# keonlee9420/Comprehensive-Transformer-TTS

Hardware: AMD Instinct MI355X
Metric: mel-frames/sec (train step) LJSpeech batch=16, 1/2/4/8 MI355X (higher is better)
Workload: dtype f32; 1 GPU; LJSpeech transformer_fs2 batch=16/GPU seq<=128->mel<=1024x80; full train step fwd+loss+bwd+clip+Adam, dropout on; workload_detail=supervised durations (BASELINE configs[1]), global_batch=16, valid_frames_per_gpu=11992, padded_frames_per_gpu=16384, launch_mode=hipgraph(fwd+bwd | clip+adam), parallelism=dp1

## Files before the change

### comprehensive-transformer-tts_amd/_lib.py

```python
import ctypes as C
import os

_HERE = os.path.dirname(os.path.abspath(__file__))
LIB_PATH = os.environ.get("CTTS_LIB") or os.path.join(_HERE, "csrc", "libctts_hip.so")

_c_f32p = C.c_void_p
_i32, _i64, _f32, _u32, _vp = C.c_int32, C.c_int64, C.c_float, C.c_uint32, C.c_void_p


class GemmDesc(C.Structure):
    _fields_ = [
        ("A", _vp), ("B", _vp), ("C", _vp),
        ("M", _i32), ("N", _i32), ("K", _i32),
        ("lda", _i64), ("ldb", _i64), ("ldc", _i64),
        ("a_kc", _i32), ("b_kc", _i32),
        ("nb0", _i32), ("nb1", _i32),
        ("sA0", _i64), ("sA1", _i64), ("sB0", _i64), ("sB1", _i64), ("sC0", _i64), ("sC1", _i64),
        ("lens", _vp),
        ("lim_m", _i32), ("lim_n", _i32), ("lim_k", _i32),
        ("conv_T", _i32), ("conv_pad", _i32), ("conv_cin", _i32), ("conv_on_b", _i32),
        ("split_k", _i32),
        ("alpha", _f32),
        ("bias", _vp),
        ("Z", _vp), ("ldz", _i64),
        ("act", _i32),
        ("p_drop", _f32), ("seed", _vp), ("drop_offset", _u32),
        ("R", _vp), ("ldr", _i64),
        ("rowscale", _vp),
        ("row_lens", _vp), ("row_T", _i32), ("row_halo", _i32),
        ("tile_map", _vp),
        ("tile_group_n", _i32),
        ("E", _vp), ("rowsub", _vp),
        ("sk_ws", _vp), ("sk_ws_bytes", _i64),
        ("epi_bwd", _i32),
        ("split_out", _vp), ("split_out_floats", _i64),
        ("split_overwrite", _i32),
        ("bf16_split", _i32),
        ("A_planes", _vp),
        ("B_planes", _vp),
        ("C_planes", _vp),
    ]


class VconvDesc(C.Structure):
    _fields_ = [
        ("x", _vp), ("sxb", _i64), ("sxt", _i64), ("sxc", _i64),
        ("B", _i32), ("T", _i32), ("Cin", _i32), ("Cout", _i32), ("k", _i32), ("dil", _i32),
        ("transposed_u", _i32),
        ("act_in", _i32), ("slope", _f32),
        ("w", _vp), ("w_planes", _vp),
        ("bias", _vp),
        ("R", _vp),
        ("out", _vp),
        ("alpha", _f32), ("beta", _f32),
        ("bf16_split", _i32),
        ("lens", _vp), ("len_mul", _i32),
    ]


class VconvHDesc(C.Structure):
    _fields_ = [
        ("x", _vp), ("sxb", _i64), ("sxt", _i64), ("sxc", _i64),
        ("x_f32", _i32),
        ("B", _i32), ("T", _i32), ("Cin", _i32), ("Cout", _i32), ("k", _i32), ("dil", _i32),
        ("transposed_u", _i32),
        ("act_in", _i32), ("slope", _f32),
        ("w", _vp),
        ("bias", _vp),
        ("R", _vp),
        ("out", _vp),
        ("alpha", _f32), ("beta", _f32),
        ("lens", _vp), ("len_mul", _i32),
    ]


class PsumTask(C.Structure):
    _fields_ = [("src", _vp), ("dst", _vp), ("n", _i64), ("stride", _i64), ("count", _i32), ("alpha", _f32)]


class SplitTask(C.Structure):
    _fields_ = [("src", _vp), ("dst", _vp), ("rows", _i64), ("cols", _i64), ("ld", _i64)]


class RepackTask(C.Structure):
    _fields_ = [("src", _vp), ("dst", _vp), ("cout", _i32), ("cin", _i32), ("k", _i32)]


_SIGNATURES = {
    "ctts_conv_dgrad_weights": [C.POINTER(RepackTask), C.c_int, _vp],
    "ctts_gemm_split_plan": [C.POINTER(GemmDesc), C.POINTER(_i32), C.POINTER(_i64)],
    "ctts_partial_sums": [C.POINTER(PsumTask), C.c_int, _vp],
    "ctts_reduce_parts": [C.c_int, _i64, C.c_int],
    "ctts_xcd_probe": [_vp, C.c_int, _vp],
    "ctts_posembed_fwd": [_vp, _vp, _vp, _vp, _vp, _vp, _i64, C.c_int, _f32, _vp, _u32, _vp],
    "ctts_posembed_bwd": [_vp, _vp, _vp, _vp, _vp, _vp, _i64, C.c_int, _f32, _vp, _u32, C.c_int, _vp, _vp],
    "ctts_gemm": [C.POINTER(GemmDesc), _vp],
    "ctts_gemm_takes_persistent": [C.POINTER(GemmDesc)],
    "ctts_gemm_ws_enable": [C.c_int],
    "ctts_gemm_takes_weight_stationary": [C.POINTER(GemmDesc)],
    "ctts_gemm_takes_bf16_split": [C.POINTER(GemmDesc)],
    "ctts_gemm_takes_planes": [C.POINTER(GemmDesc)],
    "ctts_split_planes": [C.POINTER(SplitTask), C.c_int, _vp],
    "ctts_rowdot_heads": [_vp, _vp, _vp, C.c_int, C.c_int, C.c_int, C.c_int, _vp],
    "ctts_mel_prepare": [_vp, C.c_int, C.c_int, _vp, _vp],
    "ctts_mel_spectrogram": [_vp, _vp, _vp, _vp, _vp, _vp, _vp, _i64, C.c_int, C.c_int, C.c_int, C.c_int, C.c_int, _f32, C.c_int, _vp, _vp],
    "ctts_mha_fwd": [_vp, _vp, _vp, _vp, C.c_int, C.c_int, C.c_int, C.c_int, _f32, _vp],
    "ctts_mha_bwd": [_vp, _vp, _vp, _vp, _vp, _vp, _vp, _vp, _vp, C.c_int, C.c_int, C.c_int, C.c_int, _f32, C.c_int, _vp, _vp],
    "ctts_relmha_fwd": [_vp, _vp, _vp, _vp, _vp, _vp, C.c_int, C.c_int, C.c_int, C.c_int, _f32, _f32, _vp, _u32, _vp],
    "ctts_relmha_bwd": [_vp, _vp, _vp, _vp, _vp, _vp, _vp, _vp, _vp, _vp, _vp, _vp, _vp, C.c_int, C.c_int, C.c_int, C.c_int,
                        _f32, _f32, _vp, _u32, _vp],
    "ctts_weighted_colsum": [_vp, _vp, _vp, _i64, C.c_int, _f32, C.c_int, _vp, _vp, _vp],
    "ctts_epilogue_bwd": [_vp, _vp, _vp, _vp, _vp, _vp, _i64, C.c_int, C.c_int, _f32, _vp, _u32, _f32, C.c_int, _vp, _vp, _vp],
    "ctts_row_tile_map": [_vp, C.c_int, C.c_int, C.c_int, _vp, _vp],
    "ctts_conv_weight_repack": [_vp, _vp, C.c_int, C.c_int, C.c_int, C.c_int, _vp],
    "ctts_lr_index": [_vp, C.c_int, C.c_int, _vp, C.c_int, C.c_int, C.c_int, _vp, _vp, _vp, _vp],
    "ctts_lr_gather_fwd": [_vp, _vp, _vp, C.c_int, C.c_int, C.c_int, C.c_int, _vp],
    "ctts_lr_gather_bwd": [_vp, _vp, _vp, C.c_int, C.c_int, C.c_int, C.c_int, _vp],
    "ctts_embedding_fwd": [_vp, _vp, _vp, _i64, C.c_int, C.c_int, _vp],
    "ctts_embedding_bwd": [_vp, _vp, _vp, _i64, C.c_int, C.c_int, C.c_int, C.c_int, _vp, _vp],
    "ctts_positions": [_vp, C.c_int, _i64, C.c_int, C.c_int, _vp, _vp],
    "ctts_cwt_pitch": [_vp, _i64, C.c_int, _vp, _vp, _f32, _vp, C.c_int, _f32, _f32, _f32, C.c_int, _vp, _vp, _vp, C.c_int, C.c_int, C.c_int, _vp],
    "ctts_layernorm_fwd": [_vp, _vp, _vp, _vp, _vp, _vp, C.c_int, C.c_int, _f32, _f32, _vp, _u32, _vp, _vp, _vp],
    "ctts_layernorm_bwd": [_vp, _vp, _vp, _vp, _vp, _vp, _vp, _vp, C.c_int, C.c_int, _f32, _vp, _u32, _vp, C.c_int, _vp, _vp, _vp, _vp],
    "ctts_colstats": [_vp, _vp, C.c_int, C.c_int, _vp, _vp],
    "ctts_bn_finalize": [_vp, C.c_int, C.c_int, _f32, _f32, _vp, _vp, _vp, _vp, _vp, _vp],
    "ctts_bn_apply": [_vp, _vp, _vp, _vp, _vp, _vp, C.c_int, C.c_int, C.c_int, _f32, _vp, _u32, _vp, _vp],
    "ctts_bn_bwd_reduce": [_vp, _vp, _vp, _vp, _vp, _vp, _vp, C.c_int, C.c_int, C.c_int, _f32, _vp, _u32, _vp, _vp],
    "ctts_bn_bwd_apply": [_vp, _vp, _vp, _vp, _vp, _vp, _vp, _vp, _vp, _vp, C.c_int, C.c_int, C.c_int, _f32, _vp,
                          _u32, C.c_int, _vp, _vp],
    "ctts_softmax_fwd": [_vp, _vp, C.c_int, C.c_int, C.c_int, _i64, _vp],
    "ctts_softmax_bwd": [_vp, _vp, _vp, C.c_int, C.c_int, C.c_int, _i64, _vp],
    "ctts_act_dropout_bwd": [_vp, _vp, _vp, _i64, C.c_int, C.c_int, _f32, _f32, _vp, _u32, _vp],
    "ctts_rowscale_dropout": [_vp, _vp, _i64, C.c_int, _vp, _f32, _vp, _u32, _vp],
    "ctts_colsum": [_vp, _vp, _i64, C.c_int, _i64, _f32, C.c_int, _vp, _vp, _vp],
    "ctts_reflect_pad": [_vp, _vp, C.c_int, C.c_int, C.c_int, _i64, _vp],
    "ctts_stft_magnitude": [_vp, _i64, _vp, _i64, _vp, _i64, C.c_int, _vp],
    "ctts_log_clamp_transpose": [_vp, _vp, C.c_int, C.c_int, C.c_int, _f32, _vp],
    "ctts_relattn_split_fwd": [_vp, _vp, _vp, _vp, _vp, _vp, _i64, C.c_int, _vp],
    "ctts_relattn_split_bwd": [_vp, _vp, _vp, _vp, _i64, C.c_int, _vp],
    "ctts_glu_fwd": [_vp, _vp, _i64, C.c_int, _vp],
    "ctts_glu_bwd": [_vp, _vp, _vp, _i64, C.c_int, _vp],
    "ctts_dwconv_fwd": [_vp, _vp, _vp, C.c_int, C.c_int, C.c_int, C.c_int, C.c_int, _vp],
    "ctts_dwconv_wgrad": [_vp, _vp, _vp, _vp, C.c_int, C.c_int, C.c_int, C.c_int, C.c_int, _vp],
    "ctts_relpos_softmax_fwd": [_vp, _vp, _vp, C.c_int, C.c_int, _f32, _f32, _vp, _u32, _vp],
    "ctts_relpos_softmax_bwd": [_vp, _vp, C.c_int, C.c_int, _f32, _f32, _vp, _u32, _vp],
    "ctts_relshift_bwd": [_vp, _vp, C.c_int, C.c_int, _vp],
    "ctts_neg_sqdist": [_vp, _vp, _vp, C.c_int, C.c_int, C.c_int, C.c_int, _f32, _vp],
    "ctts_mas": [_vp, _vp, _vp, _vp, _vp, _vp, C.c_int, C.c_int, C.c_int, _vp],
    "ctts_forward_sum_fwd": [_vp, _vp, _vp, _f32, _vp, _vp, _vp, C.c_int, C.c_int, C.c_int, _vp],
    "ctts_forward_sum_bwd": [_vp, _vp, _vp, _f32, _vp, _vp, _vp, _vp, _vp, C.c_int, C.c_int, C.c_int, _vp],
    "ctts_var_loss_fwd": [_vp] * 2 + [C.c_int] + [_vp] * 12 + [C.c_int] * 3 + [_vp, C.c_int, _vp] + [_vp] * 4 + [_vp],
    "ctts_var_loss_bwd": [_vp] * 2 + [C.c_int] + [_vp] * 12 + [C.c_int] * 3 + [_vp, C.c_int, _vp] + [_vp] * 4 + [_vp] * 5 + [_vp],
    "ctts_bin_loss_fwd": [_vp, _vp, _i64, _vp, _vp, _vp],
    "ctts_bin_loss_bwd": [_vp, _vp, _vp, _vp, _vp, _i64, _vp],
    "ctts_masked_loss_fwd": [_vp, _vp, _vp, _i64, _i32, _vp, _vp, _vp],
    "ctts_masked_loss_bwd": [_vp, _vp, _vp, _vp, _vp, _vp, _i64, _i32, _vp],
    "ctts_mel_l1_fwd": [_vp, _vp, _vp, _vp, _vp, _vp, _i64, C.c_int, _vp, _vp],
    "ctts_mel_l1_bwd": [_vp, _vp, _vp, _vp, _vp, _vp, _vp, _vp, _i64, C.c_int, _vp],
    "ctts_adam_clip_step": [_vp, _vp, _vp, _vp, C.c_int64, _vp, _f32, _f32, _f32, _f32, _f32, _vp, _vp],
    "ctts_im2col_3x3s2": [_vp, _vp, C.c_int, C.c_int, C.c_int, C.c_int, _vp],
    "ctts_col2im_3x3s2": [_vp, _vp, C.c_int, C.c_int, C.c_int, C.c_int, _vp],
    "ctts_gru_fwd": [_vp, _vp, _vp, _vp, _vp, C.c_int, C.c_int, C.c_int, C.c_int, C.c_int, _vp],
    "ctts_gru_bwd": [_vp, _vp, _vp, _vp, _vp, _vp, _vp, C.c_int, C.c_int, C.c_int, C.c_int, C.c_int, _vp],
    "ctts_softmax_rect_fwd": [_vp, _vp, _vp, C.c_int, C.c_int, C.c_int, _vp],
    "ctts_softmax_rect_bwd": [_vp, _vp, _vp, _vp, C.c_int, C.c_int, C.c_int, _vp],
    "ctts_vocoder_conv": [C.POINTER(VconvDesc), _vp],
    "ctts_vocoder_post": [_vp, C.c_int, C.c_int, C.c_int, C.c_int, _vp, _vp, _f32, _vp, _vp],
    "ctts_vocoder_post_ragged": [_vp, C.c_int, C.c_int, C.c_int, C.c_int, _vp, _vp, _f32, _vp, _vp, C.c_int, _vp],
    "ctts_vocoder_conv_h": [C.POINTER(VconvHDesc), _vp],
    "ctts_vocoder_post_h": [_vp, C.c_int, C.c_int, C.c_int, C.c_int, _vp, _vp, _f32, _vp, _vp, C.c_int, _vp],
    "ctts_fastformer_pool_fwd": [_vp, _i64, _vp, _i64, _vp, _vp, _vp, _vp, C.c_int, C.c_int, C.c_int, C.c_int, _f32, _vp],
    "ctts_fastformer_pool_bwd": [_vp, _vp, _vp, _vp, _i64, _vp, _i64, _vp, _vp, _vp, _vp, C.c_int, C.c_int, C.c_int, C.c_int, _f32, _vp],
    "ctts_fastformer_bcast": [_vp, _i64, _vp, _vp, C.c_int, C.c_int, C.c_int, _vp],
    "ctts_fastformer_bcast_bwd": [_vp, _vp, _vp, _i64, _vp, _vp, _vp, _vp, _vp, C.c_int, C.c_int, C.c_int, _vp],
    "ctts_fastformer_resdrop": [_vp, _vp, _vp, _vp, _i64, C.c_int, _vp, _f32, _vp, _u32, C.c_int, _vp],
    "ctts_griffinlim_prepare": [_vp, C.c_int, C.c_int, _vp, _vp],
    "ctts_stft_transform": [_vp, _vp, _vp, _vp, _vp, _i64, _i64, _i64, C.c_int, C.c_int, C.c_int, C.c_int, _vp],
    "ctts_istft_frames": [_vp, _vp, _i64, _i64, _i64, _vp, _vp, _vp, _vp, C.c_int, C.c_int, C.c_int, C.c_int, _vp],
    "ctts_griffinlim_iter": [_vp, _vp, _vp, _vp, _vp, C.c_int, C.c_int, C.c_int, C.c_int, _vp],
    "ctts_istft_ola": [_vp, _vp, _vp, _vp, _i64, C.c_int, C.c_int, C.c_int, C.c_int, _vp],
    "ctts_griffinlim_iter_momentum": [_vp, _vp, _vp, _vp, _vp, _vp, _f32, C.c_int, C.c_int, C.c_int, C.c_int, C.c_int, _vp],
    "ctts_istft_frames_seeded": [_vp, _i64, _i64, _i64, _vp, _vp, _vp, _vp, _vp, C.c_int, C.c_int, C.c_int, C.c_int, _vp],
    "ctts_pitch_track_prepare": [_vp, _vp],
    "ctts_pitch_track": [_vp, _vp, _vp, _vp, _vp, _vp, C.c_int, C.c_int, C.c_int, C.c_int, _f32, _f32, _f32, _f32, _vp],
    "ctts_f0_targets": [_vp, _vp, _vp, _vp, _vp, _vp, _vp, C.c_int, C.c_int, _vp],
    "ctts_norm_interp_f0": [_vp, _vp, _vp, _vp, C.c_int, C.c_int, _f32, _vp],
    "ctts_trim_silence": [_vp, _vp, _vp, _vp, _vp, C.c_int, C.c_int, _f32, C.c_int, C.c_int, _vp],
    "ctts_attn_prior": [_vp, _vp, _vp, C.c_int, C.c_int, C.c_int, _i64, _i64, _f32, _vp],
    "ctts_outlier_stats": [_vp, _vp, _vp, _vp, _vp, _vp, _vp, _vp, C.c_int, C.c_int, _vp],
    "ctts_comm_unique_id": [_vp],
    "ctts_comm_create": [C.POINTER(_vp), _i32, _i32, _vp],
    "ctts_comm_destroy": [_vp],
    "ctts_allreduce_mean": [_vp, _i64, _vp, _vp],
}
COMM_ID_BYTES = 128
EXPORTED_SYMBOLS = sorted(list(_SIGNATURES) + ["ctts_last_error", "ctts_version", "ctts_mha_supported", "ctts_relmha_workspace_floats",
                                               "ctts_mel_spectrogram_workspace_bytes", "ctts_gemm_workspace_bytes", "ctts_workspace_bytes",
                                               "ctts_workspace_error_word", "ctts_fastformer_workspace_floats",
                                               "ctts_griffinlim_workspace_bytes", "ctts_griffinlim_state_floats",
                                               "ctts_pitch_track_workspace_bytes", "ctts_trim_silence_workspace_bytes"])
ADAM_STATE_FLOATS = 3 + 2048

_lib = None


class CttsError(RuntimeError):
    pass


def load():
    global _lib
    if _lib is not None:
        return _lib
    if not os.path.exists(LIB_PATH):
        raise CttsError(
            f"{LIB_PATH} not found - build it with comprehensive-transformer-tts_amd/csrc/build.sh "
            "(or __graft_entry__.build()).  There is no CPU / PyTorch fallback for the hot path."
        )
    lib = C.CDLL(LIB_PATH)
    for name, argtypes in _SIGNATURES.items():
        fn = getattr(lib, name)
        fn.argtypes = argtypes
        fn.restype = C.c_int
    lib.ctts_last_error.restype = C.c_char_p
    lib.ctts_last_error.argtypes = []
    lib.ctts_version.restype = C.c_int
    lib.ctts_version.argtypes = []
    lib.ctts_mha_supported.restype = C.c_int
    lib.ctts_mha_supported.argtypes = [C.c_int, C.c_int]
    lib.ctts_mel_spectrogram_workspace_bytes.restype = C.c_size_t
    lib.ctts_mel_spectrogram_workspace_bytes.argtypes = [C.c_int, C.c_int]
    lib.ctts_gemm_workspace_bytes.restype = C.c_size_t
    lib.ctts_gemm_workspace_bytes.argtypes = []
    lib.ctts_workspace_bytes.restype = C.c_size_t
    lib.ctts_workspace_bytes.argtypes = []
    lib.ctts_workspace_error_word.restype = C.c_void_p
    lib.ctts_workspace_error_word.argtypes = [C.c_void_p]
    lib.ctts_fastformer_workspace_floats.restype = C.c_size_t
    lib.ctts_fastformer_workspace_floats.argtypes = [C.c_int, C.c_int, C.c_int, C.c_int]
    lib.ctts_griffinlim_workspace_bytes.restype = C.c_size_t
    lib.ctts_griffinlim_workspace_bytes.argtypes = [C.c_int, C.c_int]
    lib.ctts_griffinlim_state_floats.restype = C.c_size_t
    lib.ctts_griffinlim_state_floats.argtypes = [C.c_int, C.c_int]
    lib.ctts_pitch_track_workspace_bytes.restype = C.c_size_t
    lib.ctts_pitch_track_workspace_bytes.argtypes = []
    lib.ctts_trim_silence_workspace_bytes.restype = C.c_size_t
    lib.ctts_trim_silence_workspace_bytes.argtypes = [C.c_int, C.c_int, C.c_int]
    lib.ctts_relmha_workspace_floats.restype = C.c_size_t
    lib.ctts_relmha_workspace_floats.argtypes = [C.c_int, C.c_int, C.c_int]
    _lib = lib
    return lib

# ... 6 lines not shown
```

### comprehensive-transformer-tts_amd/csrc/elementwise.hip

```cpp
#include "ctts_common.h"

namespace {
__global__ void zero_u32_kernel(uint32_t* __restrict__ p, size_t n) {
  for (size_t i = (size_t)blockIdx.x * blockDim.x + threadIdx.x; i < n; i += (size_t)gridDim.x * blockDim.x) p[i] = 0u;
}
}

int ctts_zero_async(void* p, size_t bytes, hipStream_t st) {
  if (bytes == 0) return 0;
  const size_t n = (bytes + 3) / 4;
  const unsigned blocks = (unsigned)((n + 255) / 256 > 2048 ? 2048 : (n + 255) / 256);
  hipLaunchKernelGGL(zero_u32_kernel, dim3(blocks), dim3(256), 0, st, (uint32_t*)p, n);
  return hipGetLastError() == hipSuccess ? 0 : -1;
}

namespace {

__global__ void act_dropout_bwd_kernel(const float* __restrict__ dg, const float* __restrict__ z, float* __restrict__ dz,
                                       long total, int act, float p_drop, const uint64_t* seed, uint32_t drop_offset) {
  const bool do_drop = p_drop > 0.f;
  uint32_t dkey = 0; float inv_keep = 1.f;
  if (do_drop) { dkey = ctts_drop_key(seed, drop_offset); inv_keep = 1.f / (1.f - p_drop); }
  if (total & 3) {
    for (long i = (long)blockIdx.x * blockDim.x + threadIdx.x; i < total; i += (long)gridDim.x * blockDim.x) {
      float g = dg[i];
      if (do_drop) g *= ctts_drop_scale(dkey, (uint32_t)i, p_drop, inv_keep);
      dz[i] = g * ctts_act_grad(z[i], act);
    }
    return;
  }
  const long n4 = total >> 2;
  for (long i = (long)blockIdx.x * blockDim.x + threadIdx.x; i < n4; i += (long)gridDim.x * blockDim.x) {
    const float4 g = reinterpret_cast<const float4*>(dg)[i];
    const float4 zz = reinterpret_cast<const float4*>(z)[i];
    float ga[4] = {g.x, g.y, g.z, g.w};
    const float za[4] = {zz.x, zz.y, zz.z, zz.w};
#pragma unroll
    for (int e = 0; e < 4; ++e) {
      if (do_drop) ga[e] *= ctts_drop_scale(dkey, (uint32_t)(i * 4 + e), p_drop, inv_keep);
      ga[e] *= ctts_act_grad(za[e], act);
    }
    reinterpret_cast<float4*>(dz)[i] = make_float4(ga[0], ga[1], ga[2], ga[3]);
  }
}

__global__ void rowscale_dropout_kernel(const float* __restrict__ x, float* __restrict__ y, long total, int C,
                                        const float* __restrict__ rowscale, float p_drop, const uint64_t* seed,
                                        uint32_t drop_offset) {
  const bool do_drop = p_drop > 0.f;
  uint32_t dkey = 0; float inv_keep = 1.f;
  if (do_drop) { dkey = ctts_drop_key(seed, drop_offset); inv_keep = 1.f / (1.f - p_drop); }
  if (C & 3) {
    for (long i = (long)blockIdx.x * blockDim.x + threadIdx.x; i < total; i += (long)gridDim.x * blockDim.x) {
      float a = x[i];
      if (do_drop) a *= ctts_drop_scale(dkey, (uint32_t)i, p_drop, inv_keep);
      y[i] = a * (rowscale ? rowscale[i / C] : 1.f);
    }
    return;
  }
  const long n4 = total >> 2;
  const int C4 = C >> 2;
  for (long i = (long)blockIdx.x * blockDim.x + threadIdx.x; i < n4; i += (long)gridDim.x * blockDim.x) {
    const float4 v = reinterpret_cast<const float4*>(x)[i];
    float a[4] = {v.x, v.y, v.z, v.w};
    const float sc = rowscale ? rowscale[i / C4] : 1.f;
#pragma unroll
    for (int e = 0; e < 4; ++e) {
      if (do_drop) a[e] *= ctts_drop_scale(dkey, (uint32_t)(i * 4 + e), p_drop, inv_keep);
      a[e] *= sc;
    }
    reinterpret_cast<float4*>(y)[i] = make_float4(a[0], a[1], a[2], a[3]);
  }
}

__device__ __forceinline__ void ctts_colsum_emit(float tot, float* s64, float* __restrict__ out, int c, int C, int creal, float scale,
                                                 int accumulate) {
  const int ty = threadIdx.x >> 6, l = threadIdx.x & 63;
  if (C != creal) {
    __syncthreads();
    if (ty == 0) s64[l] = c < C ? tot : 0.f;
    __syncthreads();
    if (ty == 0 && l < creal) {
      float a = 0.f;
      for (int j = l; j < C; j += creal) a += s64[j];
      out[l] = accumulate ? out[l] + scale * a : scale * a;
    }
    return;
  }
  if (ty == 0 && c < C) out[c] = accumulate ? out[c] + scale * tot : scale * tot;
}

__global__ __launch_bounds__(256) void colsum_kernel(const float* __restrict__ x, float* __restrict__ out, long rows, int C,
                                                      int creal, long ld, float scale, unsigned char* ws, int G, int accumulate,
                                                      float* __restrict__ parts) {
  __shared__ float s[4][64];
  const int c = blockIdx.x * 64 + (threadIdx.x & 63), ty = threadIdx.x >> 6;
  const long stripe = (rows + gridDim.y - 1) / gridDim.y;
  const long r0 = blockIdx.y * stripe, r1 = min(rows, r0 + stripe);
  float a = 0.f;
  if (c < C) {
#pragma unroll 4
    for (long r = r0 + ty; r < r1; r += 4) a += x[r * ld + c];
  }
  s[ty][threadIdx.x & 63] = a;
  __syncthreads();
  float tot[1] = {0.f};
  if (ty == 0) { const int l = threadIdx.x; tot[0] = s[0][l] + s[1][l] + s[2][l] + s[3][l]; }
  if (parts) {
    if (ty == 0 && c < C) parts[(long)blockIdx.y * C + c] = tot[0];
    return;
  }
  if (!ctts_ordered_colsum<float, 1>(tot, ws, blockIdx.x, blockIdx.y, gridDim.y, G)) return;
  ctts_colsum_emit(tot[0], s[0], out, c, C, creal, scale, accumulate);
}

__global__ __launch_bounds__(256) void epilogue_bwd_kernel(const float* __restrict__ dy, const float* __restrict__ rowscale,
                                                            const float* __restrict__ z, float* __restrict__ dz, float* __restrict__ gm,
                                                            float* __restrict__ dbias, long rows, int C, int act, float p_drop,
                                                            const uint64_t* seed, uint32_t drop_offset, float bias_scale,
                                                            unsigned char* ws, int G, int accumulate, float* __restrict__ parts) {
  __shared__ float s[4][64];
  const int c = blockIdx.x * 64 + (threadIdx.x & 63), ty = threadIdx.x >> 6;
  const long stripe = (rows + gridDim.y - 1) / gridDim.y;
  const long r0 = blockIdx.y * stripe, r1 = min(rows, r0 + stripe);
  const bool do_drop = p_drop > 0.f;
  uint32_t dkey = 0; float inv_keep = 1.f;
  if (do_drop) { dkey = ctts_drop_key(seed, drop_offset); inv_keep = 1.f / (1.f - p_drop); }
  float a = 0.f;
  if (c < C) {
#pragma unroll 4
    for (long r = r0 + ty; r < r1; r += 4) {
      const long e = r * C + c;
      float g = dy[e];
      if (rowscale) g *= rowscale[r];
      if (gm) gm[e] = g;
      if (do_drop) g *= ctts_drop_scale(dkey, (uint32_t)e, p_drop, inv_keep);
      if (z) g *= ctts_act_grad(z[e], act);
      dz[e] = g;
      a += g;
    }
  }
  if (!dbias && !parts) return;
  s[ty][threadIdx.x & 63] = a;
  __syncthreads();
  float tot[1] = {0.f};
  if (ty == 0) { const int l = threadIdx.x; tot[0] = s[0][l] + s[1][l] + s[2][l] + s[3][l]; }
  if (parts) {
    if (ty == 0 && c < C) parts[(long)blockIdx.y * C + c] = tot[0];
    return;
  }
  if (!ctts_ordered_colsum<float, 1>(tot, ws, blockIdx.x, blockIdx.y, gridDim.y, G)) return;
  ctts_colsum_emit(tot[0], s[0], dbias, c, C, C, bias_scale, accumulate);
}
// ... 151 lines not shown
    return 0;
  }
  const int gx = (C + 63) / 64;
  const int gy = colsum_stripes(gx, min((long)max(1, 1024 / gx), (long)rows / 64), ws != nullptr || parts != nullptr);
  hipLaunchKernelGGL(weighted_colsum_kernel, dim3(gx, gy), dim3(256), 0, st, x, w, out, (long)rows, C, scale, (unsigned char*)ws,
                     ctts_red_group(gy), accumulate, parts);
  CTTS_CHECK_LAUNCH("ctts_weighted_colsum");
  return 0;
}

extern "C" int ctts_colsum(const float* x, float* out, int64_t rows, int C, int64_t ld, float scale, int accumulate, void* ws,
                           float* parts, void* stream) {
  CTTS_REQUIRE(x && (out || parts) && C > 0 && (C + 63) / 64 <= CTTS_RED_MAX_COLBLOCKS, "ctts_colsum: bad arguments");
  CTTS_REQUIRE(!parts || ctts_reduce_parts(0, rows, C) > 0, "ctts_colsum: this shape has no deferred mode (ctts_reduce_parts = 0)");
  hipStream_t st = (hipStream_t)stream;
  if (rows == 0) {
    if (!accumulate && ctts_zero_async(out, sizeof(float) * C, st) != 0) { ctts_set_error("ctts_colsum: zero fill failed"); return -2; }
    return 0;
  }
  int k = 1;
  if (ld == C && !parts)
    while (C * k * 2 <= 64 && rows % (k * 2) == 0) k *= 2;
  const int Cv = C * k, gx = (Cv + 63) / 64;
  const long Rv = rows / k;
  const int gy = colsum_stripes(gx, min((long)max(1, 1024 / gx), Rv / 64), ws != nullptr || parts != nullptr);
  hipLaunchKernelGGL(colsum_kernel, dim3(gx, gy), dim3(256), 0, st, x, out, Rv, Cv, C, (long)ld * k, scale, (unsigned char*)ws,
                     ctts_red_group(gy), accumulate, parts);
  CTTS_CHECK_LAUNCH("ctts_colsum");
  return 0;
}

extern "C" int ctts_epilogue_bwd(const float* dy, const float* rowscale, const float* z, float* dz, float* gm, float* dbias,
                                 int64_t rows, int C, int act, float p_drop, const uint64_t* seed, uint32_t drop_offset, float bias_scale,
                                 int accumulate_bias, void* ws, float* parts, void* stream) {
  CTTS_REQUIRE(dy && dz && rows >= 0 && C > 0 && p_drop >= 0.f && p_drop < 1.f && (p_drop == 0.f || seed), "ctts_epilogue_bwd: bad arguments");
  CTTS_REQUIRE(!dbias || (C + 63) / 64 <= CTTS_RED_MAX_COLBLOCKS, "ctts_epilogue_bwd: C too large for the bias-gradient reduction");
  hipStream_t st = (hipStream_t)stream;
  if (rows == 0) {
    if (dbias && !accumulate_bias && ctts_zero_async(dbias, sizeof(float) * C, st) != 0) { ctts_set_error("ctts_epilogue_bwd: zero fill failed"); return -2; }
    return 0;
  }
  const int gx = (C + 63) / 64;
  const long want = min((long)max(1, 2048 / gx), (long)rows / 32);
  CTTS_REQUIRE(!parts || rows > 0, "ctts_epilogue_bwd: deferred bias gradient needs rows > 0");
  const int gy = (dbias || parts) ? colsum_stripes(gx, want, ws != nullptr || parts != nullptr) : (int)max((long)1, want);
  hipLaunchKernelGGL(epilogue_bwd_kernel, dim3(gx, gy), dim3(256), 0, st, dy, rowscale, act ? z : nullptr, dz, gm, dbias, (long)rows, C, act,
                     p_drop, seed, drop_offset, bias_scale, (unsigned char*)ws, ctts_red_group(gy), accumulate_bias, parts);
  CTTS_CHECK_LAUNCH("ctts_epilogue_bwd");
  return 0;
}

extern "C" int ctts_conv_weight_repack(const float* src, float* dst, int cout, int cin, int k, int mode, void* stream) {
  CTTS_REQUIRE(src && dst && mode >= 0 && mode <= 4, "ctts_conv_weight_repack: bad arguments");
  const long total = (long)cout * cin * k;
  if (total == 0) return 0;
  hipLaunchKernelGGL(conv_weight_repack_kernel, dim3(grid_for(total)), dim3(256), 0, (hipStream_t)stream, src, dst, cout, cin, k,
                     mode, total);
  CTTS_CHECK_LAUNCH("ctts_conv_weight_repack");
  return 0;
}

extern "C" int ctts_reflect_pad(const float* y, float* ypad, int B, int N, int pad, int64_t ld_out, void* stream) {
  CTTS_REQUIRE(y && ypad && N > pad && ld_out >= N + 2 * pad, "ctts_reflect_pad: need N > pad and ld_out >= N + 2*pad");
  const long total = (long)B * ld_out;
  if (total == 0) return 0;
  hipLaunchKernelGGL(reflect_pad_kernel, dim3(grid_for(total)), dim3(256), 0, (hipStream_t)stream, y, ypad, N, pad, (long)ld_out, total);
  CTTS_CHECK_LAUNCH("ctts_reflect_pad");
  return 0;
}

extern "C" int ctts_stft_magnitude(const float* reim, int64_t ld_reim, float* mag, int64_t ld_mag, float* energy,
                                   int64_t frames, int nbins, void* stream) {
  CTTS_REQUIRE(reim && mag && energy && ld_mag >= nbins, "ctts_stft_magnitude: bad arguments");
  if (frames == 0) return 0;
  const int blocks = (int)min((frames + 3) / 4, (int64_t)4096);
  hipLaunchKernelGGL(stft_magnitude_kernel, dim3(blocks), dim3(256), 0, (hipStream_t)stream, reim, (long)ld_reim, mag,
                     (long)ld_mag, energy, (long)frames, nbins);
  CTTS_CHECK_LAUNCH("ctts_stft_magnitude");
  return 0;
}

extern "C" int ctts_log_clamp_transpose(const float* mel_fm, float* out, int B, int F, int n_mel, float clip, void* stream) {
  CTTS_REQUIRE(mel_fm && out, "ctts_log_clamp_transpose: null pointer");
  const long total = (long)B * F * n_mel;
  if (total == 0) return 0;
  hipLaunchKernelGGL(log_clamp_transpose_kernel, dim3(grid_for(total)), dim3(256), 0, (hipStream_t)stream, mel_fm, out, F, n_mel,
                     clip, total);
  CTTS_CHECK_LAUNCH("ctts_log_clamp_transpose");
  return 0;
}


namespace {
constexpr int RPK_BATCH = 32;
struct RepackBatch {
  const float* src[RPK_BATCH];
  float* dst[RPK_BATCH];
  int cout[RPK_BATCH], cin[RPK_BATCH], k[RPK_BATCH];
  int first_block[RPK_BATCH + 1];
  int ntasks;
};

__global__ __launch_bounds__(256) void conv_dgrad_weights_kernel(const RepackBatch b) {
  __shared__ float tile[32][33];
  int t = 0;
  while (t + 1 < b.ntasks && (int)blockIdx.x >= b.first_block[t + 1]) ++t;
  const float* __restrict__ src = b.src[t];
  float* __restrict__ dst = b.dst[t];
  const int cout = b.cout[t], cin = b.cin[t], k = b.k[t];
  const int tco = (cout + 31) / 32, tci = (cin + 31) / 32;
  int blk = (int)blockIdx.x - b.first_block[t];
  const int kk = blk / (tco * tci);
  blk -= kk * tco * tci;
  const int co0 = (blk / tci) * 32, ci0 = (blk % tci) * 32;
  const int tx = threadIdx.x & 31, ty = threadIdx.x >> 5;
#pragma unroll
  for (int r = ty; r < 32; r += 8) {
    const int co = co0 + r, ci = ci0 + tx;
    tile[r][tx] = (co < cout && ci < cin) ? src[((long)co * k + (k - 1 - kk)) * cin + ci] : 0.f;
  }
  __syncthreads();
#pragma unroll
  for (int r = ty; r < 32; r += 8) {
    const int ci = ci0 + r, co = co0 + tx;
    if (ci < cin && co < cout) dst[((long)ci * k + kk) * cout + co] = tile[tx][r];
  }
}
}

extern "C" int ctts_conv_dgrad_weights(const ctts_repack_task* tasks, int ntasks, void* stream) {
  CTTS_REQUIRE(ntasks >= 0 && (tasks || ntasks == 0), "ctts_conv_dgrad_weights: bad arguments");
  hipStream_t st = (hipStream_t)stream;
  for (int t0 = 0; t0 < ntasks; t0 += RPK_BATCH) {
    RepackBatch b;
    b.ntasks = 0;
    int blocks = 0;
    for (int t = t0; t < ntasks && t < t0 + RPK_BATCH; ++t) {
      const ctts_repack_task& q = tasks[t];
      CTTS_REQUIRE(q.src && q.dst && q.cout > 0 && q.cin > 0 && q.k > 0, "ctts_conv_dgrad_weights: bad task %d", t);
      const int i = b.ntasks++;
      b.src[i] = q.src; b.dst[i] = q.dst; b.cout[i] = q.cout; b.cin[i] = q.cin; b.k[i] = q.k;
      b.first_block[i] = blocks;
      blocks += ((q.cout + 31) / 32) * ((q.cin + 31) / 32) * q.k;
    }
    if (b.ntasks == 0) continue;
    b.first_block[b.ntasks] = blocks;
    hipLaunchKernelGGL(conv_dgrad_weights_kernel, dim3(blocks), dim3(256), 0, st, b);
    CTTS_CHECK_LAUNCH("ctts_conv_dgrad_weights");
  }
  return 0;
}

namespace {
__global__ __launch_bounds__(256) void posembed_fwd_kernel(const float4* __restrict__ x, const int32_t* __restrict__ pos, const float4* __restrict__ table,
                                                            const float* __restrict__ alpha, const float* __restrict__ rowscale, float4* __restrict__ y,
                                                            long n4, int C4, float p_drop, const uint64_t* seed, uint32_t drop_offset) {
#pragma clang fp contract(off)
  const bool do_drop = p_drop > 0.f;
  uint32_t dkey = 0; float inv_keep = 1.f;
  if (do_drop) { dkey = ctts_drop_key(seed, drop_offset); inv_keep = 1.f / (1.f - p_drop); }
  const float a = alpha ? alpha[0] : 1.f;
  for (long i = (long)blockIdx.x * blockDim.x + threadIdx.x; i < n4; i += (long)gridDim.x * blockDim.x) {
    const long row = i / C4;
    const int c = (int)(i - row * C4);
    const float4 xv = x[i], tv = table[(long)pos[row] * C4 + c];
    float v[4] = {xv.x + a * tv.x, xv.y + a * tv.y, xv.z + a * tv.z, xv.w + a * tv.w};
    const float sc = rowscale ? rowscale[row] : 1.f;
#pragma unroll
    for (int e = 0; e < 4; ++e) {
      if (do_drop) v[e] *= ctts_drop_scale(dkey, (uint32_t)(i * 4 + e), p_drop, inv_keep);
      v[e] *= sc;
    }
    y[i] = make_float4(v[0], v[1], v[2], v[3]);
  }
}

__global__ __launch_bounds__(256) void posembed_bwd_kernel(const float4* __restrict__ dy, const int32_t* __restrict__ pos, const float4* __restrict__ table,
                                                            const float* __restrict__ rowscale, float4* __restrict__ dx, float* __restrict__ dalpha,
                                                            long n4, int C4, float p_drop, const uint64_t* seed, uint32_t drop_offset,
                                                            unsigned char* ws, int G, int accumulate) {
  __shared__ float s_w[4];
  const bool do_drop = p_drop > 0.f;
  uint32_t dkey = 0; float inv_keep = 1.f;
  if (do_drop) { dkey = ctts_drop_key(seed, drop_offset); inv_keep = 1.f / (1.f - p_drop); }
  float dot = 0.f;
  for (long i = (long)blockIdx.x * blockDim.x + threadIdx.x; i < n4; i += (long)gridDim.x * blockDim.x) {
    const long row = i / C4;
    const int c = (int)(i - row * C4);
    const float4 g = dy[i];
    float v[4] = {g.x, g.y, g.z, g.w};
    const float sc = rowscale ? rowscale[row] : 1.f;
#pragma unroll
    for (int e = 0; e < 4; ++e) {
      v[e] *= sc;
      if (do_drop) v[e] *= ctts_drop_scale(dkey, (uint32_t)(i * 4 + e), p_drop, inv_keep);
    }
    dx[i] = make_float4(v[0], v[1], v[2], v[3]);
    if (dalpha) {
      const float4 tv = table[(long)pos[row] * C4 + c];
      dot += v[0] * tv.x + v[1] * tv.y + v[2] * tv.z + v[3] * tv.w;
    }
  }
  if (!dalpha) return;
  dot = ctts_wave_sum(dot);
  if ((threadIdx.x & 63) == 0) s_w[threadIdx.x >> 6] = dot;
  __syncthreads();
  float tot[1] = {0.f};
  if (threadIdx.x == 0) tot[0] = ((s_w[0] + s_w[1]) + s_w[2]) + s_w[3];
  if (!ctts_ordered_colsum<float, 1>(tot, ws, 0, blockIdx.x, gridDim.x, G)) return;
  if (threadIdx.x == 0) dalpha[0] = accumulate ? dalpha[0] + tot[0] : tot[0];
}
}

extern "C" int ctts_posembed_fwd(const float* x, const int32_t* pos, const float* table, const float* alpha, const float* rowscale, float* y,
                                 int64_t rows, int C, float p_drop, const uint64_t* seed, uint32_t drop_offset, void* stream) {
  CTTS_REQUIRE(x && pos && table && y && rows >= 0 && C > 0 && (C % 4) == 0 && p_drop >= 0.f && p_drop < 1.f && (p_drop == 0.f || seed),
               "ctts_posembed_fwd: bad arguments (C %% 4 must be 0)");
  const long n4 = (long)rows * (C / 4);
  if (n4 == 0) return 0;
  hipLaunchKernelGGL(posembed_fwd_kernel, dim3(grid_for(n4)), dim3(256), 0, (hipStream_t)stream, (const float4*)x, pos, (const float4*)table, alpha,
                     rowscale, (float4*)y, n4, C / 4, p_drop, seed, drop_offset);
  CTTS_CHECK_LAUNCH("ctts_posembed_fwd");
  return 0;
}

extern "C" int ctts_posembed_bwd(const float* dy, const int32_t* pos, const float* table, const float* rowscale, float* dx, float* dalpha,
                                 int64_t rows, int C, float p_drop, const uint64_t* seed, uint32_t drop_offset, int accumulate, void* ws,
                                 void* stream) {
  CTTS_REQUIRE(dy && dx && rows >= 0 && C > 0 && (C % 4) == 0 && p_drop >= 0.f && p_drop < 1.f && (p_drop == 0.f || seed) &&
               (!dalpha || (pos && table)), "ctts_posembed_bwd: bad arguments (C %% 4 must be 0)");
  const long n4 = (long)rows * (C / 4);
  hipStream_t st = (hipStream_t)stream;
  if (n4 == 0) {
    if (dalpha && !accumulate && ctts_zero_async(dalpha, sizeof(float), st) != 0) return -2;
    return 0;
  }
  int grid = grid_for(n4, 1024);
  if (dalpha && !ws) grid = 1;
  hipLaunchKernelGGL(posembed_bwd_kernel, dim3(grid), dim3(256), 0, st, (const float4*)dy, pos, (const float4*)table, rowscale, (float4*)dx, dalpha,
                     n4, C / 4, p_drop, seed, drop_offset, (unsigned char*)ws, ctts_red_group(grid), accumulate);
  CTTS_CHECK_LAUNCH("ctts_posembed_bwd");
  return 0;
}

namespace {
constexpr int PSUM_BATCH = 24;
struct PsumBatch {
  const float* src[PSUM_BATCH];
  float* dst[PSUM_BATCH];
  long n[PSUM_BATCH];
  long stride[PSUM_BATCH];
  int count[PSUM_BATCH];
  float alpha[PSUM_BATCH];
  int first_block[PSUM_BATCH + 1];
  int ntasks;
};

#ifndef CTTS_PSUM_CHUNKS
#define CTTS_PSUM_CHUNKS 8
#endif
constexpr int PSUM_CHUNKS = CTTS_PSUM_CHUNKS;
__global__ __launch_bounds__(256) void partial_sums_kernel(const PsumBatch b) {
  int t = 0;
  while (t + 1 < b.ntasks && (int)blockIdx.x >= b.first_block[t + 1]) ++t;
  const float* src = b.src[t];
  float* dst = b.dst[t];
  const long n = b.n[t], stride = b.stride[t];
  const int count = b.count[t];
  const float alpha = b.alpha[t];
  const bool aligned = !(stride & 3) && !((reinterpret_cast<uintptr_t>(src) | reinterpret_cast<uintptr_t>(dst)) & 15);
  const long s4 = stride >> 2;
#pragma unroll 1
  for (int c = 0; c < PSUM_CHUNKS; ++c) {
    const long i0 = (((long)(blockIdx.x - b.first_block[t]) * PSUM_CHUNKS + c) * 256 + threadIdx.x) * 4;
    if (i0 >= n) return;
    if (aligned && i0 + 4 <= n) {
      const float4* p = reinterpret_cast<const float4*>(src + i0);
      float4 a = make_float4(0.f, 0.f, 0.f, 0.f);
      for (int s = 0; s < count; s += 8) {
        float4 v[8];
#pragma unroll
        for (int u = 0; u < 8; ++u) v[u] = (s + u < count) ? p[(long)(s + u) * s4] : make_float4(0.f, 0.f, 0.f, 0.f);
#pragma unroll
        for (int u = 0; u < 8; ++u) { a.x += v[u].x; a.y += v[u].y; a.z += v[u].z; a.w += v[u].w; }
      }
      float4 cc = *reinterpret_cast<float4*>(dst + i0);
      cc.x += alpha * a.x; cc.y += alpha * a.y; cc.z += alpha * a.z; cc.w += alpha * a.w;
      *reinterpret_cast<float4*>(dst + i0) = cc;
    } else {
      for (int q = 0; q < 4 && i0 + q < n; ++q) {
        float a = 0.f;
        for (int s = 0; s < count; ++s) a += src[(long)s * stride + i0 + q];
        dst[i0 + q] += alpha * a;
      }
    }
  }
}
}

extern "C" int ctts_partial_sums(const ctts_psum_task* tasks, int ntasks, void* stream) {
  CTTS_REQUIRE(ntasks >= 0 && (tasks || ntasks == 0), "ctts_partial_sums: bad arguments");
  hipStream_t st = (hipStream_t)stream;
  for (int t0 = 0; t0 < ntasks; t0 += PSUM_BATCH) {
    PsumBatch b;
    b.ntasks = 0;
    int blocks = 0;
// ... 17 lines not shown
```

### comprehensive-transformer-tts_amd/csrc/gemm_common.h

```cpp
#pragma once
#include "ctts_common.h"

typedef float floatx16 __attribute__((ext_vector_type(16)));

namespace {

template <int MT, int NT>
__device__ __forceinline__ void gemm_epilogue(const ctts_gemm_desc& d, floatx16 (&acc)[MT][NT], float* Cb, int z, int row0, int col0,
                                              int wm0, int wn0, int l31, int h, int Mv, int Nv) {
  const float alpha = d.alpha;
  const bool do_drop = d.p_drop > 0.f;
  uint32_t dkey = 0;
  float inv_keep = 1.f;
  if (do_drop) { dkey = ctts_drop_key(d.seed, d.drop_offset); inv_keep = 1.f / (1.f - d.p_drop); }
  const uint32_t zoff = (uint32_t)z * (uint32_t)d.M * (uint32_t)d.N;
  if (d.E) {
    const float* Eb = d.E + (Cb - d.C);
    const float* rs = d.rowsub + (long)z * d.M;
#pragma unroll
    for (int i = 0; i < MT; ++i)
#pragma unroll
      for (int j = 0; j < NT; ++j) {
        const int n = col0 + wn0 + j * 32 + l31;
#pragma unroll
        for (int r = 0; r < 16; ++r) {
          const int m = row0 + wm0 + i * 32 + (r & 3) + 8 * (r >> 2) + 4 * h;
          if (m < Mv && n < Nv) Cb[(long)m * d.ldc + n] = Eb[(long)m * d.ldc + n] * (alpha * acc[i][j][r] - rs[m]);
        }
      }
    return;
  }
  if (d.epi_bwd) {
#pragma unroll
    for (int i = 0; i < MT; ++i)
#pragma unroll
      for (int j = 0; j < NT; ++j) {
        const int n = col0 + wn0 + j * 32 + l31;
#pragma unroll
        for (int r = 0; r < 16; ++r) {
          const int m = row0 + wm0 + i * 32 + (r & 3) + 8 * (r >> 2) + 4 * h;
          if (m < Mv && n < Nv) {
            float v = alpha * acc[i][j][r];
            if (do_drop) v *= ctts_drop_scale(dkey, zoff + (uint32_t)m * (uint32_t)d.N + (uint32_t)n, d.p_drop, inv_keep);
            if (d.act) v *= ctts_act_grad(d.Z[(long)m * d.ldz + n], d.act);
            Cb[(long)m * d.ldc + n] = v;
          }
        }
      }
    return;
  }
#pragma unroll
  for (int i = 0; i < MT; ++i)
#pragma unroll
    for (int j = 0; j < NT; ++j) {
      const int n = col0 + wn0 + j * 32 + l31;
      const float bv = (d.bias && n < Nv) ? d.bias[n] : 0.f;
#pragma unroll
      for (int r = 0; r < 16; ++r) {
        const int m = row0 + wm0 + i * 32 + (r & 3) + 8 * (r >> 2) + 4 * h;
        if (m < Mv && n < Nv) {
          float v = alpha * (acc[i][j][r] + bv);
          if (d.Z) d.Z[(long)m * d.ldz + n] = v;
          v = ctts_act(v, d.act);
          if (do_drop) v *= ctts_drop_scale(dkey, zoff + (uint32_t)m * (uint32_t)d.N + (uint32_t)n, d.p_drop, inv_keep);
          if (d.R) v += d.R[(long)m * d.ldr + n];
          if (d.rowscale) v *= d.rowscale[m];
          Cb[(long)m * d.ldc + n] = v;
        }
      }
    }
}


constexpr unsigned GEMM_OOB = 0x80000000u;

typedef __bf16 gemm_bf16x2 __attribute__((ext_vector_type(2)));
typedef float gemm_floatx2 __attribute__((ext_vector_type(2)));
__device__ __forceinline__ void gemm_split3(float x, unsigned& hi, unsigned& mid, unsigned& lo) {
  const gemm_floatx2 v0 = {x, 0.f};
  unsigned hb = __builtin_bit_cast(unsigned, __builtin_convertvector(v0, gemm_bf16x2)) & 0xFFFFu;
  const bool x_fin = fabsf(x) < __builtin_inff();
  if ((hb & 0x7F80u) == 0x7F80u) {
    if (x_fin) hb = (hb & 0x8000u) | 0x7F7Fu;
    else { hi = hb; mid = 0u; lo = 0u; return; }
  }
  const float r1 = x - __uint_as_float(hb << 16);
  const gemm_floatx2 v1 = {r1, 0.f};
  const unsigned mb = __builtin_bit_cast(unsigned, __builtin_convertvector(v1, gemm_bf16x2)) & 0xFFFFu;
  const float r2 = r1 - __uint_as_float(mb << 16);
  const gemm_floatx2 v2 = {r2, 0.f};
  const unsigned lb = __builtin_bit_cast(unsigned, __builtin_convertvector(v2, gemm_bf16x2)) & 0xFFFFu;
  hi = hb; mid = mb; lo = lb;
}
__device__ __host__ __forceinline__ bool gemm_fits32(const void* p, long M, long ld, long N);

__device__ __forceinline__ __amdgpu_buffer_rsrc_t gemm_rsrc(const void* p, long bytes) {
  return __builtin_amdgcn_make_buffer_rsrc(const_cast<void*>(p), 0, (int)bytes, 0x00020000);
}

template <int MT, int NT, int ACT, bool DROP, bool BWD, bool AUX, bool RS = false, bool PLANES = false>
__device__ __forceinline__ void gemm_epilogue_lean(const ctts_gemm_desc& d, const floatx16 (&acc)[MT][NT], float* Cb, int z, int row0,
                                                   int col0, int wm0, int wn0, int l31, int h, int Mv, int Nv) {
#pragma clang fp contract(off)
  const bool planes_on = PLANES && d.C_planes != nullptr;
  const __amdgpu_buffer_rsrc_t rp = gemm_rsrc(d.C_planes, planes_on ? (long)Mv * d.ldc * 6 : 0);
  const unsigned p_row = (unsigned)(d.ldc * 6);
  const unsigned p_sel = (l31 & 1) ? 0x03020706u : 0x05040100u;
  const float alpha = d.alpha;
  uint32_t dkey = 0;
  float inv_keep = 1.f;
  if (DROP) { dkey = ctts_drop_key(d.seed, d.drop_offset); inv_keep = 1.f / (1.f - d.p_drop); }
  const uint32_t zoff = (uint32_t)z * (uint32_t)d.M * (uint32_t)d.N;
  const uint32_t dthr = DROP ? ctts_drop_threshold(d.p_drop) : 0u;
  const uint32_t drow = (uint32_t)d.N * CTTS_DROP_G;
  const long last = Mv - 1;
  const float* aux_p = BWD ? d.Z : d.R;
  const long aux_ld = BWD ? d.ldz : d.ldr;
  const bool has_z = !BWD && ACT && d.Z;
  const __amdgpu_buffer_rsrc_t rc = gemm_rsrc(Cb, (last * d.ldc + Nv) * 4);
  const __amdgpu_buffer_rsrc_t ra = gemm_rsrc(aux_p, AUX ? (last * aux_ld + Nv) * 4 : 0);
  const __amdgpu_buffer_rsrc_t rz = gemm_rsrc(d.Z, has_z ? (last * d.ldz + Nv) * 4 : 0);
  const __amdgpu_buffer_rsrc_t rr = gemm_rsrc(d.rowscale, RS ? (long)Mv * 4 : 0);
  const unsigned c_row = (unsigned)(d.ldc * 4), a_row = (unsigned)(aux_ld * 4), z_row = (unsigned)(d.ldz * 4);
#pragma unroll
  for (int j = 0; j < NT; ++j) {
    const int n = col0 + wn0 + j * 32 + l31;
    const bool n_ok = n < Nv;
    const unsigned c_lane = n_ok ? (unsigned)(4 * h) * c_row + (unsigned)n * 4u : GEMM_OOB;
    const unsigned a_lane = n_ok ? (unsigned)(4 * h) * a_row + (unsigned)n * 4u : GEMM_OOB;
    const unsigned z_lane = n_ok ? (unsigned)(4 * h) * z_row + (unsigned)n * 4u : GEMM_OOB;
    const float bv = (!BWD && d.bias && n_ok) ? d.bias[n] : 0.f;
    const uint32_t dlane = (zoff + (uint32_t)(4 * h) * (uint32_t)d.N + (uint32_t)n) * CTTS_DROP_G + dkey;
    const unsigned p_lane = n_ok ? (unsigned)(4 * h + (l31 & 1)) * p_row + (unsigned)(n >> 5) * 192u + (unsigned)(n & 30) * 2u : GEMM_OOB;
#pragma unroll
    for (int ib = 0; ib < 2 * MT; ++ib) {
      const int i = ib >> 1, rb = (ib & 1) * 8;
      float aux[8], rs[8];
      if (AUX) {
#pragma unroll
        for (int q = 0; q < 8; ++q) {
          const int r = rb + q, mu = row0 + wm0 + i * 32 + (r & 3) + 8 * (r >> 2);
          aux[q] = __builtin_bit_cast(float, __builtin_amdgcn_raw_buffer_load_b32(ra, a_lane + (unsigned)mu * a_row, 0, 0));
        }
      }
      if (RS) {
#pragma unroll
        for (int q = 0; q < 8; ++q) {
          const int r = rb + q, mu = row0 + wm0 + i * 32 + (r & 3) + 8 * (r >> 2);
          rs[q] = __builtin_bit_cast(float, __builtin_amdgcn_raw_buffer_load_b32(rr, (unsigned)(mu + 4 * h) * 4u, 0, 0));
        }
      }
#pragma unroll
      for (int q = 0; q < 8; ++q) {
        const int r = rb + q, mu = row0 + wm0 + i * 32 + (r & 3) + 8 * (r >> 2);
        const int m = mu + 4 * h;
        float v;
        if (BWD) {
          v = alpha * acc[i][j][r];
          if (DROP) v *= ctts_drop_scale_pre(dlane + (uint32_t)mu * drow, dthr, inv_keep);
          if (ACT) v *= ctts_act_grad(aux[q], ACT);
        } else {
          v = alpha * (acc[i][j][r] + bv);
          if (ACT) __builtin_amdgcn_raw_buffer_store_b32(__builtin_bit_cast(unsigned, v), rz, z_lane + (unsigned)mu * z_row, 0, 0);
          v = ctts_act(v, ACT);
          if (DROP) v *= ctts_drop_scale_pre(dlane + (uint32_t)mu * drow, dthr, inv_keep);
          if (AUX) v += aux[q];
          if (RS) v *= rs[q];
        }
        __builtin_amdgcn_raw_buffer_store_b32(__builtin_bit_cast(unsigned, v), rc, c_lane + (unsigned)mu * c_row, 0, 0);
        if (PLANES) aux[q] = v;
      }
      if (PLANES) {
        if (planes_on) {
#pragma unroll
          for (int q = 0; q < 8; q += 2) {
            const int r = rb + q, mu = row0 + wm0 + i * 32 + (r & 3) + 8 * (r >> 2);
            unsigned ha, ma, la, hb, mb, lb;
            gemm_split3(aux[q], ha, ma, la);
            gemm_split3(aux[q + 1], hb, mb, lb);
            const unsigned own[3] = {ha | (hb << 16), ma | (mb << 16), la | (lb << 16)};
#pragma unroll
            for (int pc = 0; pc < 3; ++pc) {
              const unsigned nbr = (unsigned)__builtin_amdgcn_mov_dpp((int)own[pc], 0xB1, 0xF, 0xF, true);
              const unsigned out = __builtin_amdgcn_perm(nbr, own[pc], p_sel);
              __builtin_amdgcn_raw_buffer_store_b32(out, rp, p_lane + (unsigned)mu * p_row + (unsigned)(pc * 64), 0, 0);
            }
          }
        }
      }
    }
  }
}

template <int MT, int NT>
__device__ __forceinline__ void gemm_accumulate_lean(const ctts_gemm_desc& d, const floatx16 (&acc)[MT][NT], float* Cb, int row0, int col0,
                                                     int wm0, int wn0, int l31, int h, int Mv, int Nv) {
  const __amdgpu_buffer_rsrc_t rc = gemm_rsrc(Cb, ((long)(Mv - 1) * d.ldc + Nv) * 4);
  const unsigned c_row = (unsigned)(d.ldc * 4);
#pragma unroll
  for (int j = 0; j < NT; ++j) {
    const int n = col0 + wn0 + j * 32 + l31;
    const unsigned c_lane = n < Nv ? (unsigned)(4 * h) * c_row + (unsigned)n * 4u : GEMM_OOB;
#pragma unroll
    for (int ib = 0; ib < 2 * MT; ++ib) {
      const int i = ib >> 1, rb = (ib & 1) * 8;
      float old[8];
#pragma unroll
      for (int q = 0; q < 8; ++q) {
        const int r = rb + q, mu = row0 + wm0 + i * 32 + (r & 3) + 8 * (r >> 2);
        old[q] = __builtin_bit_cast(float, __builtin_amdgcn_raw_buffer_load_b32(rc, c_lane + (unsigned)mu * c_row, 0, 0));
      }
#pragma unroll
      for (int q = 0; q < 8; ++q) {
        const int r = rb + q, mu = row0 + wm0 + i * 32 + (r & 3) + 8 * (r >> 2);
        const float v = old[q] + d.alpha * acc[i][j][r];
        __builtin_amdgcn_raw_buffer_store_b32(__builtin_bit_cast(unsigned, v), rc, c_lane + (unsigned)mu * c_row, 0, 0);
      }
    }
  }
}

__device__ __host__ __forceinline__ long gemm_partial_ld(int N) { return (long)((N + 3) / 4) * 4; }
__device__ __forceinline__ float* gemm_partial_base(const ctts_gemm_desc& d, int z, int split) {
  float* P = reinterpret_cast<float*>(reinterpret_cast<unsigned char*>(d.sk_ws) + CTTS_WS_SLABS);
  return P + ((long)z * d.split_k + split) * (long)d.M * gemm_partial_ld(d.N);
}

template <int MT, int NT>
__device__ __forceinline__ void gemm_softmax_bwd_lean(const ctts_gemm_desc& d, const floatx16 (&acc)[MT][NT], float* Cb, int z, int row0,
                                                      int col0, int wm0, int wn0, int l31, int h, int Mv, int Nv) {
  const long bytes = ((long)(Mv - 1) * d.ldc + Nv) * 4;
  const __amdgpu_buffer_rsrc_t rc = gemm_rsrc(Cb, bytes);
  const __amdgpu_buffer_rsrc_t re = gemm_rsrc(d.E + (Cb - d.C), bytes);
  const __amdgpu_buffer_rsrc_t rr = gemm_rsrc(d.rowsub + (long)z * d.M, (long)Mv * 4);
  const unsigned c_row = (unsigned)(d.ldc * 4);
#pragma unroll
  for (int i = 0; i < MT; ++i) {
    float rs[16];
#pragma unroll
    for (int r = 0; r < 16; ++r)
      rs[r] = __builtin_bit_cast(float, __builtin_amdgcn_raw_buffer_load_b32(rr, (unsigned)(row0 + wm0 + i * 32 + (r & 3) + 8 * (r >> 2) + 4 * h) * 4u, 0, 0));
#pragma unroll
    for (int j = 0; j < NT; ++j) {
      const int n = col0 + wn0 + j * 32 + l31;
      const unsigned c_lane = n < Nv ? (unsigned)(4 * h) * c_row + (unsigned)n * 4u : GEMM_OOB;
#pragma unroll
      for (int rb = 0; rb < 16; rb += 8) {
        float e[8];
#pragma unroll
        for (int q = 0; q < 8; ++q) {
          const int r = rb + q, mu = row0 + wm0 + i * 32 + (r & 3) + 8 * (r >> 2);
          e[q] = __builtin_bit_cast(float, __builtin_amdgcn_raw_buffer_load_b32(re, c_lane + (unsigned)mu * c_row, 0, 0));
        }
#pragma unroll
        for (int q = 0; q < 8; ++q) {
          const int r = rb + q, mu = row0 + wm0 + i * 32 + (r & 3) + 8 * (r >> 2);
          const float v = e[q] * (d.alpha * acc[i][j][r] - rs[r]);
          __builtin_amdgcn_raw_buffer_store_b32(__builtin_bit_cast(unsigned, v), rc, c_lane + (unsigned)mu * c_row, 0, 0);
        }
      }
    }
  }
}

__device__ __host__ __forceinline__ bool gemm_fits32(const void* p, long M, long ld, long N) {
  return !p || ((M + 128) * ld * 4 < 0x7FFF0000L && ld >= N);
}

template <int MT, int NT>
__device__ __forceinline__ void gemm_epilogue_auto(const ctts_gemm_desc& d, floatx16 (&acc)[MT][NT], float* Cb, int z, int row0, int col0,
                                                   int wm0, int wn0, int l31, int h, int Mv, int Nv) {
  const bool flat = d.nb0 * d.nb1 == 1 && Mv == d.M && Nv == d.N;
  const bool c_ok = gemm_fits32(Cb, Mv, d.ldc, Nv);
  if (d.E) {
    if (c_ok) return gemm_softmax_bwd_lean<MT, NT>(d, acc, Cb, z, row0, col0, wm0, wn0, l31, h, Mv, Nv);
  } else if (c_ok && (flat ? gemm_fits32(d.Z, d.M, d.ldz, d.N) && gemm_fits32(d.R, d.M, d.ldr, d.N) : !d.Z && !d.R && !d.rowscale)) {
#define CTTS_LEAN(ACT, DROP, BWD, AUX, RS) \
  return gemm_epilogue_lean<MT, NT, ACT, DROP, BWD, AUX, RS>(d, acc, Cb, z, row0, col0, wm0, wn0, l31, h, Mv, Nv)
    const bool drop = d.p_drop > 0.f, res = d.R != nullptr, rs = d.rowscale != nullptr;
    if (!d.epi_bwd) {
      if (d.act == 0 && !d.Z) {
        if (!res && !rs && !drop) CTTS_LEAN(0, false, false, false, false);
        if (res && !rs) { if (drop) CTTS_LEAN(0, true, false, true, false); else CTTS_LEAN(0, false, false, true, false); }
        if (res && rs) { if (drop) CTTS_LEAN(0, true, false, true, true); else CTTS_LEAN(0, false, false, true, true); }
      } else if (!res && !rs && flat) {
        if (d.act == 1 && !drop) CTTS_LEAN(1, false, false, false, false);
        if (d.act == 2) { if (drop) CTTS_LEAN(2, true, false, false, false); else CTTS_LEAN(2, false, false, false, false); }
        if (d.act == 4) { if (drop) CTTS_LEAN(4, true, false, false, false); else CTTS_LEAN(4, false, false, false, false); }
      }
    } else if (d.Z && !rs && flat) {
      if (d.act == 1 && !drop) CTTS_LEAN(1, false, true, true, false);
      if (d.act == 2 && drop) CTTS_LEAN(2, true, true, true, false);
      if (d.act == 4 && drop) CTTS_LEAN(4, true, true, true, false);
    }
#undef CTTS_LEAN
  }
  gemm_epilogue<MT, NT>(d, acc, Cb, z, row0, col0, wm0, wn0, l31, h, Mv, Nv);
}

}

int ctts_gemm_sk_try(const ctts_gemm_desc& d, hipStream_t st);

int ctts_gemm_ws_try(const ctts_gemm_desc& d, hipStream_t st);

int ctts_gemm_pl_try(const ctts_gemm_desc& d, hipStream_t st);

int ctts_gemm_plw_try(const ctts_gemm_desc& d, hipStream_t st);
int ctts_gemm_plw_takes(const ctts_gemm_desc& d);
```

### comprehensive-transformer-tts_amd/csrc/gemm_pl.hip

```cpp
#include "gemm_pl_common.h"
#include "planes_common.h"
#include <stdlib.h>
#include <type_traits>

namespace {

struct PlArgs {
  int tiles_m, tiles_n;
  int nkb;
  int gw;
  int whole_tiles;
  int ntap;
  int nutt, tpu;
  int debug;
  unsigned* ws;
};

__host__ __device__ __forceinline__ int pl_epilogue_kind(const ctts_gemm_desc& d) {
  const bool drop = d.p_drop > 0.f, res = d.R != nullptr, rs = d.rowscale != nullptr;
  if (d.E || !gemm_fits32(d.C, d.M, d.ldc, d.N) || !gemm_fits32(d.Z, d.M, d.ldz, d.N) || !gemm_fits32(d.R, d.M, d.ldr, d.N)) return -1;
  if (d.epi_bwd) {
    if (d.Z && !rs && drop && d.act == 2) return 8;
    if (d.Z && !rs && drop && d.act == 4) return 9;
    return -1;
// ... 250 lines not shown
    const bool do_mma = PL_DBG(8) == 0 && !(SKEW && idle);
    if (do_mma) {
      read_frag(stage, 1, f1);
      mma_terms(f0, 0, 6);
      if constexpr (TERMS == 1) { PL_INTERLEAVE_4x1(); } else { PL_INTERLEAVE_12(); }
    }
    __builtin_amdgcn_sched_barrier(0);
    __builtin_amdgcn_s_waitcnt(0xC07F);
    asm volatile("s_waitcnt vmcnt(0)\n\ts_barrier" ::: "memory");
    if constexpr (!SKEW) {
      if (have_l && !PL_DBG(1)) loader_issue(stage);
      __builtin_amdgcn_sched_barrier(0);
    }
    if (do_mma) {
      read_frag(stage ^ 1, 0, f0);
      mma_terms(f1, 0, 6);
      if constexpr (TERMS == 1) { PL_INTERLEAVE_4x1(); } else { PL_INTERLEAVE_12(); }
    }
    __builtin_amdgcn_sched_barrier(0);
    if constexpr (SKEW) {
      if (have_l && !PL_DBG(1)) loader_issue(stage);
    }
    if (have_l) loader_advance();
    --remaining;
    ++ckb;
    stage ^= 1;
    if (ckb < cp.kb_hi) continue;

    int e_l31 = l31, e_h = h, e_wm0 = wm0, e_wn0 = wn0;
    unsigned long long kargs = (unsigned long long)(const void*)__builtin_amdgcn_kernarg_segment_ptr();
    asm volatile("" : "+v"(e_l31), "+v"(e_h), "+s"(e_wm0), "+s"(e_wn0), "+s"(kargs));
    const ctts_gemm_desc& dc = *(const ctts_gemm_desc*)(const __attribute__((address_space(4))) ctts_gemm_desc*)kargs;
    const int Mv = dc.M, Nv = dc.N;
    int row0, col0; bool pad_hi;
    decode(cp, row0, col0, pad_hi);
    if (cp.kb_hi < nkb) {
      const unsigned base = (unsigned)blockIdx.x * (PL_SLAB * 4) + (unsigned)(wave * (PL_SLAB / 8) + lane * 4) * 4u;
#pragma unroll
      for (int i = 0; i < 2; ++i)
#pragma unroll
        for (int j = 0; j < 2; ++j)
#pragma unroll
          for (int q = 0; q < 4; ++q) {
            pl_u32x4 v;
            v.x = __float_as_uint(acc[i][j][4 * q + 0]); v.y = __float_as_uint(acc[i][j][4 * q + 1]);
            v.z = __float_as_uint(acc[i][j][4 * q + 2]); v.w = __float_as_uint(acc[i][j][4 * q + 3]);
            __builtin_amdgcn_raw_buffer_store_b128(v, rs_src, base + (unsigned)(((i * 2 + j) * 4 + q) * 1024), 0, 16);
          }
      asm volatile("s_waitcnt vmcnt(0)" ::: "memory");
      __syncthreads();
      if (tid == 0) __hip_atomic_store((pl_gu32*)(flags + blockIdx.x), 1u, __ATOMIC_RELAXED, __HIP_MEMORY_SCOPE_AGENT);
    } else {
      if (cp.kb_lo > 0) {
        const int tile_lo = cp.t * nkb;
        const int Ux = (rg.T1 - rg.T0) * nkb;
        int upper = rg.lo;
        for (int jj = wj - 1; jj >= 0 && upper > tile_lo; --jj) {
          const int blo = sk_bound(g, Ux, jj);
          if (blo >= upper) continue;
          upper = blo;
          const int src = jj * 8 + xcd;
          if (tid == 0) {
            unsigned spins = 0;
            while (__hip_atomic_load((pl_gu32*)(flags + src), __ATOMIC_RELAXED, __HIP_MEMORY_SCOPE_AGENT) != 1u) {
              __builtin_amdgcn_s_sleep(8);
              if (++spins > (1u << 24)) {
                __hip_atomic_store((pl_gu32*)(flags + PL_MAX_WG), 1u + (unsigned)src, __ATOMIC_RELAXED, __HIP_MEMORY_SCOPE_AGENT);
                break;
              }
            }
            __hip_atomic_store((pl_gu32*)(flags + src), 0u, __ATOMIC_RELAXED, __HIP_MEMORY_SCOPE_AGENT);
            __builtin_amdgcn_fence(__ATOMIC_ACQUIRE, "agent");
          }
          asm volatile("s_waitcnt vmcnt(0)" ::: "memory");
          __syncthreads();
          const unsigned base = (unsigned)src * (PL_SLAB * 4) + (unsigned)(wave * (PL_SLAB / 8) + lane * 4) * 4u;
#pragma unroll
          for (int g = 0; g < 16 / PL_SLAB_BATCH; ++g) {
            pl_u32x4 sv[PL_SLAB_BATCH];
#pragma unroll
            for (int e = 0; e < PL_SLAB_BATCH; ++e) sv[e] = __builtin_amdgcn_raw_buffer_load_b128(rs_src, base + (unsigned)((g * PL_SLAB_BATCH + e) * 1024), 0, 0);
#pragma unroll
            for (int e = 0; e < PL_SLAB_BATCH; ++e) {
              const int n = g * PL_SLAB_BATCH + e, i = n >> 3, j = (n >> 2) & 1, q = n & 3;
              acc[i][j][4 * q + 0] += __uint_as_float(sv[e].x); acc[i][j][4 * q + 1] += __uint_as_float(sv[e].y);
              acc[i][j][4 * q + 2] += __uint_as_float(sv[e].z); acc[i][j][4 * q + 3] += __uint_as_float(sv[e].w);
            }
          }
        }
      }
      if (pad_hi && e_wm0 == 64) {
        for (int e = lane; e < 64 * 64; e += 64) {
          const int r = e >> 6, c = e & 63;
          const int n = col0 + e_wn0 + c;
          if (n < Nv) {
            dc.C[(long)(row0 + 64 + r) * dc.ldc + n] = 0.f;
            if (dc.Z && !dc.epi_bwd) dc.Z[(long)(row0 + 64 + r) * dc.ldz + n] = 0.f;
          }
        }
      } else if (!PL_DBG(4)) {
        pl_epilogue(dc, acc, row0, col0, e_wm0, e_wn0, e_l31, e_h, Mv, Nv);
      }
    }
    if (PL_DBG(16) && blockIdx.x == 8 && tid == 0) {
      unsigned long long* o = reinterpret_cast<unsigned long long*>(p.ws + PL_MAX_WG + 2);
      o[0] = clock64() - dbg_c0;
      o[1] = wall_clock64() - dbg_w0;
    }
    __builtin_amdgcn_s_waitcnt(0);
    if (!sk_next_piece(cu, rg.lo, nkb, cp)) break;
    ckb = cp.kb_lo;
    zero_acc();
    if constexpr (SKEW) { int r0_, c0_; decode(cp, r0_, c0_, idle); }
    read_frag(stage, 0, f0);
  }
  };
  if (wave >= 4 && !PL_DBG(32)) run(std::true_type{});
  else run(std::false_type{});
}

int pl_env(const char* name, int dflt) {
  const char* v = getenv(name);
  return v ? atoi(v) : dflt;
}

constexpr int SPL_BATCH = 32;
struct SplitBatch {
  const float* src[SPL_BATCH];
  uint16_t* dst[SPL_BATCH];
  long rows[SPL_BATCH], cols8[SPL_BATCH], ld[SPL_BATCH];
  int first_block[SPL_BATCH + 1];
  int ntasks;
};
constexpr int SPL_PER_BLOCK = 256 * 4;

__global__ __launch_bounds__(256) void split_planes_kernel(const SplitBatch b) {
  int t = 0;
  while (t + 1 < b.ntasks && (int)blockIdx.x >= b.first_block[t + 1]) ++t;
  const float* __restrict__ src = b.src[t];
  uint16_t* __restrict__ dst = b.dst[t];
  const long c8 = b.cols8[t], ld = b.ld[t], n8 = b.rows[t] * c8;
  const long g0 = (long)((int)blockIdx.x - b.first_block[t]) * SPL_PER_BLOCK;
#pragma unroll
  for (int u = 0; u < 4; ++u) {
    const long gidx = g0 + u * 256 + threadIdx.x;
    if (gidx >= n8) continue;
    const long r = gidx / c8, c = (gidx - r * c8) * 8;
    const float4 x0 = *reinterpret_cast<const float4*>(src + r * ld + c), x1 = *reinterpret_cast<const float4*>(src + r * ld + c + 4);
    const float xs[8] = {x0.x, x0.y, x0.z, x0.w, x1.x, x1.y, x1.z, x1.w};
    spl_store8(dst, r, ld, c, xs);
  }
}

}

extern "C" int ctts_split_planes(const ctts_split_task* tasks, int ntasks, void* stream) {
  CTTS_REQUIRE(ntasks >= 0 && (tasks || ntasks == 0), "ctts_split_planes: bad arguments");
  hipStream_t st = (hipStream_t)stream;
  for (int t0 = 0; t0 < ntasks; t0 += SPL_BATCH) {
    SplitBatch b;
    b.ntasks = 0;
    long blocks = 0;
    for (int t = t0; t < ntasks && t < t0 + SPL_BATCH; ++t) {
      const ctts_split_task& q = tasks[t];
      CTTS_REQUIRE(q.src && q.dst && q.rows >= 0 && q.cols >= 0 && q.cols % 32 == 0 && q.ld >= q.cols && q.ld % 32 == 0 &&
                       (reinterpret_cast<uintptr_t>(q.src) & 15) == 0 && (reinterpret_cast<uintptr_t>(q.dst) & 15) == 0,
                   "ctts_split_planes: task %d needs 16-byte aligned pointers, cols %% 32 == 0 and ld %% 32 == 0", t);
      if (q.rows == 0 || q.cols == 0) continue;
      const int i = b.ntasks++;
      b.src[i] = q.src; b.dst[i] = q.dst; b.rows[i] = q.rows; b.cols8[i] = q.cols / 8; b.ld[i] = q.ld;
      b.first_block[i] = (int)blocks;
      blocks += (q.rows * (q.cols / 8) + SPL_PER_BLOCK - 1) / SPL_PER_BLOCK;
      CTTS_REQUIRE(blocks < (1L << 30), "ctts_split_planes: too many elements in one call");
    }
    if (b.ntasks == 0) continue;
    b.first_block[b.ntasks] = (int)blocks;
    hipLaunchKernelGGL(split_planes_kernel, dim3((unsigned)blocks), dim3(256), 0, st, b);
    CTTS_CHECK_LAUNCH("ctts_split_planes");
  }
  return 0;
}

static int pl_try(const ctts_gemm_desc& d, hipStream_t st, bool launch) {
  static const int enabled = pl_env("CTTS_PL", 1);
  static const int min_units = pl_env("CTTS_PL_MIN_UNITS", 4096);
  static const int split_from = pl_env("CTTS_PL_SPLIT_NKB", 24);
  static const int max_split = pl_env("CTTS_PL_MAX_SPLIT", 8);
  static const int wg_units = pl_env("CTTS_PL_WG_UNITS", 16);
  static const int force_w = pl_env("CTTS_PL_W", 0);
  static const int debug = pl_env("CTTS_PL_DEBUG", 0);
  if (!enabled || d.bf16_split < 1 || !d.A_planes || !d.B_planes) return 0;
  if (!d.sk_ws || d.sk_ws_bytes < (int64_t)CTTS_WS_BYTES) return 0;
  if (!d.a_kc || !d.b_kc || d.nb0 * d.nb1 != 1 || d.lens || d.E) return 0;
  if (d.split_k > 1 && !d.split_overwrite) return 0;
  if (d.K % 32 != 0 || d.K < 64 || d.N % 128 != 0 || d.N < 256 || d.M < 128) return 0;
  auto al16 = [](const void* q) { return (reinterpret_cast<uintptr_t>(q) & 15) == 0; };
  if (!al16(d.A_planes) || !al16(d.B_planes) || ((d.lda | d.ldb) & 31)) return 0;
  const bool conv = d.conv_T > 0;
  if (conv && (d.conv_on_b || d.conv_cin % 32 != 0 || d.K % d.conv_cin != 0 || d.conv_T < 16)) return 0;
  const long a_ext = (long)(d.M + 256) * d.lda * 3 + 3L * d.K;
  const long b_ext = (long)(d.N + 256) * d.ldb * 3 + 3L * d.K;
  if (a_ext * 2 >= 0x7FFF0000L || b_ext * 2 >= 0x7FFF0000L) return 0;
  if (pl_epilogue_kind(d) < 0) return 0;
  PlArgs p;
  p.nutt = p.tpu = 0;
  p.tiles_m = (d.M + PL_BM - 1) / PL_BM;
  long act_tiles_m = p.tiles_m;
  if (d.row_lens) {
    if (d.row_T <= 0 || d.row_T % PL_BM != 0 || d.M % d.row_T != 0 || d.M / d.row_T > PL_MAX_UTT) return 0;
    p.nutt = d.M / d.row_T;
    p.tpu = d.row_T / PL_BM;
  }
  p.tiles_n = (d.N + PL_BN - 1) / PL_BN;
  p.nkb = d.K / 32;
  p.ntap = conv ? d.K / d.conv_cin : 1;
  p.whole_tiles = p.nkb < split_from ? 1 : 0;
  p.gw = (p.tiles_n % 4 == 0) ? p.tiles_n / 4 : p.tiles_n;
  p.debug = debug;
  p.ws = reinterpret_cast<unsigned*>(d.sk_ws);
  const long tiles = act_tiles_m * p.tiles_n;
  const long units = tiles * p.nkb;
  const bool forced = d.bf16_split == 2 || d.bf16_split == 4;
  if (!forced && units < min_units) return 0;
  const int cuts = p.whole_tiles ? 1 : ((p.nkb >= 256 && max_split < 4) ? 4 : max_split);
  long W = force_w > 0 ? force_w : 32;
  const long Wu = units / (8L * wg_units);
  if (W > Wu) W = Wu;
  const long Wt = (d.row_lens && p.tpu >= 4) ? (tiles * cuts * 3 / 4) / 8 : (tiles * cuts) / 8;
  if (W > Wt) W = Wt;
  if (W < 1) {
    if (!forced) return 0;
    W = 1;
  }
  const int grid = (int)W * 8;
  if (grid > PL_MAX_WG || (long)grid * PL_SLAB > PL_SLAB_FLOATS_MAX) return 0;
  if (!launch) return 1;
  if (d.bf16_split >= 3) {
    if (conv) hipLaunchKernelGGL((gemm_pl_kernel<true, 1>), dim3(grid), dim3(512), 0, st, d, p);
    else hipLaunchKernelGGL((gemm_pl_kernel<false, 1>), dim3(grid), dim3(512), 0, st, d, p);
  } else {
    if (conv) hipLaunchKernelGGL((gemm_pl_kernel<true, 6>), dim3(grid), dim3(512), 0, st, d, p);
    else hipLaunchKernelGGL((gemm_pl_kernel<false, 6>), dim3(grid), dim3(512), 0, st, d, p);
  }
  CTTS_CHECK_LAUNCH("ctts_gemm(planes)");
  return 1;
}

int ctts_gemm_pl_try(const ctts_gemm_desc& d, hipStream_t st) { return pl_try(d, st, true); }

extern "C" int ctts_gemm_takes_planes(const ctts_gemm_desc* d) {
  if (!d) return 0;
  ctts_gemm_desc c = *d;
  if (c.nb0 < 1) c.nb0 = 1;
  if (c.nb1 < 1) c.nb1 = 1;
  return (pl_try(c, nullptr, false) > 0 || ctts_gemm_plw_takes(c)) ? 1 : 0;
}
```

### comprehensive-transformer-tts_amd/csrc/gemm_ws.hip

```cpp
#include "ctts_common.h"
#include "gemm_common.h"
#include <stdlib.h>
#include <type_traits>

namespace {

typedef int ws_i32x4 __attribute__((ext_vector_type(4)));
typedef unsigned int ws_u32x4 __attribute__((ext_vector_type(4)));
constexpr unsigned WS_OOB = GEMM_OOB;

__device__ __forceinline__ ws_i32x4 ws_make_rsrc(const void* base) {
  const unsigned long long a = reinterpret_cast<unsigned long long>(base);
  ws_i32x4 r;
  r.x = __builtin_amdgcn_readfirstlane((int)(unsigned)a);
  r.y = __builtin_amdgcn_readfirstlane((int)(unsigned)(a >> 32));
  r.z = 0x7FFFFFFE;
  r.w = 0x00020000;
  return r;
}

__device__ __forceinline__ void ws_dma16(ws_i32x4 rsrc, unsigned lds_addr, unsigned voff) {
  asm volatile("s_mov_b32 m0, %0\n\tbuffer_load_dwordx4 %1, %2, 0 offen lds"
               :: "s"(__builtin_amdgcn_readfirstlane(lds_addr)), "v"(voff), "s"(rsrc) : "memory");
}

struct WsArgs {
  int tiles_m;
  int n_blocks;
  int wg_per_block;
  int xcd_aligned;
  int debug;
};

template <int KB, bool B_KC, int ACT, bool DROP, bool BWD, bool AUX>
__global__ __launch_bounds__(256, 2) void gemm_ws_kernel(const ctts_gemm_desc d, const WsArgs p) {
  constexpr int HB = KB / 2;
  constexpr int STAGE = 64 * HB * 32;
  extern __shared__ __attribute__((aligned(16))) float smem[];
  const int tid = threadIdx.x, lane = tid & 63;
  const int wave = __builtin_amdgcn_readfirstlane(tid >> 6);
  const int l31 = lane & 31, h = lane >> 5;
  int nb, wj;
  if (p.xcd_aligned) {
    const int xcd = blockIdx.x & 7, idx = blockIdx.x >> 3;
    nb = idx % p.n_blocks;
    wj = (idx / p.n_blocks) * 8 + xcd;
  } else {
    nb = blockIdx.x % p.n_blocks;
    wj = blockIdx.x / p.n_blocks;
  }
  const int col0 = nb * 128, wn0 = wave * 32;
  const int n = col0 + wn0 + l31;

  typedef const __attribute__((address_space(4))) int32_t* ws_cmap;
  const ws_cmap mmap = (ws_cmap)(uintptr_t)d.tile_map;
  const int n_mt = mmap ? mmap[0] : p.tiles_m;
  if (mmap) {
    const int n_zero = (p.tiles_m - n_mt) * p.n_blocks;
    for (int zt = blockIdx.x; zt < n_zero; zt += gridDim.x) {
      const int mi = zt / p.n_blocks, zb = zt - mi * p.n_blocks;
      const int row0 = mmap[1 + n_mt + mi] * 64, c0 = zb * 128;
      const int nrows = min(64, d.M - row0), ncols = min(128, d.N - c0);
      for (int e = tid; e < nrows * 128; e += 256) {
        const int r = e >> 7, c = e & 127;
        if (c < ncols) {
          d.C[(long)(row0 + r) * d.ldc + c0 + c] = 0.f;
          if (d.Z && !d.epi_bwd) d.Z[(long)(row0 + r) * d.ldz + c0 + c] = 0.f;
        }
      }
      if (BWD && d.C_planes) {
        for (int e = tid; e < nrows * 48; e += 256) {
          const int r = e / 48, q = e - r * 48;
          if (q * 8 / 96 * 32 < ncols)
            *reinterpret_cast<uint4*>(d.C_planes + (long)(row0 + r) * d.ldc * 3 + (long)(c0 >> 5) * 96 + q * 8) = make_uint4(0u, 0u, 0u, 0u);
        }
      }
    }
  }
  const ws_i32x4 ra_src = ws_make_rsrc(d.A);
  const unsigned smem_addr = (unsigned)reinterpret_cast<uintptr_t>(smem);
  const int r_in = lane >> 3;
  const int c_in = lane & 7;
  auto issue_half = [&](int slot, int half) {
    const int row0 = (mmap ? mmap[1 + slot] : slot) * 64;
    for (int kbi = wave; kbi < HB; kbi += 4) {
#pragma unroll
      for (int g = 0; g < 8; ++g) {
        const int r = g * 8 + r_in;
        const int c = c_in ^ ((r >> 1) & 7);
        const int row = row0 + r;
        const unsigned v = row < d.M ? ((unsigned)row * (unsigned)d.lda + (unsigned)((half * HB + kbi) * 32 + c * 4)) * 4u : WS_OOB;
        ws_dma16(ra_src, smem_addr + (unsigned)(half * STAGE + kbi * 2048 + g * 256) * 4u, v);
      }
    }
  };
  if (wj < n_mt) issue_half(wj, 0);
  float bf[KB][16];
  if (n < d.N) {
    if (B_KC) {
      const float* bp = d.B + (long)n * d.ldb + h * 16;
#pragma unroll
      for (int kb = 0; kb < KB; ++kb)
#pragma unroll
        for (int q = 0; q < 4; ++q) {
          const float4 v = *reinterpret_cast<const float4*>(bp + kb * 32 + q * 4);
          bf[kb][4 * q + 0] = v.x; bf[kb][4 * q + 1] = v.y; bf[kb][4 * q + 2] = v.z; bf[kb][4 * q + 3] = v.w;
        }
    } else {
      const float* bp = d.B + (long)(h * 16) * d.ldb + n;
#pragma unroll
      for (int kb = 0; kb < KB; ++kb)
#pragma unroll
        for (int j = 0; j < 16; ++j) bf[kb][j] = bp[(long)(kb * 32 + j) * d.ldb];
    }
  } else {
#pragma unroll
    for (int kb = 0; kb < KB; ++kb)
#pragma unroll
      for (int j = 0; j < 16; ++j) bf[kb][j] = 0.f;
  }

  const int sw = (l31 >> 1) & 7;
  floatx16 acc[2][1];
  auto compute_half = [&](auto HALF) {
    constexpr int half = decltype(HALF)::value;
    const float* sA = smem + half * STAGE + l31 * 32;
    auto ld = [&](int g, int i) {
      return *reinterpret_cast<const float4*>(sA + (g >> 2) * 2048 + i * 1024 + (((h * 4 + (g & 3)) ^ sw) << 2));
    };
    float4 c0 = ld(0, 0), c1 = ld(0, 1);
#pragma unroll
    for (int g = 0; g < HB * 4; ++g) {
      float4 n0 = c0, n1 = c1;
      if (g + 1 < HB * 4) { n0 = ld(g + 1, 0); n1 = ld(g + 1, 1); }
      __builtin_amdgcn_sched_barrier(0);
      const int kb = half * HB + (g >> 2), j = (g & 3) * 4;
      acc[0][0] = __builtin_amdgcn_mfma_f32_32x32x2f32(c0.x, bf[kb][j + 0], acc[0][0], 0, 0, 0);
      acc[1][0] = __builtin_amdgcn_mfma_f32_32x32x2f32(c1.x, bf[kb][j + 0], acc[1][0], 0, 0, 0);
      acc[0][0] = __builtin_amdgcn_mfma_f32_32x32x2f32(c0.y, bf[kb][j + 1], acc[0][0], 0, 0, 0);
      acc[1][0] = __builtin_amdgcn_mfma_f32_32x32x2f32(c1.y, bf[kb][j + 1], acc[1][0], 0, 0, 0);
      acc[0][0] = __builtin_amdgcn_mfma_f32_32x32x2f32(c0.z, bf[kb][j + 2], acc[0][0], 0, 0, 0);
      acc[1][0] = __builtin_amdgcn_mfma_f32_32x32x2f32(c1.z, bf[kb][j + 2], acc[1][0], 0, 0, 0);
      acc[0][0] = __builtin_amdgcn_mfma_f32_32x32x2f32(c0.w, bf[kb][j + 3], acc[0][0], 0, 0, 0);
      acc[1][0] = __builtin_amdgcn_mfma_f32_32x32x2f32(c1.w, bf[kb][j + 3], acc[1][0], 0, 0, 0);
      c0 = n0; c1 = n1;
    }
  };
  const bool wave_has_cols = col0 + wn0 < d.N;

  int slot = wj;
  long long t_start = 0, t_loop = 0, t_w1 = 0, t_w2 = 0, t_epi = 0, t_c0 = 0, t_c1 = 0;
  if (p.debug & 1) t_start = __builtin_readcyclecounter();
  int n_done = 0;
  for (; slot < n_mt; slot += p.wg_per_block) {
    const int row0 = (mmap ? mmap[1 + slot] : slot) * 64;
    long long t0 = 0, t1 = 0;
    if (p.debug & 1) t0 = __builtin_readcyclecounter();
    asm volatile("s_waitcnt vmcnt(0)\n\ts_barrier" ::: "memory");
    __builtin_amdgcn_s_waitcnt(0);
    if (p.debug & 1) { t1 = __builtin_readcyclecounter(); if (n_done == 0) t_loop = t1; else t_w1 += t1 - t0; }
    if (!(p.debug & 4)) issue_half(slot, 1);
#pragma unroll
    for (int i = 0; i < 2; ++i)
#pragma unroll
      for (int r = 0; r < 16; ++r) acc[i][0][r] = 0.f;
    if (!(p.debug & 8)) compute_half(std::integral_constant<int, 0>{});
    if (p.debug & 1) { t0 = __builtin_readcyclecounter(); t_c0 += t0 - t1; }
    asm volatile("s_waitcnt vmcnt(0)\n\ts_barrier" ::: "memory");
    if (p.debug & 1) { t1 = __builtin_readcyclecounter(); t_w2 += t1 - t0; }
    const int next = slot + p.wg_per_block;
    if (next < n_mt && !(p.debug & 4)) issue_half(next, 0);
    if (!(p.debug & 8)) compute_half(std::integral_constant<int, 1>{});
    if (p.debug & 1) { t0 = __builtin_readcyclecounter(); t_c1 += t0 - t1; }
    if (wave_has_cols && !(p.debug & 2)) gemm_epilogue_lean<2, 1, ACT, DROP, BWD, AUX, false, BWD>(d, acc, d.C, 0, row0, col0, 0, wn0, l31, h, d.M, d.N);
    if (p.debug & 1) { t1 = __builtin_readcyclecounter(); t_epi += t1 - t0; }
    ++n_done;
  }
  if ((p.debug & 1) && d.sk_ws && tid == 0 && blockIdx.x < 1024) {
    long long* o = reinterpret_cast<long long*>(reinterpret_cast<char*>(d.sk_ws) + d.sk_ws_bytes - 65536) + blockIdx.x * 8;
    const long long t_end = __builtin_readcyclecounter();
    o[0] = t_end - t_start; o[1] = t_loop - t_start; o[2] = t_w1; o[3] = t_w2; o[4] = t_c0; o[5] = t_c1; o[6] = t_epi; o[7] = n_done;
  }
}

template <int KB, bool B_KC, int ACT, bool DROP, bool BWD, bool AUX>
int ws_launch(const ctts_gemm_desc& d, const WsArgs& p, hipStream_t st) {
  const size_t lds = (size_t)64 * KB * 32 * sizeof(float);
  (void)hipFuncSetAttribute(reinterpret_cast<const void*>(gemm_ws_kernel<KB, B_KC, ACT, DROP, BWD, AUX>),
                            hipFuncAttributeMaxDynamicSharedMemorySize, (int)lds);
  hipLaunchKernelGGL((gemm_ws_kernel<KB, B_KC, ACT, DROP, BWD, AUX>), dim3(p.n_blocks * p.wg_per_block), dim3(256), lds, st, d, p);
  CTTS_CHECK_LAUNCH("ctts_gemm(weight-stationary)");
  return 1;
}

template <int KB, bool B_KC, int ACT>
int ws_launch_act(const ctts_gemm_desc& d, const WsArgs& p, hipStream_t st) {
  const bool drop = d.p_drop > 0.f;
  if (d.epi_bwd)
    return drop ? ws_launch<KB, B_KC, ACT, true, true, ACT != 0>(d, p, st) : ws_launch<KB, B_KC, ACT, false, true, ACT != 0>(d, p, st);
  if (d.R) return drop ? ws_launch<KB, B_KC, ACT, true, false, true>(d, p, st) : ws_launch<KB, B_KC, ACT, false, false, true>(d, p, st);
  return drop ? ws_launch<KB, B_KC, ACT, true, false, false>(d, p, st) : ws_launch<KB, B_KC, ACT, false, false, false>(d, p, st);
}

template <int KB, bool B_KC>
int ws_launch_layout(const ctts_gemm_desc& d, const WsArgs& p, hipStream_t st) {
  switch (d.act) {
    case 0: return ws_launch_act<KB, B_KC, 0>(d, p, st);
    case 1: return ws_launch_act<KB, B_KC, 1>(d, p, st);
    case 2: return ws_launch_act<KB, B_KC, 2>(d, p, st);
    case 4: return ws_launch_act<KB, B_KC, 4>(d, p, st);
    default: return 0;
  }
}

int ws_env(const char* name, int dflt) {
  const char* v = getenv(name);
  return v ? atoi(v) : dflt;
}

}

static int g_ws_enabled = -1;

extern "C" int ctts_gemm_ws_enable(int on) {
  const int prev = g_ws_enabled < 0 ? ws_env("CTTS_WS", 1) : g_ws_enabled;
  g_ws_enabled = on ? 1 : 0;
  return prev;
}

static bool ws_plan(const ctts_gemm_desc& d, WsArgs& p) {
  if (g_ws_enabled < 0) g_ws_enabled = ws_env("CTTS_WS", 1) ? 1 : 0;
  static const int min_rows = ws_env("CTTS_WS_MIN_ROWS", 4096);
  static const int slots = ws_env("CTTS_WS_SLOTS", 512);
  static const int align = ws_env("CTTS_WS_XCD_ALIGN", 1);
  static const int debug = ws_env("CTTS_WS_DEBUG", 0);
  if (!g_ws_enabled) return false;
  if (d.nb0 * d.nb1 != 1 || (d.lens && (d.lim_m || d.lim_n || d.lim_k)) || d.E || d.split_k > 1 || d.conv_T > 0) return false;
  if (!d.a_kc || d.K != 256) return false;
  if (d.M < min_rows || d.N < 64) return false;
  auto al16 = [](const void* q) { return (reinterpret_cast<uintptr_t>(q) & 15) == 0; };
  if (!al16(d.A) || !al16(d.B) || ((d.lda | d.ldb) & 3)) return false;
  if ((long)(d.M + 64) * d.lda * 4 >= 0x7FFF0000L) return false;
  if (!gemm_fits32(d.C, d.M, d.ldc, d.N) || !gemm_fits32(d.Z, d.M, d.ldz, d.N) || !gemm_fits32(d.R, d.M, d.ldr, d.N)) return false;
  if (d.row_lens && !d.tile_map) return false;
  if (d.C_planes && (!d.epi_bwd || (d.ldc & 31) || (d.N & 31) || !al16(d.C_planes) || (long)(d.M + 64) * d.ldc * 6 >= 0x7FFF0000L)) return false;
  if (d.rowscale || d.act == 3 || (d.Z && !d.act && !d.epi_bwd)) return false;
  if (d.tile_map == reinterpret_cast<const int32_t*>(1)) return false;
  p.tiles_m = (d.M + 63) / 64;
  p.n_blocks = (d.N + 127) / 128;
  if (p.n_blocks > slots) return false;
  int per = slots / p.n_blocks;
  if (per > p.tiles_m) per = p.tiles_m;
  const int rounds = (p.tiles_m + per - 1) / per;
  const int per8 = 8 * ((slots / 8) / p.n_blocks);
  p.xcd_aligned = 0;
  if (align && per8 >= 8 && per8 <= p.tiles_m && (p.tiles_m + per8 - 1) / per8 <= rounds) { per = per8; p.xcd_aligned = 1; }
  p.wg_per_block = per;
  p.debug = debug;
  return true;
}

int ctts_gemm_ws_try(const ctts_gemm_desc& d, hipStream_t st) {
  WsArgs p;
  if (!ws_plan(d, p)) return 0;
  return d.b_kc ? ws_launch_layout<8, true>(d, p, st) : ws_launch_layout<8, false>(d, p, st);
}

extern "C" int ctts_gemm_takes_weight_stationary(const ctts_gemm_desc* dp) {
  if (!dp) return 0;
  ctts_gemm_desc d = *dp;
  if (d.nb0 < 1) d.nb0 = 1;
  if (d.nb1 < 1) d.nb1 = 1;
  WsArgs p;
  return ws_plan(d, p) ? 1 : 0;
}
```

### comprehensive-transformer-tts_amd/kernels.py

```python
import ctypes as C

import torch

from . import _lib
from ._lib import GemmDesc

ACT_NONE, ACT_RELU, ACT_GELU, ACT_TANH, ACT_SWISH = 0, 1, 2, 3, 4


def _stream():
    return C.c_void_p(torch.cuda.current_stream().cuda_stream)


def _p(t, offset=0):
    if t is None:
        return None
    if not t.is_cuda:
        raise _lib.CttsError("ctts kernels need device (HIP) tensors; got a CPU tensor - no CPU fallback exists")
    return t.data_ptr() + offset * t.element_size()


def _f32c(t, name):
    if t.dtype != torch.float32 or not t.is_contiguous():
        raise _lib.CttsError(f"{name}: expected contiguous float32 tensor, got {t.dtype} contiguous={t.is_contiguous()}")
# ... 32 lines not shown
SK_ENABLED = _os.environ.get("CTTS_SK", "1") != "0"
BF16_SPLIT = 0 if _os.environ.get("CTTS_X6", "1") == "0" else 1
PLW_ENABLED = _os.environ.get("CTTS_PLW", "1") != "0"
PLANES_ENABLED = _os.environ.get("CTTS_PL", "1") != "0"
PLANES_MIN_UNITS = int(_os.environ.get("CTTS_PL_MIN_UNITS", "4096"))
PLANES_MIN_TILES = int(_os.environ.get("CTTS_PL_MIN_TILES", "64"))
_SK_WS = {}


def gemm_workspace(device):
    key = (device.index if device.index is not None else torch.cuda.current_device(), torch.cuda.current_stream().cuda_stream)
    ws = _SK_WS.get(key)
    if ws is None:
        if SK_ENABLED and not torch.cuda.is_current_stream_capturing():
            check_xcd_dispatch(device)
        ws = torch.zeros(_lib.load().ctts_workspace_bytes(), dtype=torch.uint8, device=device)
        _SK_WS[key] = ws
    return ws


_XCD_OK = {}


def check_xcd_dispatch(device):
    global SK_ENABLED
    idx = device.index if device.index is not None else torch.cuda.current_device()
    if idx in _XCD_OK:
        return _XCD_OK[idx]
    out = torch.full((64,), -1, dtype=torch.int32, device=device)
    _lib.check(_lib.load().ctts_xcd_probe(_p(out), 64, _stream()), "ctts_xcd_probe")
    got = out.cpu().tolist()
    ok = got == [b % 8 for b in range(64)]
    _XCD_OK[idx] = ok
    if not ok:
        import warnings
        SK_ENABLED = False
        warnings.warn(f"ctts_amd: workgroups are not dispatched round-robin over 8 XCDs on cuda:{idx} (XCC_ID of workgroups 0..15: {got[:16]}) - "
                      "not the SPX partition mode; the persistent stream-K GEMM is disabled, the tile kernels take its launches")
    return ok


workspace = gemm_workspace


def _ws(t):
    return gemm_workspace(t.device).data_ptr()


class WorkspaceErrorProbe:

    def __init__(self):
        self._pending = []

    def poll(self):
        lib = _lib.load()
        self._pending = []
        for ws in list(_SK_WS.values()):
            off = lib.ctts_workspace_error_word(C.c_void_p(ws.data_ptr())) - ws.data_ptr()
            host = torch.empty(4, dtype=torch.uint8, pin_memory=True)
            with torch.cuda.device(ws.device):
                host.copy_(ws[off:off + 4], non_blocking=True)
                ev = torch.cuda.Event()
                ev.record()
            self._pending.append((ws, host, ev))

    def check(self):
        bad = []
        for ws, host, ev in self._pending:
            ev.synchronize()
            word = int(host.view(torch.int32)[0])
            if word != 0:
                bad.append((ws, word))
        self._pending = []
        for ws, word in bad:
            torch.cuda.synchronize(ws.device)
            ws.zero_()
        if bad:
            raise _lib.CttsError("stream-K GEMM hand-off failed: an owner workgroup gave up waiting for workgroup "
                                 f"{bad[0][1] - 1}'s partial tile - the results of that launch are invalid (workspace re-zeroed)")

    def poll_and_check(self):
        self.poll()
        self.check()


class PartialSink:

    FLUSH_BYTES = int(float(_os.environ.get("CTTS_DEFER_FLUSH_MB", "256")) * (1 << 20))

    def __init__(self):
        self.tasks = []
        self.keep = []
        self.pending = 0
        self.streams = []

    def add(self, src, count, stride, n, dst, alpha, src_off=0, dst_off=0):
        d0 = dst.data_ptr() + 4 * int(dst_off)
        if any(d0 < t[1] + 4 * t[2] and t[1] < d0 + 4 * int(n) for t in self.tasks):
            self.flush()
        self.tasks.append((src.data_ptr() + 4 * int(src_off), d0, int(n), int(stride), int(count), float(alpha)))
        self.keep.append((src, dst))
        if src.is_cuda:
            st = torch.cuda.current_stream(src.device)
            if st not in self.streams:
                self.streams.append(st)
        self.pending += 4 * int(count) * int(n)
        if self.FLUSH_BYTES and self.pending >= self.FLUSH_BYTES:
            self.flush()

    def flush(self):
        if not self.tasks:
            return
        arr = (_lib.PsumTask * len(self.tasks))()
        for t, (src, dst, n, stride, count, alpha) in zip(arr, self.tasks):
            t.src, t.dst, t.n, t.stride, t.count, t.alpha = src, dst, n, stride, count, alpha
        self.tasks = []
        self.pending = 0
        producers, self.streams = self.streams, []
        try:
            cur = torch.cuda.current_stream()
            for st in producers:
                if st != cur:
                    cur.wait_stream(st)
            _lib.check(_lib.load().ctts_partial_sums(arr, len(arr), _stream()), "ctts_partial_sums")
            for src, _ in self.keep:
                if src.is_cuda:
                    src.record_stream(cur)
        finally:
            self.keep = []


WEIGHTS_EPOCH = [0]

_SINK = None
DEFER_ENABLED = _os.environ.get("CTTS_DEFER_SUMS", "1") != "0"


def set_partial_sink(sink):
    global _SINK
    prev, _SINK = _SINK, (sink if DEFER_ENABLED else None)
    return prev


def _sink_for(dst):
    if _SINK is None or dst is None or not dst.is_contiguous():
        return None
    return _SINK


def _gemm_desc(A, B, Cout, M, N, K, lda, ldb, ldc, a_kc=True, b_kc=True, a_off=0, b_off=0, c_off=0, nb0=1, nb1=1,
               sA=(0, 0), sB=(0, 0), sC=(0, 0), lens=None, lim=(0, 0, 0), conv=None, conv_on_b=False, split_k=1, alpha=1.0,
               bias=None, Z=None, ldz=0, act=ACT_NONE, p_drop=0.0, seed=None, drop_offset=0, R=None, ldr=0, rowscale=None,
               row_lens=None, row_T=0, row_halo=0, tile_map=None, E=None, rowsub=None, use_sk=None, epi_bwd=False, split_overwrite=False,
               bf16_split=None, a_planes=None, b_planes=None, c_planes=None):
    d = GemmDesc()
    if c_planes is not None:
        d.C_planes = c_planes.data_ptr()
    d.bf16_split = int(BF16_SPLIT if bf16_split is None else bf16_split)
    if a_planes is not None and b_planes is not None:
        d.A_planes, d.B_planes = a_planes.data_ptr(), b_planes.data_ptr()
    d.A, d.B, d.C = _p(A, a_off), _p(B, b_off), _p(Cout, c_off)
    d.M, d.N, d.K = int(M), int(N), int(K)
    d.lda, d.ldb, d.ldc = int(lda), int(ldb), int(ldc)
    d.a_kc, d.b_kc = int(a_kc), int(b_kc)
    d.nb0, d.nb1 = int(nb0), int(nb1)
    d.sA0, d.sA1 = int(sA[0]), int(sA[1])
    d.sB0, d.sB1 = int(sB[0]), int(sB[1])
    d.sC0, d.sC1 = int(sC[0]), int(sC[1])
    d.lens = _p(lens)
    d.lim_m, d.lim_n, d.lim_k = int(lim[0]), int(lim[1]), int(lim[2])
    if conv is not None:
        d.conv_T, d.conv_pad, d.conv_cin = int(conv[0]), int(conv[1]), int(conv[2])
        d.conv_on_b = int(conv_on_b)
    d.split_k = int(split_k)
    d.alpha = float(alpha)
    d.bias = _p(bias)
    d.Z, d.ldz = _p(Z), int(ldz)
    d.act = int(act)
    d.p_drop = float(p_drop)
    d.seed = _p(seed)
    d.drop_offset = int(drop_offset)
    d.R, d.ldr = _p(R), int(ldr)
    d.rowscale = _p(rowscale)
    if row_lens is not None:
        d.row_lens, d.row_T, d.row_halo = _p(row_lens), int(row_T), int(row_halo)
        d.tile_map = _p(tile_map)
    d.E, d.rowsub = _p(E), _p(rowsub)
    d.epi_bwd = int(bool(epi_bwd))
    d.split_overwrite = int(bool(split_overwrite))
    if int(split_k) > 1 or a_planes is not None or ((SK_ENABLED if use_sk is None else use_sk) and nb0 * nb1 == 1 and M * N * K >= (1 << 24)):
        ws = gemm_workspace(A.device)
        d.sk_ws, d.sk_ws_bytes = ws.data_ptr(), ws.numel()
    return d


def gemm(A, B, Cout, M, N, K, lda, ldb, ldc, a_kc=True, b_kc=True, defer=False, **kw):
    d = _gemm_desc(A, B, Cout, M, N, K, lda, ldb, ldc, a_kc, b_kc, **kw)
    lib = _lib.load()
    if defer and _SINK is not None and d.split_k > 1 and d.nb0 * d.nb1 == 1 and ldc == N and N % 4 == 0:
        cnt, stride = C.c_int32(0), C.c_int64(0)
        if lib.ctts_gemm_split_plan(C.byref(d), C.byref(cnt), C.byref(stride)) == 1:
            P = torch.empty(d.split_k * stride.value, dtype=torch.float32, device=A.device)
            d.split_out, d.split_out_floats = P.data_ptr(), P.numel()
            _lib.check(lib.ctts_gemm(C.byref(d), _stream()), "ctts_gemm")
            _SINK.add(P, cnt.value, stride.value, M * N, Cout, d.alpha, dst_off=kw.get("c_off", 0))
            return Cout
    _lib.check(lib.ctts_gemm(C.byref(d), _stream()), "ctts_gemm")
    return Cout


def gemm_takes_persistent(A, B, Cout, M, N, K, lda, ldb, ldc, a_kc=True, b_kc=True, **kw):
    if not SK_ENABLED:
        return False
    d = _gemm_desc(A, B, Cout, M, N, K, lda, ldb, ldc, a_kc, b_kc, **kw)
    return bool(_lib.load().ctts_gemm_takes_persistent(C.byref(d)))


def gemm_takes_bf16_split(A, B, Cout, M, N, K, lda, ldb, ldc, a_kc=True, b_kc=True, **kw):
    d = _gemm_desc(A, B, Cout, M, N, K, lda, ldb, ldc, a_kc, b_kc, **kw)
    return bool(_lib.load().ctts_gemm_takes_bf16_split(C.byref(d)))


def gemm_bf16_split_enable(on):
    global BF16_SPLIT
    prev = BF16_SPLIT
    BF16_SPLIT = 3 if on == "amp" else (int(on) if on in (2, 3, 4) else int(bool(on)))
    return prev


def amp_split():
    if BF16_SPLIT < 1:
        return None
    return 4 if BF16_SPLIT in (2, 4) else 3


def gemm_takes_planes(A, B, Cout, M, N, K, lda, ldb, ldc, a_kc=True, b_kc=True, **kw):
    d = _gemm_desc(A, B, Cout, M, N, K, lda, ldb, ldc, a_kc, b_kc, **kw)
    return bool(_lib.load().ctts_gemm_takes_planes(C.byref(d)))


def plane_shape_ok(M, N, K, conv_cin=None):
    if not PLANES_ENABLED or BF16_SPLIT < 1 or not SK_ENABLED:
        return False
    if K % 32 or K < 64 or N % 128 or N < 256 or M < 128:
        return False
    if conv_cin is not None and (conv_cin % 32 or K % conv_cin):
        return False
    tiles = -(-M // 128) * -(-N // 256)
    return BF16_SPLIT in (2, 4) or (tiles * (K // 32) >= PLANES_MIN_UNITS and tiles >= PLANES_MIN_TILES)


def plane_wgrad_shape_ok(Mo, No, Kred, cin=None):
    if not PLANES_ENABLED or not PLW_ENABLED or BF16_SPLIT < 1 or not SK_ENABLED:
        return False
    if Mo % 128 or No % 256 or Kred < 64:
        return False
    if cin is not None and (cin % 256 or No % cin):
        return False
    tiles = (Mo // 128) * (No // 256)
    return BF16_SPLIT in (2, 4) or (tiles >= 32 and tiles * (-(-Kred // 32)) >= PLANES_MIN_UNITS)


def split_planes(mats):
    if not mats:
        return []
    outs = []
    arr = (_lib.SplitTask * len(mats))()
    for t, m in zip(arr, mats):
        _f32c(m, "split_planes operand")
        rows, cols = m.shape
        if cols % 32:
            raise _lib.CttsError(f"split_planes: cols = {cols} is not a multiple of 32")
        o = torch.empty(rows, cols // 32, 3, 32, dtype=torch.bfloat16, device=m.device)
        outs.append(o)
        t.src, t.dst, t.rows, t.cols, t.ld = _p(m), o.data_ptr(), int(rows), int(cols), int(cols)
    _lib.check(_lib.load().ctts_split_planes(arr, len(arr), _stream()), "ctts_split_planes")
    return outs


PRODUCER_PLANES = _os.environ.get("CTTS_PRODUCER_PLANES", "1") != "0"


def _al16(*ts):
    return all(t.data_ptr() % 16 == 0 for t in ts)


def new_planes(rows, cols, device):
    return torch.empty(rows, cols // 32, 3, 32, dtype=torch.bfloat16, device=device)


def attach_planes(t, pl):
    t._ctts_planes = (pl, t.data_ptr(), t._version, t.numel())
    return t


def planes_of(t):
    ent = getattr(t, "_ctts_planes", None)
    if ent is None:
        return None
    pl, ptr, ver, n = ent
    if ptr != t.data_ptr() or ver != t._version or n != t.numel() or pl.numel() != 3 * n:
        return None
    return pl


def planes_piece(pl, q):
    return pl[:, :, q, :].reshape(pl.shape[0], -1)


def gemm_takes_weight_stationary(A, B, Cout, M, N, K, lda, ldb, ldc, a_kc=True, b_kc=True, **kw):
    d = _gemm_desc(A, B, Cout, M, N, K, lda, ldb, ldc, a_kc, b_kc, **kw)
    return bool(_lib.load().ctts_gemm_takes_weight_stationary(C.byref(d)))


def gemm_ws_enable(on):
    return bool(_lib.load().ctts_gemm_ws_enable(1 if on else 0))


def row_tile_map(row_lens, row_T, row_halo, M):
    tm = torch.empty(1 + (M + 63) // 64, dtype=torch.int32, device=row_lens.device)
    lib = _lib.load()
    _lib.check(lib.ctts_row_tile_map(_p(row_lens), int(row_T), int(row_halo), int(M), _p(tm), _stream()), "ctts_row_tile_map")
    return tm


def conv_dgrad_weights(weights):
    if not weights:
        return []
    outs = [torch.empty(cin, k * cout, dtype=torch.float32, device=w.device) for w, cout, cin, k in weights]
    arr = (_lib.RepackTask * len(weights))()
    for t, (w, cout, cin, k), o in zip(arr, weights, outs):
        t.src, t.dst, t.cout, t.cin, t.k = _p(_f32c(w, "conv weight (GEMM-major)")), _p(o), int(cout), int(cin), int(k)
    _lib.check(_lib.load().ctts_conv_dgrad_weights(arr, len(arr), _stream()), "ctts_conv_dgrad_weights")
    return outs


def conv_weight_repack(src, dst, cout, cin, k, mode):
    lib = _lib.load()
    _lib.check(lib.ctts_conv_weight_repack(_p(src), _p(dst), cout, cin, k, mode, _stream()), "ctts_conv_weight_repack")
    return dst


def lr_index(dur, Tm, pad=None, round_mode=0, want_mel2ph=True):
    B, Ts = dur.shape
    is_float = dur.dtype == torch.float32
    if not is_float and dur.dtype != torch.int64:
        raise _lib.CttsError(f"lr_index: durations must be int64 or float32, got {dur.dtype}")
    dur = dur.contiguous()
    mel2ph = torch.empty(B, Tm, dtype=torch.int32, device=dur.device) if want_mel2ph else None
    mel_len = torch.empty(B, dtype=torch.int64, device=dur.device)
    cum = torch.empty(B, Ts, dtype=torch.int32, device=dur.device)
    padp = None
    if pad is not None:
        pad = pad.to(torch.uint8).contiguous()
        padp = _p(pad)
    lib = _lib.load()
    _lib.check(lib.ctts_lr_index(_p(dur), int(is_float), int(round_mode), padp, B, Ts, int(Tm), _p(mel2ph), _p(mel_len),
                                 _p(cum), _stream()), "ctts_lr_index")
    return mel2ph, mel_len, cum


def lr_gather_fwd(x, mel2ph):
    B, Ts, Cc = x.shape
    Tm = mel2ph.shape[1]
    out = torch.empty(B, Tm, Cc, dtype=torch.float32, device=x.device)
    lib = _lib.load()
    _lib.check(lib.ctts_lr_gather_fwd(_p(_f32c(x, "x")), _p(mel2ph), _p(out), B, Ts, Tm, Cc, _stream()), "ctts_lr_gather_fwd")
    return out


def lr_gather_bwd(dy, cum, Ts):
    B, Tm, Cc = dy.shape
    dx = torch.empty(B, Ts, Cc, dtype=torch.float32, device=dy.device)
    lib = _lib.load()
    _lib.check(lib.ctts_lr_gather_bwd(_p(_f32c(dy, "dy")), _p(cum), _p(dx), B, Ts, Tm, Cc, _stream()), "ctts_lr_gather_bwd")
    return dx


def positions(src, stride=1):
    B, T = src.shape[0], src.shape[1]
    pos = torch.empty(B, T, dtype=torch.int32, device=src.device)
    is_float = src.dtype == torch.float32
    lib = _lib.load()
    _lib.check(lib.ctts_positions(_p(src), int(is_float), int(stride), B, T, _p(pos), _stream()), "ctts_positions")
    return pos


def cwt_pitch(spec, f0_mean, f0_std, std_scale, eps, mel_min, mel_max, f0_bin, uv=None, uv_chan=-1, nscale=10, width=None):
    spec = _f32c(spec, "cwt_pitch spec")
    B, T, ld = spec.shape
    width = T if width is None else int(width)
    f0 = torch.empty(B, width, dtype=torch.float32, device=spec.device)
    den = torch.empty_like(f0)
    ids = torch.empty(B, width, dtype=torch.int64, device=spec.device)
    if uv is not None:
        uv = _f32c(uv if uv.dtype == torch.float32 else uv.float(), "cwt_pitch uv")
        if tuple(uv.shape) != (B, width):
            raise _lib.CttsError(f"cwt_pitch: uv has shape {tuple(uv.shape)}, expected {(B, width)}")
    f0_mean, f0_std = _f32c(f0_mean.contiguous(), "f0_mean"), _f32c(f0_std.contiguous(), "f0_std")
    _lib.check(_lib.load().ctts_cwt_pitch(_p(spec), ld, int(nscale), _p(f0_mean), _p(f0_std), float(std_scale),
                                          _p(uv), int(uv_chan), float(eps), float(mel_min), float(mel_max), int(f0_bin), _p(f0), _p(den), _p(ids),
                                          B, T, width, _stream()), "ctts_cwt_pitch")
    return f0, den, ids


def layernorm_fwd(x, gamma, beta, eps, p_drop=0.0, seed=None, drop_offset=0, rowscale=None, want_planes=False):
    Cc = x.shape[-1]
    rows = x.numel() // Cc
    y = torch.empty_like(x)
    mean = torch.empty(rows, dtype=torch.float32, device=x.device)
    rstd = torch.empty(rows, dtype=torch.float32, device=x.device)
    pl = new_planes(rows, Cc, x.device) if (want_planes and PRODUCER_PLANES and Cc % 32 == 0 and x.is_cuda) else None
    lib = _lib.load()
    _lib.check(lib.ctts_layernorm_fwd(_p(_f32c(x, "x")), _p(gamma), _p(beta), _p(y), _p(mean), _p(rstd), rows, Cc, eps,
                                      p_drop, _p(seed), drop_offset, _p(rowscale), _p(pl), _stream()), "ctts_layernorm_fwd")
    if pl is not None:
        attach_planes(y, pl)
    return y, mean, rstd


def layernorm_bwd(dy, x, gamma, mean, rstd, p_drop=0.0, seed=None, drop_offset=0, rowscale=None, acc_into=None, dres=None):
    Cc = x.shape[-1]
    rows = x.numel() // Cc
    dx = torch.empty_like(x)
    if acc_into is None:
        dgamma = torch.empty(Cc, dtype=torch.float32, device=x.device)
        dbeta = torch.empty(Cc, dtype=torch.float32, device=x.device)
    else:
        dgamma, dbeta = acc_into
    lib = _lib.load()
    sink = _sink_for(dgamma) if (acc_into is not None and dbeta.is_contiguous()) else None
    nparts = lib.ctts_reduce_parts(3, rows, Cc) if sink is not None else 0
    if nparts > 1:
        parts = torch.empty(nparts, 2 * Cc, dtype=torch.float32, device=x.device)
        _lib.check(lib.ctts_layernorm_bwd(_p(_f32c(dy, "dy")), _p(x), _p(gamma), _p(mean), _p(rstd), _p(dx), None, None, rows, Cc, p_drop,
                                          _p(seed), drop_offset, _p(rowscale), 1, _p(dres), None, _p(parts), _stream()), "ctts_layernorm_bwd")
        sink.add(parts, nparts, 2 * Cc, Cc, dgamma, 1.0)
        sink.add(parts, nparts, 2 * Cc, Cc, dbeta, 1.0, src_off=Cc)
        return dx, dgamma, dbeta
    _lib.check(lib.ctts_layernorm_bwd(_p(_f32c(dy, "dy")), _p(x), _p(gamma), _p(mean), _p(rstd), _p(dx), _p(dgamma),
                                      _p(dbeta), rows, Cc, p_drop, _p(seed), drop_offset, _p(rowscale), int(acc_into is not None),
                                      _p(dres), _ws(dy), None, _stream()), "ctts_layernorm_bwd")
    return dx, dgamma, dbeta


def colstats(x2d):
    rows, Cc = x2d.shape
    sums = torch.empty(2 * Cc, dtype=torch.float64, device=x2d.device)
    lib = _lib.load()
    _lib.check(lib.ctts_colstats(_p(_f32c(x2d, "x")), _p(sums), rows, Cc, _ws(x2d), _stream()), "ctts_colstats")
    return sums


def bn_batch_stats(x2d, eps, momentum, running_mean, running_var, num_batches):
    rows, Cc = x2d.shape
    sums = colstats(x2d)
    mean = torch.empty(Cc, dtype=torch.float32, device=x2d.device)
    rstd = torch.empty_like(mean)
    lib = _lib.load()
    _lib.check(lib.ctts_bn_finalize(_p(sums), rows, Cc, float(eps), float(momentum), _p(mean), _p(rstd), _p(running_mean),
                                    _p(running_var), _p(num_batches), _stream()), "ctts_bn_finalize")
    return mean, rstd


def bn_apply(x2d, mean, rstd, gamma, beta, act, p_drop=0.0, seed=None, drop_offset=0, want_planes=False):
    rows, Cc = x2d.shape
    y = torch.empty_like(x2d)
    pl = (new_planes(rows, Cc, x2d.device) if (want_planes and PRODUCER_PLANES and Cc % 32 == 0 and x2d.is_cuda and rows > 0
                                               and _al16(x2d, mean, rstd, gamma, beta)) else None)
    lib = _lib.load()
    _lib.check(lib.ctts_bn_apply(_p(_f32c(x2d, "x")), _p(mean), _p(rstd), _p(gamma), _p(beta), _p(y), rows, Cc, act, p_drop,
                                 _p(seed), drop_offset, _p(pl), _stream()), "ctts_bn_apply")
    return (y, pl) if want_planes else y


def bn_bwd(dy, x2d, mean, rstd, gamma, beta, act, p_drop, seed, drop_offset, batch_stats, acc_into=None, want_planes=False):
    rows, Cc = x2d.shape
    pl = (new_planes(rows, Cc, x2d.device) if (want_planes and PRODUCER_PLANES and Cc % 32 == 0 and x2d.is_cuda and rows > 0
                                               and _al16(dy, x2d, mean, rstd, gamma, beta)) else None)
    sums = torch.empty(2 * Cc, dtype=torch.float64, device=x2d.device)
    dx = torch.empty_like(x2d)
    if acc_into is not None:
        dgamma, dbeta = _f32c(acc_into[0], "dgamma"), _f32c(acc_into[1], "dbeta")
        batch_stats = int(batch_stats) | 2
    else:
        dgamma = torch.empty(Cc, dtype=torch.float32, device=x2d.device)
# ... 1010 lines not shown
```

### comprehensive-transformer-tts_amd/ops.py

```python
import math

import torch

from . import kernels as K
from .kernels import ACT_NONE, ACT_RELU, ACT_GELU, ACT_TANH, ACT_SWISH


_FUSE_GRAD_ACCUM = False


def set_grad_accumulation_fusion(flag):
    global _FUSE_GRAD_ACCUM
    _FUSE_GRAD_ACCUM = bool(flag)


def grad_accumulation_fusion():
    return _FUSE_GRAD_ACCUM


def _grad_of(p):
    if not _FUSE_GRAD_ACCUM or p is None or not p.requires_grad:
        return None
    if p.is_leaf:
        g = p.grad
        if g is None or g.dtype != torch.float32 or not (g.is_contiguous() or g.stride() == p.stride()):
            return None
        return g
    base = p._base
    if (base is None or not base.is_leaf or base.grad is None or base.grad.dtype != torch.float32 or p.numel() != base.numel()
            or not p.is_contiguous()):
        return None
    if base.is_contiguous() and base.grad.is_contiguous():
        return base.grad.view(p.shape)
    g = base.grad
    dense = sum((n - 1) * st for n, st in zip(base.shape, base.stride())) + 1 == base.numel()
    if dense and g.stride() == base.stride() and p.data_ptr() == base.data_ptr():
        return torch.as_strided(g, p.shape, p.stride(), g.storage_offset())
    return None


def _fusable(p):
    return _grad_of(p) is not None


_CUTS = None


class CutRecorder:

    def __init__(self, names):
        self.names = list(names)
        self.pairs = {}

    def __enter__(self):
        global _CUTS
        assert _CUTS is None, "CutRecorder is not re-entrant"
        _CUTS = self
        self.pairs = {}
        return self

    def __exit__(self, *exc):
        global _CUTS
        _CUTS = None
        return False

    def backward_stages(self, loss):
        missing = [n for n in self.names if n not in self.pairs]
        if missing:
            raise RuntimeError(f"staged backward: the forward never reached the cut point(s) {missing}")
        loss.backward()
        yield 0
        for s, name in enumerate(self.names, 1):
            xs, gs = [], []
            for x, leaf in self.pairs[name]:
                g, leaf.grad = leaf.grad, None
                if g is not None:
                    xs.append(x)
                    gs.append(g)
            if not xs:
                raise RuntimeError(f"staged backward: no gradient arrived at cut '{name}'")
            torch.autograd.backward(xs, gs)
            yield s
        self.pairs = {}


def stage_cut(x, name):
    rec = _CUTS
    if rec is None or name not in rec.names or not x.requires_grad:
        return x
    leaf = x.detach().requires_grad_(True)
    rec.pairs.setdefault(name, []).append((x, leaf))
    return leaf


def stage_cut_tree(obj, name):
    rec = _CUTS
    if rec is None or name not in rec.names:
        return obj

    def walk(o):
        if torch.is_tensor(o):
            return stage_cut(o, name) if (o.requires_grad and o.is_floating_point()) else o
        if isinstance(o, dict):
            new = {k: walk(v) for k, v in o.items()}
            return new if any(new[k] is not o[k] for k in o) else o
        if isinstance(o, (tuple, list)):
            new = [walk(v) for v in o]
            if all(a is b for a, b in zip(new, o)):
                return o
            return type(o)(new)
        return o
    return walk(obj)


def _gemm_major(w):
    if w.dim() != 3:
        return None
    N, Cin, k = w.shape
    if w.stride() == (k * Cin, 1, Cin) or (k == 1 and w.is_contiguous()):
        return w.permute(0, 2, 1).view(N, k * Cin)
    return None


_WGRAD = {"stream": None, "keep": [], "main": None, "max_rows": None}


def set_wgrad_stream(stream, max_rows=None):
    _WGRAD["stream"] = stream
    _WGRAD["max_rows"] = max_rows


def _wgrad_join():
    side, main = _WGRAD["stream"], _WGRAD["main"]
    if side is not None and main is not None:
        main.wait_stream(side)
    _WGRAD["keep"].clear()
    _WGRAD["main"] = None


class _OnWgradStream:
    def __init__(self, *operands):
        self.operands = operands

    def __enter__(self):
        side = _WGRAD["stream"]
        cur = torch.cuda.current_stream()
        if _WGRAD["main"] is None:
            _WGRAD["main"] = cur
            torch.autograd.Variable._execution_engine.queue_callback(_wgrad_join)
        side.wait_stream(cur)
        _WGRAD["keep"].extend(self.operands)
        self.ctx = torch.cuda.stream(side)
        self.ctx.__enter__()

    def __exit__(self, *exc):
        return self.ctx.__exit__(*exc)


class _Inline:
    def __enter__(self):
        return None

    def __exit__(self, *exc):
        return False


def _wgrad_scope(fused, *operands, rows=None):
    if not fused or _WGRAD["stream"] is None:
        return _Inline()
    if _WGRAD["max_rows"] is not None and rows is not None and rows > _WGRAD["max_rows"]:
        return _Inline()
    return _OnWgradStream(*operands)


import os as _os
_DGRAD_SPLIT_K = int(_os.environ.get("CTTS_DGRAD_SPLIT_K", "1"))
_FUSE_EPILOGUE_BWD = _os.environ.get("CTTS_FUSE_EPI_BWD", "1") != "0"
_WGRAD_SPLIT_MULT = float(_os.environ.get("CTTS_WGRAD_SPLIT_MULT", "1"))
_WGRAD_SPLIT_CAP = int(_os.environ.get("CTTS_WGRAD_SPLIT_CAP", "512"))


def _split_k_for(Mo, No, Kred):
    forced = int(_os.environ.get("CTTS_WGRAD_SPLIT", "0"))
    t128 = ((Mo + 127) // 128) * ((No + 127) // 128)
    if forced and t128 >= 64:
        return forced
    want = max(1, int(-(-512 // t128) * _WGRAD_SPLIT_MULT))
    return int(max(1, min(want, max(1, Kred // _WGRAD_SPLIT_CAP))))


class EpiLink:

    def __init__(self):
        self.Z = self.seed = None
        self.act, self.p_drop, self.drop_offset = ACT_NONE, 0.0, 0
        self.conv_dims = None
        self.armed = False
        self.gen = 0
        self.done = set()

    def arm(self, Z, act, p_drop, seed, drop_offset, conv_dims=None):
        self.Z, self.act, self.p_drop, self.seed, self.drop_offset = Z, act, p_drop, seed, drop_offset
        self.conv_dims = conv_dims
        self.gen += 1
        self.armed = True
        return self.gen

    def take(self):
        self.armed = False
        return (self.Z, self.act, self.p_drop, self.seed, self.drop_offset, self.gen, self.conv_dims)


class _LinearConv(torch.autograd.Function):

    @staticmethod
    def forward(ctx, x, w, b, residual, rowscale, act, alpha, p_drop, seed, drop_offset, ksize, row_lens, row_T, pr=None, link=None,
                link_role=0, pad_left=None):
        x = x.contiguous()
        Cin = x.shape[-1]
        M = x.numel() // Cin
        N = w.shape[0]
        out = torch.empty(*x.shape[:-1], N, dtype=torch.float32, device=x.device)
        Z = torch.empty_like(out) if act != ACT_NONE else None
        if ksize:
            T = x.shape[-2]
            wf = _gemm_major(w)
            if wf is None:
                wf = torch.empty(N, ksize * Cin, dtype=torch.float32, device=x.device)
                K.conv_weight_repack(w.contiguous(), wf, N, Cin, ksize, 0)
            ctx.pad_left = (ksize - 1) // 2 if pad_left is None else int(pad_left)
            conv = (T, ctx.pad_left, Cin)
            Kdim = ksize * Cin
        else:
            wf, conv, Kdim = w.contiguous(), None, Cin
        if residual is not None:
            residual = residual.contiguous()
        gk = dict(conv=conv, alpha=alpha, bias=b, Z=Z, ldz=N, act=act, p_drop=p_drop, seed=seed, drop_offset=drop_offset, R=residual, ldr=N,
                  rowscale=rowscale, row_lens=row_lens, row_T=row_T, row_halo=0)
        ctx.amp = (K.amp_split() if (ksize and x.is_cuda and torch.is_autocast_enabled("cuda")) else None)
        if ctx.amp is not None:
            gk["bf16_split"] = ctx.amp
        planes = _operand_planes("fwd", w, x.view(M, Cin), wf, M, N, Kdim, Cin, Kdim, N, out, gk, a_given=K.planes_of(x)) if ksize else {}
        K.gemm(x, wf, out, M, N, Kdim, Cin, Kdim, N, True, True, tile_map=pr.tile_map(0, M) if (pr is not None and not planes) else None,
               **gk, **planes)
        ctx.x_planes = planes.get("a_planes")
        ctx.save_for_backward(x, w, Z, rowscale, seed, row_lens, b)
        ctx.cfg = (act, alpha, p_drop, drop_offset, ksize, b is not None, residual is not None, row_T)
        ctx.pr = pr
        ctx.link, ctx.link_role, ctx.link_snap = None, 0, None
        if link is not None and _FUSE_EPILOGUE_BWD:
            if link_role == 1 and rowscale is None and residual is None and (act != ACT_NONE or p_drop > 0):
                ctx.link_gen = link.arm(Z, act, p_drop, seed, drop_offset, conv_dims=(Cin, ksize) if ksize else None)
                ctx.link, ctx.link_role = link, 1
            elif link_role == 2 and link.armed and not ksize:
                ctx.link, ctx.link_role, ctx.link_snap = link, 2, link.take()
        return out

    @staticmethod
    def backward(ctx, dY):
        x, w, Z, rowscale, seed, row_lens, b = ctx.saved_tensors
        act, alpha, p_drop, drop_offset, ksize, has_bias, has_res, row_T = ctx.cfg
        rl = dict(row_lens=row_lens, row_T=row_T) if row_lens is not None else {}
        if getattr(ctx, "amp", None) is not None:
            rl["bf16_split"] = ctx.amp
        pr = ctx.pr
        kmap = pr.tile_map(0, x.numel() // x.shape[-1]) if (pr is not None and row_lens is not None) else None
        dY = dY.contiguous()
        Cin = x.shape[-1]
        M = x.numel() // Cin
        N = w.shape[0]
        dX = dW = dB = None
        want_bias = has_bias and ctx.needs_input_grad[2]
        fuse_bias = want_bias and _fusable(b)
        if ctx.link_role == 1 and ctx.link_gen in ctx.link.done:
            ctx.link.done.discard(ctx.link_gen)
            dZ, d_res = dY, None
            if want_bias:
                if fuse_bias:
                    K.colsum(dZ.view(M, N), scale=alpha, acc_into=_grad_of(b))
                else:
                    dB = K.colsum(dZ.view(M, N), scale=alpha)
        elif rowscale is None and act == ACT_NONE and p_drop == 0:
            dZ, d_res = dY, (dY if has_res else None)
            if want_bias:
                if fuse_bias:
                    K.colsum(dZ.view(M, N), scale=alpha, acc_into=_grad_of(b))
                else:
                    dB = K.colsum(dZ.view(M, N), scale=alpha)
        else:
            dZ, gm, dBn = K.epilogue_bwd(dY, rowscale, Z, act, p_drop, seed, drop_offset, want_gm=has_res and rowscale is not None,
                                         want_bias=want_bias, bias_scale=alpha, bias_acc_into=_grad_of(b) if fuse_bias else None)
            d_res = (gm if rowscale is not None else dY) if has_res else None
            if want_bias and not fuse_bias:
                dB = dBn
        dz_planes = K.planes_of(dZ) if ksize else None
        if ksize:
            T = x.shape[-2]
            pad = ctx.pad_left
            pad_d = ksize - 1 - pad
            if ctx.needs_input_grad[0]:
                wd = _DGRAD_W.take(w, (Cin, ksize * N))
                if wd is None:
                    wd = torch.empty(Cin, ksize * N, dtype=torch.float32, device=x.device)
                    wmaj = _gemm_major(w)
                    if wmaj is not None:
                        K.conv_weight_repack(wmaj, wd, N, Cin, ksize, 4)
                    else:
                        K.conv_weight_repack(w.contiguous(), wd, N, Cin, ksize, 1)
                tiles = -(-M // 64) * -(-Cin // 64)
                sk = min(4, max(2, -(-2304 // tiles))) if (_DGRAD_SPLIT_K and tiles < 1536 and ksize * N >= 4096) else 1
                dX = torch.empty_like(x)
                dg0 = dict(conv=(T, pad_d, N), alpha=alpha, row_halo=pad_d, **rl)
                planes = _operand_planes("dgrad", w, dZ.view(M, N), wd, M, Cin, ksize * N, N, ksize * N, Cin, dX, dict(split_overwrite=True, **dg0),
                                         a_given=dz_planes)
                if planes:
                    dz_planes = planes["a_planes"]
                    K.gemm(dZ, wd, dX, M, Cin, ksize * N, N, ksize * N, Cin, True, True, split_k=1, split_overwrite=True, **dg0, **planes)
                else:
                    dg = dict(tile_map=pr.tile_map(pad_d, M) if pr is not None else None, **dg0)
                    if sk > 1 and K.gemm_takes_persistent(dZ, wd, x, M, Cin, ksize * N, N, ksize * N, Cin, True, True, split_k=1, **dg):
                        sk = 1
                    K.gemm(dZ, wd, dX, M, Cin, ksize * N, N, ksize * N, Cin, True, True, split_k=sk, split_overwrite=True, **dg)
            if ctx.needs_input_grad[1]:
                Kd = ksize * Cin
                fused = _fusable(w)
                gmaj = _gemm_major(_grad_of(w)) if fused else None
                wk = dict(conv=(T, pad, Cin), conv_on_b=True, split_k=max(2, _split_k_for(N, Kd, M)), alpha=alpha, **rl)
                if gmaj is not None:
                    wp = _wgrad_planes(dZ.view(M, N), x.view(M, Cin), dz_planes, getattr(ctx, "x_planes", None), gmaj, N, Kd, M, Cin, wk)
                    with _wgrad_scope(True, dZ, x, *wp.values(), rows=M):
                        K.gemm(dZ, x, gmaj, N, Kd, M, N, Cin, Kd, False, False, tile_map=kmap, defer=_WGRAD["stream"] is None, **wk, **wp)
                else:
                    dwf = torch.empty(N, Kd, dtype=torch.float32, device=x.device)
                    wk["split_overwrite"] = True
                    wp = _wgrad_planes(dZ.view(M, N), x.view(M, Cin), dz_planes, getattr(ctx, "x_planes", None), dwf, N, Kd, M, Cin, wk)
                    with _wgrad_scope(fused, dZ, x, dwf, *wp.values(), rows=M):
                        K.gemm(dZ, x, dwf, N, Kd, M, N, Cin, Kd, False, False, tile_map=kmap, **wk, **wp)
                        if fused:
                            K.conv_weight_repack(dwf, _grad_of(w), N, Cin, ksize, 3)
                        elif _gemm_major(w) is not None:
                            dW = dwf.view(N, ksize, Cin).permute(0, 2, 1)
                        else:
                            dW = torch.empty_like(w)
                            K.conv_weight_repack(dwf, dW, N, Cin, ksize, 2)
        else:
            if ctx.needs_input_grad[0]:
                dX = torch.empty_like(x)
                if ctx.link_role == 2:
                    lZ, lact, lp, lseed, loff, lgen, lconv = ctx.link_snap
                    gk = dict(alpha=alpha, epi_bwd=True, Z=lZ, ldz=Cin, act=lact, p_drop=lp, seed=lseed, drop_offset=loff,
                              tile_map=pr.tile_map(0, M) if pr is not None else None, **rl)
                    cpl = None
                    if (lconv is not None and K.PRODUCER_PLANES and dZ.is_cuda and Cin % 32 == 0
                            and K.plane_shape_ok(M, lconv[0], lconv[1] * Cin, Cin)):
                        cand = K.new_planes(M, Cin, dZ.device)
                        if K.gemm_takes_weight_stationary(dZ, w, dX, M, Cin, N, N, Cin, Cin, True, False, c_planes=cand, **gk):
                            cpl = cand
                    K.gemm(dZ, w, dX, M, Cin, N, N, Cin, Cin, True, False, c_planes=cpl, **gk)
                    if cpl is not None:
                        K.attach_planes(dX, cpl)
                    ctx.link.done.add(lgen)
                else:
                    K.gemm(dZ, w, dX, M, Cin, N, N, Cin, Cin, True, False, alpha=alpha,
                           tile_map=pr.tile_map(0, M) if pr is not None else None, **rl)
            if ctx.needs_input_grad[1] and N == 1 and row_lens is None:
                fused = _fusable(w)
                got = K.weighted_colsum(x.view(M, Cin), dZ.reshape(M), scale=alpha, acc_into=_grad_of(w).view(-1) if fused else None)
                dW = None if fused else got.view(1, Cin)
            elif ctx.needs_input_grad[1]:
                fused = _fusable(w)
                dW = _grad_of(w) if fused else torch.empty_like(w)
                with _wgrad_scope(fused, dZ, x, rows=M):
                    K.gemm(dZ, x, dW, N, Cin, M, N, Cin, Cin, False, False, split_k=max(2, _split_k_for(N, Cin, M)), alpha=alpha,
                           tile_map=kmap, defer=fused and _WGRAD["stream"] is None, split_overwrite=not fused, **rl)
                if fused:
                    dW = None
        return dX, dW, dB, d_res, None, None, None, None, None, None, None, None, None, None, None, None, None




def _wstamp(w):
    return (w._version, K.WEIGHTS_EPOCH[0])


class _DgradCache(dict):

    def take(self, w, shape):
        ent = dict.pop(self, w.data_ptr(), None)
        if ent is None or ent[1] != _wstamp(w) or tuple(ent[0].shape) != tuple(shape):
            return None
        return ent[0]


_DGRAD_W = _DgradCache()

_PLANES = {"fwd": {}, "dgrad": {}, "want_fwd": set(), "want_dgrad": set()}


def _operand_planes(kind, w, a_mat, b_mat, M, N, Kdim, lda, ldb, ldc, out, gk, a_given=None):
    conv = gk.get("conv")
    if not K.plane_shape_ok(M, N, Kdim, conv[2] if conv is not None else None):
        return {}
    if not (a_mat.is_contiguous() and b_mat.is_contiguous() and a_mat.shape[1] % 32 == 0 and b_mat.shape[1] % 32 == 0):
        return {}
    if not K.gemm_takes_planes(a_mat, b_mat, out, M, N, Kdim, lda, ldb, ldc, True, True, a_planes=_FakePlanes(a_mat), b_planes=_FakePlanes(b_mat), **gk):
        return {}
    ent = _PLANES[kind].get(w.data_ptr())
    if ent is not None and ent[1] == _wstamp(w) and ent[0].numel() == 3 * b_mat.numel():
        bp = ent[0]
    else:
        _PLANES["want_" + kind].add(w.data_ptr())
        bp = K.split_planes([b_mat])[0]
    return dict(a_planes=a_given if a_given is not None else K.split_planes([a_mat])[0], b_planes=bp)


def _wgrad_planes(dz_mat, x_mat, dz_pl, x_pl, out, Mo, No, Kred, cin, kw):
    if not K.plane_wgrad_shape_ok(Mo, No, Kred, cin) or not (dz_mat.is_contiguous() and x_mat.is_contiguous()):
        return {}
    a = dz_pl if dz_pl is not None else _FakePlanes(dz_mat)
    b = x_pl if x_pl is not None else _FakePlanes(x_mat)
    if not K.gemm_takes_planes(dz_mat, x_mat, out, Mo, No, Kred, Mo, cin, No, False, False, a_planes=a, b_planes=b, **kw):
        return {}
    made = iter(K.split_planes([m for m, pl in ((dz_mat, dz_pl), (x_mat, x_pl)) if pl is None]))
    return dict(a_planes=dz_pl if dz_pl is not None else next(made), b_planes=x_pl if x_pl is not None else next(made))


class _FakePlanes:

    def __init__(self, mat):
        self._m = mat

    def data_ptr(self):
        return self._m.data_ptr()


def prepare_dgrad_weights(params):
    clear_dgrad_weights()
    params = list(params)
    live = {w.data_ptr() for w in params}
    _PLANES["want_fwd"] &= live
    _PLANES["want_dgrad"] &= live
    todo = []
    for w in params:
        wm = _gemm_major(w) if w.dim() == 3 else None
        if wm is not None and w.requires_grad:
            N, Cin, k = w.shape
            todo.append((w, (wm.detach(), N, Cin, k)))
    mats, slots = [], []
    for (w, (wm, _, _, _)), wd in zip(todo, K.conv_dgrad_weights([t for _, t in todo])):
        _DGRAD_W[w.data_ptr()] = (wd, _wstamp(w))
        if w.data_ptr() in _PLANES["want_fwd"]:
            mats.append(wm.contiguous()); slots.append(("fwd", w))
        if w.data_ptr() in _PLANES["want_dgrad"]:
            mats.append(wd); slots.append(("dgrad", w))
    for (kind, w), pl in zip(slots, K.split_planes(mats)):
        _PLANES[kind][w.data_ptr()] = (pl, _wstamp(w))


def clear_dgrad_weights():
    _DGRAD_W.clear()
    _PLANES["fwd"].clear()
    _PLANES["dgrad"].clear()


class PadRows:

    def __init__(self, lens, T):
        self.lens, self.T = lens, int(T)
        self._maps = {}

    def tile_map(self, halo, M):
        key = (int(halo), int(M))
        if key not in self._maps:
            self._maps[key] = K.row_tile_map(self.lens, self.T, halo, M)
        return self._maps[key]


def _pad_rows(pad_rows):
    if pad_rows is None:
        return None, 0, None
    if isinstance(pad_rows, PadRows):
        return pad_rows.lens, pad_rows.T, pad_rows
    return pad_rows[0], int(pad_rows[1]), PadRows(pad_rows[0], pad_rows[1])


def linear(x, w, b=None, act=ACT_NONE, alpha=1.0, residual=None, rowscale=None, p_drop=0.0, drop=None, pad_rows=None, link=None,
           link_role=0):
    seed, off = (drop.seed, drop.next_offset()) if (drop is not None and p_drop > 0) else (None, 0)
    rl, rT, pr = _pad_rows(pad_rows)
    return _LinearConv.apply(x, w, b, residual, rowscale, act, alpha, p_drop if seed is not None else 0.0, seed, off, 0, rl, rT, pr,
                             link, link_role)


def conv1d(x, w, b=None, act=ACT_NONE, alpha=1.0, residual=None, rowscale=None, p_drop=0.0, drop=None, pad_rows=None, link=None,
           link_role=0, padding="SAME"):
    seed, off = (drop.seed, drop.next_offset()) if (drop is not None and p_drop > 0) else (None, 0)
    rl, rT, pr = _pad_rows(pad_rows)
    if padding not in ("SAME", "LEFT"):
        raise ValueError(f"conv1d: padding '{padding}' (SAME or LEFT)")
    k = w.shape[2]
    return _LinearConv.apply(x, w, b, residual, rowscale, act, alpha, p_drop if seed is not None else 0.0, seed, off,
                             k, rl, rT, pr, link, link_role, (k - 1) if padding == "LEFT" else (k - 1) // 2)


def _adjacent(ts):
    if any((not t.is_contiguous()) or t.dtype != torch.float32 for t in ts):
        return False
    try:
        st = ts[0].untyped_storage().data_ptr()
        if any(t.untyped_storage().data_ptr() != st for t in ts):
            return False
    except Exception:
        return False
    return all(b.data_ptr() == a.data_ptr() + a.numel() * 4 for a, b in zip(ts, ts[1:]))


class _PackedLinear(torch.autograd.Function):

    @staticmethod
    def forward(ctx, x, *ws):
        x = x.contiguous()
        Kd = x.shape[-1]
        M = x.numel() // Kd
        sizes = [w.shape[0] for w in ws]
        N = sum(sizes)
        wd = [w.detach() for w in ws]
        W = torch.as_strided(wd[0], (N, Kd), (Kd, 1)) if _adjacent(wd) else torch.cat(wd, 0)
        out = torch.empty(*x.shape[:-1], N, dtype=torch.float32, device=x.device)
        K.gemm(x, W, out, M, N, Kd, Kd, Kd, N, True, True)
        ctx.save_for_backward(x, *ws)
        ctx.sizes = sizes
        return out

    @staticmethod
    def backward(ctx, dY):
        x, ws = ctx.saved_tensors[0], ctx.saved_tensors[1:]
        dY = dY.contiguous()
        Kd = x.shape[-1]
        M = x.numel() // Kd
        N = sum(ctx.sizes)
        wd = [w.detach() for w in ws]
        W = torch.as_strided(wd[0], (N, Kd), (Kd, 1)) if _adjacent(wd) else torch.cat(wd, 0)
        dX = None
        if ctx.needs_input_grad[0]:
            dX = torch.empty_like(x)
            K.gemm(dY, W, dX, M, Kd, N, N, Kd, Kd, True, False)
        gs = [_grad_of(w) for w in ws]
        sk = max(2, _split_k_for(N, Kd, M))
        if all(g is not None for g in gs) and _adjacent(gs):
            G = torch.as_strided(gs[0], (N, Kd), (Kd, 1))
            K.gemm(dY, x, G, N, Kd, M, N, Kd, Kd, False, False, split_k=sk, defer=_WGRAD["stream"] is None)
            return (dX,) + (None,) * len(ws)
        dW = torch.empty(N, Kd, dtype=torch.float32, device=x.device)
        K.gemm(dY, x, dW, N, Kd, M, N, Kd, Kd, False, False, split_k=sk, split_overwrite=True)
        return (dX,) + tuple(dW.split(ctx.sizes, 0))


def linear_packed(x, weights):
    return _PackedLinear.apply(x, *weights)


class _LayerNorm(torch.autograd.Function):
    @staticmethod
    def forward(ctx, x, gamma, beta, eps, rowscale, p_drop, seed, drop_offset):
        x = x.contiguous()
        y, mean, rstd = K.layernorm_fwd(x, gamma, beta, eps, p_drop, seed, drop_offset, rowscale)
        ctx.save_for_backward(x, gamma, mean, rstd, rowscale, seed, beta)
        ctx.cfg = (p_drop, drop_offset)
        return y

    @staticmethod
    def backward(ctx, dy):
        x, gamma, mean, rstd, rowscale, seed, beta = ctx.saved_tensors
        p_drop, drop_offset = ctx.cfg
        if _fusable(gamma) and _fusable(beta):
            dx, _, _ = K.layernorm_bwd(dy.contiguous(), x, gamma, mean, rstd, p_drop, seed, drop_offset, rowscale,
                                       acc_into=(gamma.grad, beta.grad))
            return dx, None, None, None, None, None, None, None
        dx, dg, db = K.layernorm_bwd(dy.contiguous(), x, gamma, mean, rstd, p_drop, seed, drop_offset, rowscale)
        return dx, dg, db, None, None, None, None, None


class _LayerNormRes(torch.autograd.Function):

    @staticmethod
    def forward(ctx, x, gamma, beta, eps, want_planes=False):
        x = x.contiguous()
        y, mean, rstd = K.layernorm_fwd(x, gamma, beta, eps, 0.0, None, 0, None, want_planes=want_planes)
        ctx.save_for_backward(x, gamma, mean, rstd, beta)
        return y, x.view_as(x)

    @staticmethod
    def backward(ctx, dy, dres):
        x, gamma, mean, rstd, beta = ctx.saved_tensors
        if dy is None:
            return dres, None, None, None, None
        dres = dres.contiguous() if dres is not None else None
        if _fusable(gamma) and _fusable(beta):
            dx, _, _ = K.layernorm_bwd(dy.contiguous(), x, gamma, mean, rstd, acc_into=(gamma.grad, beta.grad), dres=dres)
            return dx, None, None, None, None
        dx, dg, db = K.layernorm_bwd(dy.contiguous(), x, gamma, mean, rstd, dres=dres)
        return dx, dg, db, None, None


def consumer_takes_planes(x, cout, ksize):
    Cc = x.shape[-1]
    return bool(x.is_cuda and K.PRODUCER_PLANES and K.plane_shape_ok(x.numel() // Cc, int(cout), int(ksize) * Cc, Cc))


# ... 966 lines not shown
```

### include/ctts.h

```cpp
#ifndef CTTS_H
#define CTTS_H
#include <stddef.h>
#include <stdint.h>

#ifdef __cplusplus
extern "C" {
#endif

const char* ctts_last_error(void);
int ctts_version(void);

typedef struct ctts_gemm_desc {
  const float* A; const float* B; float* C;
  int32_t M, N, K;
  int64_t lda, ldb, ldc;
  int32_t a_kc, b_kc;
  int32_t nb0, nb1;
  int64_t sA0, sA1, sB0, sB1, sC0, sC1;
  const int32_t* lens;
  int32_t lim_m, lim_n, lim_k;
  int32_t conv_T, conv_pad, conv_cin, conv_on_b;
  int32_t split_k;
  float alpha;
  const float* bias;
  float* Z; int64_t ldz;
  int32_t act;
  float p_drop; const uint64_t* seed; uint32_t drop_offset;
  const float* R; int64_t ldr;
  const float* rowscale;
  const int32_t* row_lens; int32_t row_T; int32_t row_halo;
  const int32_t* tile_map;
  int32_t tile_group_n;
  const float* E; const float* rowsub;
  void* sk_ws; int64_t sk_ws_bytes;
  int32_t epi_bwd;
  float* split_out; int64_t split_out_floats;
  int32_t split_overwrite;
  int32_t bf16_split;
  const uint16_t* A_planes;
  const uint16_t* B_planes;
  uint16_t* C_planes;
} ctts_gemm_desc;

int ctts_gemm(const ctts_gemm_desc* d, void* stream);
int ctts_gemm_split_plan(const ctts_gemm_desc* d, int32_t* count, int64_t* stride);
typedef struct ctts_repack_task { const float* src; float* dst; int32_t cout, cin, k; } ctts_repack_task;
int ctts_conv_dgrad_weights(const ctts_repack_task* tasks, int ntasks, void* stream);
int ctts_posembed_fwd(const float* x, const int32_t* pos, const float* table, const float* alpha, const float* rowscale, float* y,
                      int64_t rows, int C, float p_drop, const uint64_t* seed, uint32_t drop_offset, void* stream);
int ctts_posembed_bwd(const float* dy, const int32_t* pos, const float* table, const float* rowscale, float* dx, float* dalpha,
                      int64_t rows, int C, float p_drop, const uint64_t* seed, uint32_t drop_offset, int accumulate, void* ws, void* stream);
typedef struct ctts_psum_task { const float* src; float* dst; int64_t n; int64_t stride; int32_t count; float alpha; } ctts_psum_task;
int ctts_partial_sums(const ctts_psum_task* tasks, int ntasks, void* stream);
int ctts_reduce_parts(int kind, int64_t rows, int C);
size_t ctts_workspace_bytes(void);
size_t ctts_gemm_workspace_bytes(void);
const uint32_t* ctts_workspace_error_word(const void* ws);
int ctts_xcd_probe(int32_t* out, int nblocks, void* stream);
int ctts_gemm_takes_persistent(const ctts_gemm_desc* d);
int ctts_gemm_ws_enable(int on);
int ctts_gemm_takes_weight_stationary(const ctts_gemm_desc* d);
int ctts_gemm_takes_bf16_split(const ctts_gemm_desc* d);
int ctts_gemm_takes_planes(const ctts_gemm_desc* d);
typedef struct ctts_split_task { const float* src; uint16_t* dst; int64_t rows, cols, ld; } ctts_split_task;
int ctts_split_planes(const ctts_split_task* tasks, int ntasks, void* stream);

int ctts_rowdot_heads(const float* a, const float* b, float* out, int B, int T, int H, int dh, void* stream);

int ctts_weighted_colsum(const float* x, const float* w, float* out, int64_t rows, int C, float scale, int accumulate, void* ws, float* parts,
                         void* stream);

int ctts_epilogue_bwd(const float* dy, const float* rowscale, const float* z, float* dz, float* gm, float* dbias, int64_t rows, int C,
                      int act, float p_drop, const uint64_t* seed, uint32_t drop_offset, float bias_scale, int accumulate_bias,
                      void* ws, float* parts, void* stream);

int ctts_row_tile_map(const int32_t* row_lens, int row_T, int row_halo, int M, int32_t* tile_map, void* stream);

int ctts_conv_weight_repack(const float* src, float* dst, int cout, int cin, int k, int mode, void* stream);

int ctts_lr_index(const void* dur, int dur_is_float, int round_mode, const uint8_t* pad, int B, int Ts, int Tm,
                  int32_t* mel2ph, int64_t* mel_len, int32_t* cum, void* stream);
int ctts_lr_gather_fwd(const float* x, const int32_t* mel2ph, float* out, int B, int Ts, int Tm, int C, void* stream);
int ctts_lr_gather_bwd(const float* dy, const int32_t* cum, float* dx, int B, int Ts, int Tm, int C, void* stream);

int ctts_cwt_pitch(const float* spec, int64_t ld_spec, int nscale, const float* f0_mean, const float* f0_std, float std_scale,
                   const float* uv, int uv_chan, float eps, float mel_min, float mel_max, int f0_bin, float* f0, float* f0_denorm,
                   int64_t* ids, int B, int T, int width, void* stream);

int ctts_positions(const void* src, int src_is_float, int64_t stride, int B, int T, int32_t* pos, void* stream);

int ctts_layernorm_fwd(const float* x, const float* gamma, const float* beta, float* y, float* mean, float* rstd,
                       int rows, int C, float eps, float p_drop, const uint64_t* seed, uint32_t drop_offset,
                       const float* rowscale, uint16_t* planes, void* stream);
int ctts_layernorm_bwd(const float* dy, const float* x, const float* gamma, const float* mean, const float* rstd,
                       float* dx, float* dgamma, float* dbeta, int rows, int C, float p_drop, const uint64_t* seed,
                       uint32_t drop_offset, const float* rowscale, int accumulate, const float* dres, void* ws, float* parts,
                       void* stream);

int ctts_colstats(const float* x, double* sums, int rows, int C, void* ws, void* stream);
int ctts_bn_finalize(const double* sums, int rows, int C, float eps, float momentum, float* mean, float* rstd, float* running_mean,
                     float* running_var, int64_t* num_batches, void* stream);
int ctts_bn_apply(const float* x, const float* mean, const float* rstd, const float* gamma, const float* beta,
                  float* y, int rows, int C, int act, float p_drop, const uint64_t* seed, uint32_t drop_offset,
                  uint16_t* planes , void* stream);
int ctts_bn_bwd_reduce(const float* dy, const float* x, const float* mean, const float* rstd, const float* gamma,
                       const float* beta, double* sums, int rows, int C, int act, float p_drop, const uint64_t* seed,
                       uint32_t drop_offset, void* ws, void* stream);
int ctts_bn_bwd_apply(const float* dy, const float* x, const float* mean, const float* rstd, const float* gamma,
                      const float* beta, const double* sums, float* dx, float* dgamma, float* dbeta, int rows, int C,
                      int act, float p_drop, const uint64_t* seed, uint32_t drop_offset, int batch_stats,
                      uint16_t* planes , void* stream);

int ctts_softmax_fwd(float* S, const int32_t* lens, int nb0, int nb1, int T, int64_t ld, void* stream);
int ctts_softmax_bwd(const float* P, float* dP, const int32_t* lens, int nb0, int nb1, int T, int64_t ld,
                     void* stream);

int ctts_act_dropout_bwd(const float* dg, const float* z, float* dz, int64_t rows, int C, int act, float alpha_unused,
                         float p_drop, const uint64_t* seed, uint32_t drop_offset, void* stream);
int ctts_rowscale_dropout(const float* x, float* y, int64_t rows, int C, const float* rowscale, float p_drop,
                          const uint64_t* seed, uint32_t drop_offset, void* stream);
int ctts_colsum(const float* x, float* out, int64_t rows, int C, int64_t ld, float scale, int accumulate, void* ws, float* parts, void* stream);

int ctts_reflect_pad(const float* y, float* ypad, int B, int N, int pad, int64_t ld_out, void* stream);
int ctts_stft_magnitude(const float* reim, int64_t ld_reim, float* mag, int64_t ld_mag, float* energy, int64_t frames,
                        int nbins, void* stream);
int ctts_log_clamp_transpose(const float* mel_fm, float* out, int B, int F, int n_mel, float clip, void* stream);

int ctts_relattn_split_fwd(const float* qkv, const float* u_bias, const float* v_bias, float* qu, float* qv, float* kv, int64_t rows,
                           int C, void* stream);
int ctts_relattn_split_bwd(const float* dqu, const float* dqv, const float* dkv, float* dqkv, int64_t rows, int C, void* stream);
int ctts_glu_fwd(const float* a, float* out, int64_t rows, int C, void* stream);
int ctts_glu_bwd(const float* a, const float* dout, float* da, int64_t rows, int C, void* stream);
int ctts_dwconv_fwd(const float* x, const float* wT, float* y, int B, int T, int C, int K, int flip, void* stream);
int ctts_dwconv_wgrad(const float* dy, const float* x, float* dw, float* partials, int B, int T, int C, int K, int accumulate,
                      void* stream);
int ctts_relpos_softmax_fwd(float* S, const float* PS, float* Pd, int nbatch, int T, float scale, float p_drop,
                            const uint64_t* seed, uint32_t drop_offset, void* stream);
int ctts_relpos_softmax_bwd(const float* P, float* dPd, int nbatch, int T, float scale, float p_drop, const uint64_t* seed,
                            uint32_t drop_offset, void* stream);
int ctts_relshift_bwd(const float* dS, float* dPS, int nbatch, int T, void* stream);

int ctts_embedding_fwd(const int64_t* ids, const float* weight, float* out, int64_t n, int C, int V, void* stream);
int ctts_embedding_bwd(const int64_t* ids, const float* dy, float* dweight, int64_t n, int C, int V, int padding_idx, int accumulate,
                       void* ws, void* stream);

int ctts_neg_sqdist(const float* q, const float* k, float* out, int B, int Tq, int Tk, int C, float temp, void* stream);
int ctts_mas(const float* attn, const int32_t* in_lens, const int32_t* out_lens, float* opt, float* dur, uint8_t* back, int B,
             int Tq, int Tk, void* stream);
int ctts_forward_sum_fwd(const float* attn_logprob, const int32_t* in_lens, const int32_t* out_lens, float blank_logprob, float* lse,
                         float* alpha, float* nll, int B, int Tq, int Tk, void* stream);
int ctts_forward_sum_bwd(const float* attn_logprob, const int32_t* in_lens, const int32_t* out_lens, float blank_logprob,
                         const float* lse, const float* alpha, const float* nll, const float* gscale, float* grad, int B, int Tq,
                         int Tk, void* stream);

int ctts_im2col_3x3s2(const float* x, float* col, int B, int T, int W, int C, void* stream);
int ctts_col2im_3x3s2(const float* dcol, float* dx, int B, int T, int W, int C, void* stream);
int ctts_gru_fwd(const float* gi, const float* whh, const float* bhh, float* out, float* gates, int B, int T, int H, int ndir,
                 int rev_mask, void* stream);
int ctts_gru_bwd(const float* dout, const float* out, const float* gates, const float* whh, float* dgi, float* dgh, float* hprev,
                 int B, int T, int H, int ndir, int rev_mask, void* stream);
int ctts_softmax_rect_fwd(float* S, const int32_t* klens, const int32_t* qlens, int nb, int Tq, int Tk, void* stream);
int ctts_softmax_rect_bwd(const float* P, float* dP, const int32_t* klens, const int32_t* qlens, int nb, int Tq, int Tk,
                          void* stream);

size_t ctts_mel_spectrogram_workspace_bytes(int n_fft, int n_mel);
int ctts_mel_prepare(const float* mel_basis, int n_fft, int n_mel, float* workspace, void* stream);
int ctts_mel_spectrogram(const float* y, const int32_t* lens, const float* window, const float* workspace, float* mel, float* energy, float* mag,
                         int64_t ld_mag, int B, int N, int n_fft, int hop, int n_mel, float clip, int kmax, uint32_t* range_flag,
                         void* stream);

int ctts_mha_supported(int C, int H);
int ctts_mha_fwd(const float* qkv, const int32_t* lens, float* out, float* lse, int B, int T, int H, int C, float scale, void* stream);
int ctts_mha_bwd(const float* qkv, const int32_t* lens, const float* out, const float* dout, const float* lse, float* Dws, float* dS,
                 float* kv_part, float* dqkv, int B, int T, int H, int C, float scale, int q_split, void* ws, void* stream);
size_t ctts_relmha_workspace_floats(int B, int T, int H);
int ctts_relmha_fwd(const float* qu, const float* qv, const float* kv, const float* pos, float* out, float* lse, int B, int T,
                    int H, int C, float scale, float p_drop, const uint64_t* seed, uint32_t drop_offset, void* stream);
int ctts_relmha_bwd(const float* qu, const float* qv, const float* kv, const float* pos, const float* out,
                    const float* dout, const float* lse, float* Dws, float* dS, float* dqu, float* dqv, float* dkv,
                    float* dpos_b, int B, int T, int H, int C, float scale, float p_drop, const uint64_t* seed, uint32_t drop_offset,
                    void* stream);

int ctts_var_loss_fwd(const float* log_d, const void* dur, int dur_is_float, const int64_t* texts, const uint8_t* src_pad, const float* cwt,
                      const float* cwt_spec, const float* uv, const uint8_t* mel_pad, const float* f0m_p, const float* f0m_t,
                      const float* f0s_p, const float* f0s_t, const float* e_pred, const float* e_tgt, int B, int Ts, int Tm,
                      const float* lambdas5, int cwt_l2, const int64_t* sil_ids3, float* partials, float* wsum, float* terms, float* denoms,
                      void* stream);
int ctts_var_loss_bwd(const float* log_d, const void* dur, int dur_is_float, const int64_t* texts, const uint8_t* src_pad, const float* cwt,
                      const float* cwt_spec, const float* uv, const uint8_t* mel_pad, const float* f0m_p, const float* f0m_t,
                      const float* f0s_p, const float* f0s_t, const float* e_pred, const float* e_tgt, int B, int Ts, int Tm,
                      const float* lambdas5, int cwt_l2, const int64_t* sil_ids3, const float* partials, const float* wsum,
                      const float* denoms, const float* g8, float* d_log_d, float* d_cwt, float* d_f0m, float* d_f0s, float* d_e,
                      void* stream);
int ctts_bin_loss_fwd(const float* soft, const float* hard, int64_t n, float* partials, float* out2, void* stream);
int ctts_bin_loss_bwd(const float* soft, const float* hard, const float* out2, const float* g, float* dsoft, int64_t n, void* stream);
int ctts_masked_loss_fwd(const float* pred, const float* target, const float* weight, int64_t n, int kind, float* partials, float* out2,
                         void* stream);
int ctts_masked_loss_bwd(const float* pred, const float* target, const float* weight, const float* out2, const float* g, float* dpred,
                         int64_t n, int kind, void* stream);

#define CTTS_ADAM_PARTIALS 2048
#define CTTS_ADAM_STATE_FLOATS (3 + CTTS_ADAM_PARTIALS)
int ctts_adam_clip_step(float* p, const float* g, float* m, float* v, int64_t n, const float* lr, float beta1, float beta2, float eps,
                        float weight_decay, float max_norm, float* state, void* stream);

int ctts_mel_l1_fwd(const float* p1, const float* p2, const float* tgt, const uint8_t* pad, float* sums, float* roww, int64_t rows,
                    int C, void* ws, void* stream);
int ctts_mel_l1_bwd(const float* p1, const float* p2, const float* tgt, const float* roww, const float* sums, const float* g, float* d1,
                    float* d2, int64_t rows, int C, void* stream);

typedef struct ctts_vconv_desc {
  const float* x;
  int64_t sxb, sxt, sxc;
  int32_t B, T, Cin, Cout, k, dil;
  int32_t transposed_u;
  int32_t act_in; float slope;
  const float* w; const uint16_t* w_planes;
  const float* bias;
// ... 85 lines not shown
```

Baseline: 688,700 mel-frames/s.

## Fuse bias column sums into dgrad GEMM epilogue, emit planes only, merge weight prep

```diff
diff --git a/comprehensive-transformer-tts_amd/_lib.py b/comprehensive-transformer-tts_amd/_lib.py
--- a/comprehensive-transformer-tts_amd/_lib.py
+++ b/comprehensive-transformer-tts_amd/_lib.py
@@ -39,6 +39,8 @@
         ("A_planes", _vp),
         ("B_planes", _vp),
         ("C_planes", _vp),
+        ("col_parts", _vp),
+        ("c_planes_only", _i32),
     ]
 
 
@@ -86,8 +88,13 @@
     _fields_ = [("src", _vp), ("dst", _vp), ("cout", _i32), ("cin", _i32), ("k", _i32)]
 
 
+class WprepTask(C.Structure):
+    _fields_ = [("src", _vp), ("wd", _vp), ("fwd_planes", _vp), ("dgrad_planes", _vp), ("cout", _i32), ("cin", _i32), ("k", _i32)]
+
+
 _SIGNATURES = {
     "ctts_conv_dgrad_weights": [C.POINTER(RepackTask), C.c_int, _vp],
+    "ctts_conv_weight_prepare": [C.POINTER(WprepTask), C.c_int, _vp],
     "ctts_gemm_split_plan": [C.POINTER(GemmDesc), C.POINTER(_i32), C.POINTER(_i64)],
     "ctts_partial_sums": [C.POINTER(PsumTask), C.c_int, _vp],
     "ctts_reduce_parts": [C.c_int, _i64, C.c_int],
@@ -98,6 +105,8 @@
     "ctts_gemm_takes_persistent": [C.POINTER(GemmDesc)],
     "ctts_gemm_ws_enable": [C.c_int],
     "ctts_gemm_takes_weight_stationary": [C.POINTER(GemmDesc)],
+    "ctts_gemm_col_parts_rows": [C.POINTER(GemmDesc)],
+    "ctts_join_planes": [_vp, _vp, _i64, _i64, _vp],
     "ctts_gemm_takes_bf16_split": [C.POINTER(GemmDesc)],
     "ctts_gemm_takes_planes": [C.POINTER(GemmDesc)],
     "ctts_split_planes": [C.POINTER(SplitTask), C.c_int, _vp],
diff --git a/comprehensive-transformer-tts_amd/csrc/elementwise.hip b/comprehensive-transformer-tts_amd/csrc/elementwise.hip
--- a/comprehensive-transformer-tts_amd/csrc/elementwise.hip
+++ b/comprehensive-transformer-tts_amd/csrc/elementwise.hip
@@ -1,4 +1,5 @@
 #include "ctts_common.h"
+#include "planes_common.h"
 
 namespace {
 __global__ void zero_u32_kernel(uint32_t* __restrict__ p, size_t n) {
@@ -456,6 +457,86 @@
 }
 
 namespace {
+struct PrepBatch {
+  const float* src[RPK_BATCH];
+  float* wd[RPK_BATCH];
+  uint16_t* fwd[RPK_BATCH];
+  uint16_t* dgr[RPK_BATCH];
+  int cout[RPK_BATCH], cin[RPK_BATCH], k[RPK_BATCH];
+  int first_block[RPK_BATCH + 1];
+  int ntasks;
+};
+
+__global__ __launch_bounds__(256) void conv_weight_prepare_kernel(const PrepBatch b) {
+  __shared__ float tile[32][33];
+  int t = 0;
+  while (t + 1 < b.ntasks && (int)blockIdx.x >= b.first_block[t + 1]) ++t;
+  const float* __restrict__ src = b.src[t];
+  float* __restrict__ wd = b.wd[t];
+  uint16_t* __restrict__ fwd = b.fwd[t];
+  uint16_t* __restrict__ dgr = b.dgr[t];
+  const int cout = b.cout[t], cin = b.cin[t], k = b.k[t];
+  const int tco = (cout + 31) / 32, tci = (cin + 31) / 32;
+  int blk = (int)blockIdx.x - b.first_block[t];
+  const int kk = blk / (tco * tci);
+  blk -= kk * tco * tci;
+  const int co0 = (blk / tci) * 32, ci0 = (blk % tci) * 32;
+  const int tx = threadIdx.x & 31, ty = threadIdx.x >> 5;
+#pragma unroll
+  for (int r = ty; r < 32; r += 8) {
+    const int co = co0 + r, ci = ci0 + tx;
+    tile[r][tx] = (co < cout && ci < cin) ? src[((long)co * k + (k - 1 - kk)) * cin + ci] : 0.f;
+  }
+  __syncthreads();
+  if (wd) {
+#pragma unroll
+    for (int r = ty; r < 32; r += 8) {
+      const int ci = ci0 + r, co = co0 + tx;
+      if (ci < cin && co < cout) wd[((long)ci * k + kk) * cout + co] = tile[tx][r];
+    }
+  }
+  const int pr = threadIdx.x >> 3, pc = (threadIdx.x & 7) * 4;
+  if (fwd && co0 + pr < cout) {
+    const float xs[4] = {tile[pr][pc], tile[pr][pc + 1], tile[pr][pc + 2], tile[pr][pc + 3]};
+    spl_store4(fwd, co0 + pr, (long)k * cin, (long)(k - 1 - kk) * cin + ci0 + pc, xs);
+  }
+  if (dgr && ci0 + pr < cin) {
+    const float xs[4] = {tile[pc][pr], tile[pc + 1][pr], tile[pc + 2][pr], tile[pc + 3][pr]};
+    spl_store4(dgr, ci0 + pr, (long)k * cout, (long)kk * cout + co0 + pc, xs);
+  }
+}
+}
+
+extern "C" int ctts_conv_weight_prepare(const ctts_wprep_task* tasks, int ntasks, void* stream) {
+  CTTS_REQUIRE(ntasks >= 0 && (tasks || ntasks == 0), "ctts_conv_weight_prepare: bad arguments");
+  hipStream_t st = (hipStream_t)stream;
+  for (int t0 = 0; t0 < ntasks; t0 += RPK_BATCH) {
+    PrepBatch b;
+    b.ntasks = 0;
+    int blocks = 0;
+    for (int t = t0; t < ntasks && t < t0 + RPK_BATCH; ++t) {
+      const ctts_wprep_task& q = tasks[t];
+      CTTS_REQUIRE(q.src && q.cout > 0 && q.cin > 0 && q.k > 0, "ctts_conv_weight_prepare: bad task %d", t);
+      CTTS_REQUIRE(!q.fwd_planes || (q.cin % 32 == 0 && (reinterpret_cast<uintptr_t>(q.fwd_planes) & 15) == 0),
+                   "ctts_conv_weight_prepare: task %d: forward planes need cin %% 32 == 0 and a 16-byte aligned set", t);
+      CTTS_REQUIRE(!q.dgrad_planes || (q.cout % 32 == 0 && (reinterpret_cast<uintptr_t>(q.dgrad_planes) & 15) == 0),
+                   "ctts_conv_weight_prepare: task %d: data-gradient planes need cout %% 32 == 0 and a 16-byte aligned set", t);
+      if (!q.wd && !q.fwd_planes && !q.dgrad_planes) continue;
+      const int i = b.ntasks++;
+      b.src[i] = q.src; b.wd[i] = q.wd; b.fwd[i] = q.fwd_planes; b.dgr[i] = q.dgrad_planes;
+      b.cout[i] = q.cout; b.cin[i] = q.cin; b.k[i] = q.k;
+      b.first_block[i] = blocks;
+      blocks += ((q.cout + 31) / 32) * ((q.cin + 31) / 32) * q.k;
+    }
+    if (b.ntasks == 0) continue;
+    b.first_block[b.ntasks] = blocks;
+    hipLaunchKernelGGL(conv_weight_prepare_kernel, dim3(blocks), dim3(256), 0, st, b);
+    CTTS_CHECK_LAUNCH("ctts_conv_weight_prepare");
+  }
+  return 0;
+}
+
+namespace {
 __global__ __launch_bounds__(256) void posembed_fwd_kernel(const float4* __restrict__ x, const int32_t* __restrict__ pos, const float4* __restrict__ table,
                                                             const float* __restrict__ alpha, const float* __restrict__ rowscale, float4* __restrict__ y,
                                                             long n4, int C4, float p_drop, const uint64_t* seed, uint32_t drop_offset) {
diff --git a/comprehensive-transformer-tts_amd/csrc/gemm_common.h b/comprehensive-transformer-tts_amd/csrc/gemm_common.h
--- a/comprehensive-transformer-tts_amd/csrc/gemm_common.h
+++ b/comprehensive-transformer-tts_amd/csrc/gemm_common.h
@@ -100,9 +100,10 @@
 
 template <int MT, int NT, int ACT, bool DROP, bool BWD, bool AUX, bool RS = false, bool PLANES = false>
 __device__ __forceinline__ void gemm_epilogue_lean(const ctts_gemm_desc& d, const floatx16 (&acc)[MT][NT], float* Cb, int z, int row0,
-                                                   int col0, int wm0, int wn0, int l31, int h, int Mv, int Nv) {
+                                                   int col0, int wm0, int wn0, int l31, int h, int Mv, int Nv, float* csum = nullptr) {
 #pragma clang fp contract(off)
   const bool planes_on = PLANES && d.C_planes != nullptr;
+  const bool c_on = !(planes_on && d.c_planes_only);
   const __amdgpu_buffer_rsrc_t rp = gemm_rsrc(d.C_planes, planes_on ? (long)Mv * d.ldc * 6 : 0);
   const unsigned p_row = (unsigned)(d.ldc * 6);
   const unsigned p_sel = (l31 & 1) ? 0x03020706u : 0x05040100u;
@@ -117,7 +118,7 @@
   const float* aux_p = BWD ? d.Z : d.R;
   const long aux_ld = BWD ? d.ldz : d.ldr;
   const bool has_z = !BWD && ACT && d.Z;
-  const __amdgpu_buffer_rsrc_t rc = gemm_rsrc(Cb, (last * d.ldc + Nv) * 4);
+  const __amdgpu_buffer_rsrc_t rc = gemm_rsrc(Cb, c_on ? (last * d.ldc + Nv) * 4 : 0);
   const __amdgpu_buffer_rsrc_t ra = gemm_rsrc(aux_p, AUX ? (last * aux_ld + Nv) * 4 : 0);
   const __amdgpu_buffer_rsrc_t rz = gemm_rsrc(d.Z, has_z ? (last * d.ldz + Nv) * 4 : 0);
   const __amdgpu_buffer_rsrc_t rr = gemm_rsrc(d.rowscale, RS ? (long)Mv * 4 : 0);
@@ -168,6 +169,7 @@
           if (RS) v *= rs[q];
         }
         __builtin_amdgcn_raw_buffer_store_b32(__builtin_bit_cast(unsigned, v), rc, c_lane + (unsigned)mu * c_row, 0, 0);
+        if (PLANES && csum) *csum += v;
         if (PLANES) aux[q] = v;
       }
       if (PLANES) {
diff --git a/comprehensive-transformer-tts_amd/csrc/gemm_pl.hip b/comprehensive-transformer-tts_amd/csrc/gemm_pl.hip
--- a/comprehensive-transformer-tts_amd/csrc/gemm_pl.hip
+++ b/comprehensive-transformer-tts_amd/csrc/gemm_pl.hip
@@ -426,6 +426,38 @@
   }
 }
 
+__global__ __launch_bounds__(256) void join_planes_kernel(const uint16_t* __restrict__ src, float* __restrict__ dst, long n8, long c8) {
+  const long gidx = (long)blockIdx.x * 256 + threadIdx.x;
+  if (gidx >= n8) return;
+  const long r = gidx / c8, c = (gidx - r * c8) * 8;
+  const uint16_t* o = src + r * c8 * 24 + (c >> 5) * 96 + (c & 31);
+  const spl_u32x4 ph = *reinterpret_cast<const spl_u32x4*>(o), pm = *reinterpret_cast<const spl_u32x4*>(o + 32),
+                  pq = *reinterpret_cast<const spl_u32x4*>(o + 64);
+  float xs[8];
+#pragma unroll
+  for (int e = 0; e < 8; ++e) {
+    const int sh = (e & 1) ? 0 : 16;
+    const float a = __uint_as_float((ph[e >> 1] << sh) & 0xFFFF0000u);
+    const float b = __uint_as_float((pm[e >> 1] << sh) & 0xFFFF0000u);
+    const float q = __uint_as_float((pq[e >> 1] << sh) & 0xFFFF0000u);
+    xs[e] = (__float_as_uint(b) | __float_as_uint(q)) << 1 ? (a + b) + q : a;
+  }
+  *reinterpret_cast<float4*>(dst + r * c8 * 8 + c) = make_float4(xs[0], xs[1], xs[2], xs[3]);
+  *reinterpret_cast<float4*>(dst + r * c8 * 8 + c + 4) = make_float4(xs[4], xs[5], xs[6], xs[7]);
+}
+
+}
+
+extern "C" int ctts_join_planes(const uint16_t* planes, float* dst, int64_t rows, int64_t cols, void* stream) {
+  CTTS_REQUIRE(planes && dst && rows >= 0 && cols >= 0 && cols % 32 == 0 && (reinterpret_cast<uintptr_t>(planes) & 15) == 0 &&
+                   (reinterpret_cast<uintptr_t>(dst) & 15) == 0,
+               "ctts_join_planes: needs 16-byte aligned pointers and cols %% 32 == 0");
+  const long n8 = rows * (cols / 8);
+  if (n8 == 0) return 0;
+  CTTS_REQUIRE((n8 + 255) / 256 < (1L << 31), "ctts_join_planes: too many elements in one call");
+  hipLaunchKernelGGL(join_planes_kernel, dim3((unsigned)((n8 + 255) / 256)), dim3(256), 0, (hipStream_t)stream, planes, dst, n8, cols / 8);
+  CTTS_CHECK_LAUNCH("ctts_join_planes");
+  return 0;
 }
 
 extern "C" int ctts_split_planes(const ctts_split_task* tasks, int ntasks, void* stream) {
diff --git a/comprehensive-transformer-tts_amd/csrc/gemm_ws.hip b/comprehensive-transformer-tts_amd/csrc/gemm_ws.hip
--- a/comprehensive-transformer-tts_amd/csrc/gemm_ws.hip
+++ b/comprehensive-transformer-tts_amd/csrc/gemm_ws.hip
@@ -55,6 +55,7 @@
   typedef const __attribute__((address_space(4))) int32_t* ws_cmap;
   const ws_cmap mmap = (ws_cmap)(uintptr_t)d.tile_map;
   const int n_mt = mmap ? mmap[0] : p.tiles_m;
+  const bool c_on = !(BWD && d.C_planes && d.c_planes_only);
   if (mmap) {
     const int n_zero = (p.tiles_m - n_mt) * p.n_blocks;
     for (int zt = blockIdx.x; zt < n_zero; zt += gridDim.x) {
@@ -64,7 +65,7 @@
       for (int e = tid; e < nrows * 128; e += 256) {
         const int r = e >> 7, c = e & 127;
         if (c < ncols) {
-          d.C[(long)(row0 + r) * d.ldc + c0 + c] = 0.f;
+          if (c_on) d.C[(long)(row0 + r) * d.ldc + c0 + c] = 0.f;
           if (d.Z && !d.epi_bwd) d.Z[(long)(row0 + r) * d.ldz + c0 + c] = 0.f;
         }
       }
@@ -152,6 +153,7 @@
   long long t_start = 0, t_loop = 0, t_w1 = 0, t_w2 = 0, t_epi = 0, t_c0 = 0, t_c1 = 0;
   if (p.debug & 1) t_start = __builtin_readcyclecounter();
   int n_done = 0;
+  float csum = 0.f;
   for (; slot < n_mt; slot += p.wg_per_block) {
     const int row0 = (mmap ? mmap[1 + slot] : slot) * 64;
     long long t0 = 0, t1 = 0;
@@ -172,9 +174,14 @@
     if (next < n_mt && !(p.debug & 4)) issue_half(next, 0);
     if (!(p.debug & 8)) compute_half(std::integral_constant<int, 1>{});
     if (p.debug & 1) { t0 = __builtin_readcyclecounter(); t_c1 += t0 - t1; }
-    if (wave_has_cols && !(p.debug & 2)) gemm_epilogue_lean<2, 1, ACT, DROP, BWD, AUX, false, BWD>(d, acc, d.C, 0, row0, col0, 0, wn0, l31, h, d.M, d.N);
+    if (wave_has_cols && !(p.debug & 2))
+      gemm_epilogue_lean<2, 1, ACT, DROP, BWD, AUX, false, BWD>(d, acc, d.C, 0, row0, col0, 0, wn0, l31, h, d.M, d.N, BWD ? &csum : nullptr);
     if (p.debug & 1) { t1 = __builtin_readcyclecounter(); t_epi += t1 - t0; }
     ++n_done;
+  }
+  if (BWD && d.col_parts) {
+    const float other = __shfl_xor(csum, 32);
+    if (h == 0 && n < d.N) d.col_parts[(long)wj * d.N + n] = csum + other;
   }
   if ((p.debug & 1) && d.sk_ws && tid == 0 && blockIdx.x < 1024) {
     long long* o = reinterpret_cast<long long*>(reinterpret_cast<char*>(d.sk_ws) + d.sk_ws_bytes - 65536) + blockIdx.x * 8;
@@ -274,3 +281,12 @@
   WsArgs p;
   return ws_plan(d, p) ? 1 : 0;
 }
+
+extern "C" int ctts_gemm_col_parts_rows(const ctts_gemm_desc* dp) {
+  if (!dp || !dp->epi_bwd) return 0;
+  ctts_gemm_desc d = *dp;
+  if (d.nb0 < 1) d.nb0 = 1;
+  if (d.nb1 < 1) d.nb1 = 1;
+  WsArgs p;
+  return ws_plan(d, p) ? p.wg_per_block : 0;
+}
diff --git a/comprehensive-transformer-tts_amd/kernels.py b/comprehensive-transformer-tts_amd/kernels.py
--- a/comprehensive-transformer-tts_amd/kernels.py
+++ b/comprehensive-transformer-tts_amd/kernels.py
@@ -208,10 +208,13 @@
                sA=(0, 0), sB=(0, 0), sC=(0, 0), lens=None, lim=(0, 0, 0), conv=None, conv_on_b=False, split_k=1, alpha=1.0,
                bias=None, Z=None, ldz=0, act=ACT_NONE, p_drop=0.0, seed=None, drop_offset=0, R=None, ldr=0, rowscale=None,
                row_lens=None, row_T=0, row_halo=0, tile_map=None, E=None, rowsub=None, use_sk=None, epi_bwd=False, split_overwrite=False,
-               bf16_split=None, a_planes=None, b_planes=None, c_planes=None):
+               bf16_split=None, a_planes=None, b_planes=None, c_planes=None, col_parts=None, c_planes_only=False):
     d = GemmDesc()
     if c_planes is not None:
         d.C_planes = c_planes.data_ptr()
+        d.c_planes_only = int(bool(c_planes_only))
+    if col_parts is not None:
+        d.col_parts = col_parts.data_ptr()
     d.bf16_split = int(BF16_SPLIT if bf16_split is None else bf16_split)
     if a_planes is not None and b_planes is not None:
         d.A_planes, d.B_planes = a_planes.data_ptr(), b_planes.data_ptr()
@@ -369,6 +372,33 @@
     return bool(_lib.load().ctts_gemm_takes_weight_stationary(C.byref(d)))
 
 
+def gemm_col_parts_rows(A, B, Cout, M, N, K, lda, ldb, ldc, a_kc=True, b_kc=True, **kw):
+    d = _gemm_desc(A, B, Cout, M, N, K, lda, ldb, ldc, a_kc, b_kc, **kw)
+    return int(_lib.load().ctts_gemm_col_parts_rows(C.byref(d)))
+
+
+def add_col_parts(parts, count, n, dst, alpha):
+    sink = _sink_for(dst)
+    if sink is not None:
+        sink.add(parts, count, n, n, dst, alpha)
+        return
+    t = (_lib.PsumTask * 1)()
+    t[0].src, t[0].dst, t[0].n, t[0].stride, t[0].count, t[0].alpha = parts.data_ptr(), dst.data_ptr(), int(n), int(n), int(count), float(alpha)
+    _lib.check(_lib.load().ctts_partial_sums(t, 1, _stream()), "ctts_partial_sums")
+
+
+def join_planes(pl, out=None):
+    rows, cols = pl.shape[0], pl.shape[1] * 32
+    if out is None:
+        out = torch.empty(rows, cols, dtype=torch.float32, device=pl.device)
+    assert out.is_contiguous() and out.numel() == rows * cols and pl.is_contiguous()
+    _lib.check(_lib.load().ctts_join_planes(pl.data_ptr(), out.data_ptr(), rows, cols, _stream()), "ctts_join_planes")
+    return out
+
+
+POISON_PLANES_ONLY = _os.environ.get("CTTS_POISON_PLANES_ONLY", "0") == "1"
+
+
 def gemm_ws_enable(on):
     return bool(_lib.load().ctts_gemm_ws_enable(1 if on else 0))
 
@@ -388,6 +418,24 @@
     for t, (w, cout, cin, k), o in zip(arr, weights, outs):
         t.src, t.dst, t.cout, t.cin, t.k = _p(_f32c(w, "conv weight (GEMM-major)")), _p(o), int(cout), int(cin), int(k)
     _lib.check(_lib.load().ctts_conv_dgrad_weights(arr, len(arr), _stream()), "ctts_conv_dgrad_weights")
+    return outs
+
+
+def conv_weight_prepare(weights, want):
+    if not weights:
+        return []
+    outs = []
+    arr = (_lib.WprepTask * len(weights))()
+    for t, (w, cout, cin, k), (w_wd, w_fwd, w_dg) in zip(arr, weights, want):
+        if (w_fwd and cin % 32) or (w_dg and cout % 32):
+            raise _lib.CttsError(f"conv_weight_prepare: plane sets need cin % 32 == 0 (forward) / cout % 32 == 0 (data gradient); got {cin}, {cout}")
+        wd = torch.empty(cin, k * cout, dtype=torch.float32, device=w.device) if w_wd else None
+        fp = new_planes(cout, k * cin, w.device) if w_fwd else None
+        dp = new_planes(cin, k * cout, w.device) if w_dg else None
+        outs.append((wd, fp, dp))
+        t.src, t.wd, t.fwd_planes, t.dgrad_planes = _p(_f32c(w, "conv weight (GEMM-major)")), _p(wd), _p(fp), _p(dp)
+        t.cout, t.cin, t.k = int(cout), int(cin), int(k)
+    _lib.check(_lib.load().ctts_conv_weight_prepare(arr, len(arr), _stream()), "ctts_conv_weight_prepare")
     return outs
 
 
diff --git a/comprehensive-transformer-tts_amd/ops.py b/comprehensive-transformer-tts_amd/ops.py
--- a/comprehensive-transformer-tts_amd/ops.py
+++ b/comprehensive-transformer-tts_amd/ops.py
@@ -176,6 +176,9 @@
 import os as _os
 _DGRAD_SPLIT_K = int(_os.environ.get("CTTS_DGRAD_SPLIT_K", "1"))
 _FUSE_EPILOGUE_BWD = _os.environ.get("CTTS_FUSE_EPI_BWD", "1") != "0"
+_EPI_COL_PARTS = _os.environ.get("CTTS_EPI_COL_PARTS", "1") != "0"
+_EPI_PLANES_ONLY = _os.environ.get("CTTS_EPI_PLANES_ONLY", "1") != "0"
+EPI_STATS = {"col_parts": 0, "planes_only": 0, "joined": 0}
 _WGRAD_SPLIT_MULT = float(_os.environ.get("CTTS_WGRAD_SPLIT_MULT", "1"))
 _WGRAD_SPLIT_CAP = int(_os.environ.get("CTTS_WGRAD_SPLIT_CAP", "512"))
 
@@ -195,20 +198,31 @@
         self.Z = self.seed = None
         self.act, self.p_drop, self.drop_offset = ACT_NONE, 0.0, 0
         self.conv_dims = None
+        self.producer = None
         self.armed = False
         self.gen = 0
         self.done = set()
-
-    def arm(self, Z, act, p_drop, seed, drop_offset, conv_dims=None):
+        self.bias_done = set()
+        self.planes_only = {}
+
+    def arm(self, Z, act, p_drop, seed, drop_offset, conv_dims=None, producer=None):
         self.Z, self.act, self.p_drop, self.seed, self.drop_offset = Z, act, p_drop, seed, drop_offset
         self.conv_dims = conv_dims
+        self.producer = producer
         self.gen += 1
         self.armed = True
         return self.gen
 
     def take(self):
         self.armed = False
-        return (self.Z, self.act, self.p_drop, self.seed, self.drop_offset, self.gen, self.conv_dims)
+        producer, self.producer = self.producer, None
+        return (self.Z, self.act, self.p_drop, self.seed, self.drop_offset, self.gen, self.conv_dims, producer)
+
+
+class _Producer:
+
+    def __init__(self, **kw):
+        self.__dict__.update(kw)
 
 
 class _LinearConv(torch.autograd.Function):
@@ -250,7 +264,10 @@
         ctx.link, ctx.link_role, ctx.link_snap = None, 0, None
         if link is not None and _FUSE_EPILOGUE_BWD:
             if link_role == 1 and rowscale is None and residual is None and (act != ACT_NONE or p_drop > 0):
-                ctx.link_gen = link.arm(Z, act, p_drop, seed, drop_offset, conv_dims=(Cin, ksize) if ksize else None)
+                info = _Producer(bias=b if (b is not None and ctx.needs_input_grad[2]) else None, alpha=alpha, x=x, w=w, ksize=ksize,
+                                 pad_left=ctx.pad_left if ksize else 0, pr=pr, row_lens=row_lens, row_T=row_T, amp=ctx.amp,
+                                 x_planes=ctx.x_planes, need_dgrad=ctx.needs_input_grad[0], need_wgrad=ctx.needs_input_grad[1])
+                ctx.link_gen = link.arm(Z, act, p_drop, seed, drop_offset, conv_dims=(Cin, ksize) if ksize else None, producer=info)
                 ctx.link, ctx.link_role = link, 1
             elif link_role == 2 and link.armed and not ksize:
                 ctx.link, ctx.link_role, ctx.link_snap = link, 2, link.take()
@@ -272,10 +289,26 @@
         dX = dW = dB = None
         want_bias = has_bias and ctx.needs_input_grad[2]
         fuse_bias = want_bias and _fusable(b)
+        lazy_planes = None
+
+        def fp32():
+            nonlocal lazy_planes
+            if lazy_planes is not None:
+                K.join_planes(lazy_planes, out=dZ)
+                lazy_planes = None
+                EPI_STATS["joined"] += 1
         if ctx.link_role == 1 and ctx.link_gen in ctx.link.done:
             ctx.link.done.discard(ctx.link_gen)
             dZ, d_res = dY, None
-            if want_bias:
+            po = ctx.link.planes_only.pop(ctx.link_gen, None)
+            if po is not None:
+                if po[0].data_ptr() != dZ.data_ptr() or po[0].numel() != dZ.numel():
+                    raise RuntimeError("EpiLink: the planes-only dZ of the consumer did not reach its producer as it was handed out")
+                lazy_planes = po[1]
+            if ctx.link_gen in ctx.link.bias_done:
+                ctx.link.bias_done.discard(ctx.link_gen)
+            elif want_bias:
+                fp32()
                 if fuse_bias:
                     K.colsum(dZ.view(M, N), scale=alpha, acc_into=_grad_of(b))
                 else:
@@ -294,29 +327,40 @@
             if want_bias and not fuse_bias:
                 dB = dBn
         dz_planes = K.planes_of(dZ) if ksize else None
+        if lazy_planes is not None and dz_planes is None:
+            dz_planes = lazy_planes
+        if not ksize:
+            fp32()
         if ksize:
             T = x.shape[-2]
             pad = ctx.pad_left
             pad_d = ksize - 1 - pad
             if ctx.needs_input_grad[0]:
-                wd = _DGRAD_W.take(w, (Cin, ksize * N))
-                if wd is None:
-                    wd = torch.empty(Cin, ksize * N, dtype=torch.float32, device=x.device)
+                wd, wd_real = _prepared_dgrad_operand(w, (Cin, ksize * N), pop=True)
+
+                def make_wd():
+                    m = torch.empty(Cin, ksize * N, dtype=torch.float32, device=x.device)
                     wmaj = _gemm_major(w)
                     if wmaj is not None:
-                        K.conv_weight_repack(wmaj, wd, N, Cin, ksize, 4)
+                        K.conv_weight_repack(wmaj, m, N, Cin, ksize, 4)
                     else:
-                        K.conv_weight_repack(w.contiguous(), wd, N, Cin, ksize, 1)
+                        K.conv_weight_repack(w.contiguous(), m, N, Cin, ksize, 1)
+                    return m
+                if wd is None:
+                    wd, wd_real = make_wd(), True
                 tiles = -(-M // 64) * -(-Cin // 64)
                 sk = min(4, max(2, -(-2304 // tiles))) if (_DGRAD_SPLIT_K and tiles < 1536 and ksize * N >= 4096) else 1
                 dX = torch.empty_like(x)
-                dg0 = dict(conv=(T, pad_d, N), alpha=alpha, row_halo=pad_d, **rl)
+                dg0 = _conv_dgrad_kw(T, pad_d, N, alpha, rl)
                 planes = _operand_planes("dgrad", w, dZ.view(M, N), wd, M, Cin, ksize * N, N, ksize * N, Cin, dX, dict(split_overwrite=True, **dg0),
                                          a_given=dz_planes)
                 if planes:
                     dz_planes = planes["a_planes"]
                     K.gemm(dZ, wd, dX, M, Cin, ksize * N, N, ksize * N, Cin, True, True, split_k=1, split_overwrite=True, **dg0, **planes)
                 else:
+                    fp32()
+                    if not wd_real:
+                        wd, wd_real = make_wd(), True
                     dg = dict(tile_map=pr.tile_map(pad_d, M) if pr is not None else None, **dg0)
                     if sk > 1 and K.gemm_takes_persistent(dZ, wd, x, M, Cin, ksize * N, N, ksize * N, Cin, True, True, split_k=1, **dg):
                         sk = 1
@@ -325,15 +369,19 @@
                 Kd = ksize * Cin
                 fused = _fusable(w)
                 gmaj = _gemm_major(_grad_of(w)) if fused else None
-                wk = dict(conv=(T, pad, Cin), conv_on_b=True, split_k=max(2, _split_k_for(N, Kd, M)), alpha=alpha, **rl)
+                wk = _conv_wgrad_kw(T, pad, Cin, N, Kd, M, alpha, rl)
                 if gmaj is not None:
                     wp = _wgrad_planes(dZ.view(M, N), x.view(M, Cin), dz_planes, getattr(ctx, "x_planes", None), gmaj, N, Kd, M, Cin, wk)
+                    if not wp:
+                        fp32()
                     with _wgrad_scope(True, dZ, x, *wp.values(), rows=M):
                         K.gemm(dZ, x, gmaj, N, Kd, M, N, Cin, Kd, False, False, tile_map=kmap, defer=_WGRAD["stream"] is None, **wk, **wp)
                 else:
                     dwf = torch.empty(N, Kd, dtype=torch.float32, device=x.device)
                     wk["split_overwrite"] = True
                     wp = _wgrad_planes(dZ.view(M, N), x.view(M, Cin), dz_planes, getattr(ctx, "x_planes", None), dwf, N, Kd, M, Cin, wk)
+                    if not wp:
+                        fp32()
                     with _wgrad_scope(fused, dZ, x, dwf, *wp.values(), rows=M):
                         K.gemm(dZ, x, dwf, N, Kd, M, N, Cin, Kd, False, False, tile_map=kmap, **wk, **wp)
                         if fused:
@@ -347,7 +395,7 @@
             if ctx.needs_input_grad[0]:
                 dX = torch.empty_like(x)
                 if ctx.link_role == 2:
-                    lZ, lact, lp, lseed, loff, lgen, lconv = ctx.link_snap
+                    lZ, lact, lp, lseed, loff, lgen, lconv, prod = ctx.link_snap
                     gk = dict(alpha=alpha, epi_bwd=True, Z=lZ, ldz=Cin, act=lact, p_drop=lp, seed=lseed, drop_offset=loff,
                               tile_map=pr.tile_map(0, M) if pr is not None else None, **rl)
                     cpl = None
@@ -356,9 +404,26 @@
                         cand = K.new_planes(M, Cin, dZ.device)
                         if K.gemm_takes_weight_stationary(dZ, w, dX, M, Cin, N, N, Cin, Cin, True, False, c_planes=cand, **gk):
                             cpl = cand
-                    K.gemm(dZ, w, dX, M, Cin, N, N, Cin, Cin, True, False, c_planes=cpl, **gk)
+                    pbias = _grad_of(prod.bias) if (prod is not None and _EPI_COL_PARTS) else None
+                    parts, n_parts = None, 0
+                    if pbias is not None and pbias.is_contiguous() and dZ.is_cuda:
+                        n_parts = K.gemm_col_parts_rows(dZ, w, dX, M, Cin, N, N, Cin, Cin, True, False, c_planes=cpl, **gk)
+                        if n_parts > 0:
+                            parts = torch.empty(n_parts, Cin, dtype=torch.float32, device=dZ.device)
+                    only = (cpl is not None and _EPI_PLANES_ONLY and prod is not None and (prod.bias is None or parts is not None)
+                            and _producer_reads_planes_only(prod, dX, cpl))
+                    if only and K.POISON_PLANES_ONLY:
+                        dX.fill_(float("nan"))
+                    K.gemm(dZ, w, dX, M, Cin, N, N, Cin, Cin, True, False, c_planes=cpl, col_parts=parts, c_planes_only=only, **gk)
                     if cpl is not None:
                         K.attach_planes(dX, cpl)
+                    if parts is not None:
+                        K.add_col_parts(parts, n_parts, Cin, pbias, prod.alpha)
+                        ctx.link.bias_done.add(lgen)
+                        EPI_STATS["col_parts"] += 1
+                    if only:
+                        ctx.link.planes_only[lgen] = (dX, cpl)
+                        EPI_STATS["planes_only"] += 1
                     ctx.link.done.add(lgen)
                 else:
                     K.gemm(dZ, w, dX, M, Cin, N, N, Cin, Cin, True, False, alpha=alpha,
@@ -392,19 +457,31 @@
             return None
         return ent[0]
 
+    def peek(self, w, shape):
+        ent = dict.get(self, w.data_ptr())
+        if ent is None or ent[1] != _wstamp(w) or tuple(ent[0].shape) != tuple(shape):
+            return None
+        return ent[0]
+
 
 _DGRAD_W = _DgradCache()
 
 _PLANES = {"fwd": {}, "dgrad": {}, "want_fwd": set(), "want_dgrad": set()}
 
 
+def _prepared_dgrad_operand(w, shape, pop):
+    wd = _DGRAD_W.take(w, shape) if pop else _DGRAD_W.peek(w, shape)
+    if wd is not None:
+        return wd, True
+    n = int(shape[0]) * int(shape[1])
+    ent = _PLANES["dgrad"].get(w.data_ptr())
+    if ent is not None and ent[1] == _wstamp(w) and ent[0].numel() == 3 * n:
+        return ent[0].view(-1).view(torch.float32)[:n].view(*shape), False
+    return None, False
+
+
 def _operand_planes(kind, w, a_mat, b_mat, M, N, Kdim, lda, ldb, ldc, out, gk, a_given=None):
-    conv = gk.get("conv")
-    if not K.plane_shape_ok(M, N, Kdim, conv[2] if conv is not None else None):
-        return {}
-    if not (a_mat.is_contiguous() and b_mat.is_contiguous() and a_mat.shape[1] % 32 == 0 and b_mat.shape[1] % 32 == 0):
-        return {}
-    if not K.gemm_takes_planes(a_mat, b_mat, out, M, N, Kdim, lda, ldb, ldc, True, True, a_planes=_FakePlanes(a_mat), b_planes=_FakePlanes(b_mat), **gk):
+    if not _takes_operand_planes(a_mat, b_mat, M, N, Kdim, lda, ldb, ldc, out, gk):
         return {}
     ent = _PLANES[kind].get(w.data_ptr())
     if ent is not None and ent[1] == _wstamp(w) and ent[0].numel() == 3 * b_mat.numel():
@@ -424,6 +501,60 @@
         return {}
     made = iter(K.split_planes([m for m, pl in ((dz_mat, dz_pl), (x_mat, x_pl)) if pl is None]))
     return dict(a_planes=dz_pl if dz_pl is not None else next(made), b_planes=x_pl if x_pl is not None else next(made))
+
+
+def _conv_dgrad_kw(T, pad_d, N, alpha, rl):
+    return dict(conv=(T, pad_d, N), alpha=alpha, row_halo=pad_d, **rl)
+
+
+def _conv_wgrad_kw(T, pad, Cin, N, Kd, M, alpha, rl):
+    return dict(conv=(T, pad, Cin), conv_on_b=True, split_k=max(2, _split_k_for(N, Kd, M)), alpha=alpha, **rl)
+
+
+def _producer_reads_planes_only(prod, dz, dz_planes):
+    x, w, ksize = prod.x, prod.w, prod.ksize
+    if not ksize or not dz.is_contiguous():
+        return False
+    Cin = x.shape[-1]
+    M = x.numel() // Cin
+    N = w.shape[0]
+    T = x.shape[-2]
+    if dz.numel() != M * N:
+        return False
+    rl = dict(row_lens=prod.row_lens, row_T=prod.row_T) if prod.row_lens is not None else {}
+    if prod.amp is not None:
+        rl["bf16_split"] = prod.amp
+    dz_mat = dz.view(M, N)
+    if prod.need_dgrad:
+        pad_d = ksize - 1 - prod.pad_left
+        wd, _ = _prepared_dgrad_operand(w, (Cin, ksize * N), pop=False)
+        if wd is None:
+            return False
+        gk = dict(split_overwrite=True, **_conv_dgrad_kw(T, pad_d, N, prod.alpha, rl))
+        if not _takes_operand_planes(dz_mat, wd, M, Cin, ksize * N, N, ksize * N, Cin, x, gk):
+            return False
+    if prod.need_wgrad:
+        Kd = ksize * Cin
+        gmaj = _gemm_major(_grad_of(w)) if _fusable(w) else None
+        wk = _conv_wgrad_kw(T, prod.pad_left, Cin, N, Kd, M, prod.alpha, rl)
+        if gmaj is None:
+            wk["split_overwrite"] = True
+        out = gmaj if gmaj is not None else w
+        if not K.plane_wgrad_shape_ok(N, Kd, M, Cin) or not x.is_contiguous():
+            return False
+        xp = prod.x_planes if prod.x_planes is not None else _FakePlanes(x)
+        if not K.gemm_takes_planes(dz_mat, x.view(M, Cin), out, N, Kd, M, N, Cin, Kd, False, False, a_planes=dz_planes, b_planes=xp, **wk):
+            return False
+    return True
+
+
+def _takes_operand_planes(a_mat, b_mat, M, N, Kdim, lda, ldb, ldc, out, gk):
+    conv = gk.get("conv")
+    if not K.plane_shape_ok(M, N, Kdim, conv[2] if conv is not None else None):
+        return False
+    if not (a_mat.is_contiguous() and b_mat.is_contiguous() and a_mat.shape[1] % 32 == 0 and b_mat.shape[1] % 32 == 0):
+        return False
+    return bool(K.gemm_takes_planes(a_mat, b_mat, out, M, N, Kdim, lda, ldb, ldc, True, True, a_planes=_FakePlanes(a_mat), b_planes=_FakePlanes(b_mat), **gk))
 
 
 class _FakePlanes:
@@ -447,15 +578,18 @@
         if wm is not None and w.requires_grad:
             N, Cin, k = w.shape
             todo.append((w, (wm.detach(), N, Cin, k)))
-    mats, slots = [], []
-    for (w, (wm, _, _, _)), wd in zip(todo, K.conv_dgrad_weights([t for _, t in todo])):
-        _DGRAD_W[w.data_ptr()] = (wd, _wstamp(w))
-        if w.data_ptr() in _PLANES["want_fwd"]:
-            mats.append(wm.contiguous()); slots.append(("fwd", w))
-        if w.data_ptr() in _PLANES["want_dgrad"]:
-            mats.append(wd); slots.append(("dgrad", w))
-    for (kind, w), pl in zip(slots, K.split_planes(mats)):
-        _PLANES[kind][w.data_ptr()] = (pl, _wstamp(w))
+    want = []
+    for w, (_, N, Cin, _) in todo:
+        fwd = w.data_ptr() in _PLANES["want_fwd"] and Cin % 32 == 0
+        dg = w.data_ptr() in _PLANES["want_dgrad"] and N % 32 == 0
+        want.append((not dg, fwd, dg))
+    for (w, _), (wd, fp, dp) in zip(todo, K.conv_weight_prepare([t for _, t in todo], want)):
+        if wd is not None:
+            _DGRAD_W[w.data_ptr()] = (wd, _wstamp(w))
+        if fp is not None:
+            _PLANES["fwd"][w.data_ptr()] = (fp, _wstamp(w))
+        if dp is not None:
+            _PLANES["dgrad"][w.data_ptr()] = (dp, _wstamp(w))
 
 
 def clear_dgrad_weights():
diff --git a/include/ctts.h b/include/ctts.h
--- a/include/ctts.h
+++ b/include/ctts.h
@@ -40,12 +40,16 @@
   const uint16_t* A_planes;
   const uint16_t* B_planes;
   uint16_t* C_planes;
+  float* col_parts;
+  int32_t c_planes_only;
 } ctts_gemm_desc;
 
 int ctts_gemm(const ctts_gemm_desc* d, void* stream);
 int ctts_gemm_split_plan(const ctts_gemm_desc* d, int32_t* count, int64_t* stride);
 typedef struct ctts_repack_task { const float* src; float* dst; int32_t cout, cin, k; } ctts_repack_task;
 int ctts_conv_dgrad_weights(const ctts_repack_task* tasks, int ntasks, void* stream);
+typedef struct ctts_wprep_task { const float* src; float* wd; uint16_t* fwd_planes; uint16_t* dgrad_planes; int32_t cout, cin, k; } ctts_wprep_task;
+int ctts_conv_weight_prepare(const ctts_wprep_task* tasks, int ntasks, void* stream);
 int ctts_posembed_fwd(const float* x, const int32_t* pos, const float* table, const float* alpha, const float* rowscale, float* y,
                       int64_t rows, int C, float p_drop, const uint64_t* seed, uint32_t drop_offset, void* stream);
 int ctts_posembed_bwd(const float* dy, const int32_t* pos, const float* table, const float* rowscale, float* dx, float* dalpha,
@@ -60,10 +64,12 @@
 int ctts_gemm_takes_persistent(const ctts_gemm_desc* d);
 int ctts_gemm_ws_enable(int on);
 int ctts_gemm_takes_weight_stationary(const ctts_gemm_desc* d);
+int ctts_gemm_col_parts_rows(const ctts_gemm_desc* d);
 int ctts_gemm_takes_bf16_split(const ctts_gemm_desc* d);
 int ctts_gemm_takes_planes(const ctts_gemm_desc* d);
 typedef struct ctts_split_task { const float* src; uint16_t* dst; int64_t rows, cols, ld; } ctts_split_task;
 int ctts_split_planes(const ctts_split_task* tasks, int ntasks, void* stream);
+int ctts_join_planes(const uint16_t* planes, float* dst, int64_t rows, int64_t cols, void* stream);
 
 int ctts_rowdot_heads(const float* a, const float* b, float* out, int B, int T, int H, int dh, void* stream);
 
```

Measured after the change: 695,500 mel-frames/s (median of 6 runs). Within noise of the previous version (+1.0%).
